# stivalaa/cuda_satabsearch

Hardware: AMD Instinct MI355X
Metric: db-structure scorings/sec (query×db pairs/sec) at r=128; 1/2/4/8 MI355X (higher is better)
Workload: dtype i32

## Files before the change

### cuda_satabsearch_amd/_native.py

```python
import ctypes as C
import os

PKG = os.path.dirname(os.path.abspath(__file__))
DEVICE_LIB = os.environ.get("SAT_DEVICE_LIB") or os.path.join(PKG, "libsatabsearch.so")
HOST_LIB = os.path.join(PKG, "libsathost.so")

MAXDIM = 111
LABELSIZE = 8

ABI_SYMBOLS = (
    "sat_last_error", "sat_abi_version", "sat_device_count", "sat_ctx_create", "sat_ctx_destroy",
    "sat_db_upload_packed", "sat_db_upload_search", "sat_db_upload_dense", "sat_db_size", "sat_query_set", "sat_search",
    "sat_search_async", "sat_device_scores", "sat_device_ssemaps", "sat_query_order", "sat_sync",
    "sat_search_timed", "sat_use_stream", "sat_use_own_stream", "sat_results", "sat_queries_set", "sat_query_count", "sat_topk",
    "sat_topk_hits", "sat_stat_d2h_bytes", "sat_debug_lds_layout", "sat_last_launch_info",
    "sat_multi_create", "sat_multi_destroy", "sat_multi_device_count", "sat_multi_gather_kind", "sat_multi_db_upload_packed",
    "sat_multi_shards", "sat_multi_queries_set", "sat_multi_search", "sat_multi_search_topk", "sat_multi_stat_d2h_bytes",
    "sat_search_matches", "sat_multi_search_matches",
    "sat_search_pairs", "sat_search_refine", "sat_multi_search_refine",
    "sat_hits_cutoff", "sat_multi_search_cutoff", "sat_multi_hits_cutoff",
    "sat_search_pairs_matches", "sat_multi_search_pairs_matches",
)


class SatError(RuntimeError):
    pass


class Hit(C.Structure):
    _fields_ = [("entry", C.c_int32), ("score", C.c_int32), ("norm2", C.c_double), ("zscore", C.c_double),
                ("pvalue", C.c_double)]


class StructSetC(C.Structure):
    _fields_ = [
        ("count", C.c_int), ("capacity", C.c_int),
        ("cells", C.c_int64), ("cells_cap", C.c_int64),
        ("order", C.POINTER(C.c_int)), ("name", C.POINTER(C.c_char)),
        ("cell_off", C.POINTER(C.c_int64)), ("tab", C.POINTER(C.c_uint8)),
        ("dist", C.POINTER(C.c_float)), ("skipped", C.c_int),
    ]


_device = None
_host = None


def device_lib():
    global _device
    if _device is None:
        if not os.path.exists(DEVICE_LIB):
            raise SatError(f"{DEVICE_LIB} is missing: run `python -m cuda_satabsearch_amd.build` "
                           "(the GPU search has no fallback implementation)")
        lib = C.CDLL(DEVICE_LIB)
        lib.sat_last_error.restype = C.c_char_p
        lib.sat_abi_version.restype = C.c_int
        lib.sat_device_count.restype = C.c_int
        lib.sat_ctx_create.restype = C.c_void_p
        lib.sat_ctx_create.argtypes = [C.c_int, C.c_uint64]
        lib.sat_ctx_destroy.argtypes = [C.c_void_p]
        lib.sat_ctx_destroy.restype = None
        lib.sat_db_upload_packed.argtypes = [C.c_void_p, C.c_int, C.c_void_p, C.c_void_p, C.c_void_p,
                                             C.c_void_p, C.c_void_p]
        lib.sat_db_upload_search.argtypes = [C.c_void_p, C.c_int, C.c_void_p, C.c_void_p, C.c_void_p,
                                             C.c_void_p, C.c_void_p, C.c_int, C.c_int, C.c_int]
        lib.sat_db_upload_dense.argtypes = [C.c_void_p, C.c_int, C.c_void_p, C.c_void_p, C.c_void_p,
                                            C.c_int, C.c_void_p]
        lib.sat_db_size.argtypes = [C.c_void_p]
        lib.sat_query_set.argtypes = [C.c_void_p, C.c_int, C.c_void_p, C.c_void_p, C.c_int, C.c_void_p,
                                      C.c_uint32]
        lib.sat_search.argtypes = [C.c_void_p, C.c_int, C.c_int, C.c_int, C.c_void_p, C.c_void_p,
                                   C.POINTER(C.c_double)]
        lib.sat_search_async.argtypes = [C.c_void_p, C.c_int, C.c_int, C.c_int]
        lib.sat_use_stream.argtypes = [C.c_void_p, C.c_void_p]
        lib.sat_use_own_stream.argtypes = [C.c_void_p]
        lib.sat_results.argtypes = [C.c_void_p, C.c_int, C.c_void_p, C.c_void_p]
        lib.sat_queries_set.argtypes = [C.c_void_p, C.c_int, C.c_void_p, C.c_void_p, C.c_void_p, C.c_int,
                                        C.c_void_p, C.c_uint32]
        lib.sat_query_count.argtypes = [C.c_void_p]
        lib.sat_topk.argtypes = [C.c_void_p, C.c_int, C.c_int, C.c_void_p, C.c_void_p]
        lib.sat_topk_hits.argtypes = [C.c_void_p, C.c_int, C.c_void_p, C.c_void_p]
        lib.sat_stat_d2h_bytes.argtypes = [C.c_void_p]
        lib.sat_stat_d2h_bytes.restype = C.c_uint64
        lib.sat_last_launch_info.argtypes = [C.c_void_p]
        lib.sat_last_launch_info.restype = C.c_char_p
        lib.sat_debug_lds_layout.argtypes = [C.c_int] * 8 + [C.c_void_p]
        lib.sat_debug_lds_layout.restype = None
        lib.sat_multi_create.restype = C.c_void_p
        lib.sat_multi_create.argtypes = [C.c_int, C.c_void_p, C.c_uint64]
        lib.sat_multi_destroy.argtypes = [C.c_void_p]
        lib.sat_multi_destroy.restype = None
        lib.sat_multi_device_count.argtypes = [C.c_void_p]
        lib.sat_multi_gather_kind.argtypes = [C.c_void_p]
        lib.sat_multi_gather_kind.restype = C.c_char_p
        lib.sat_multi_db_upload_packed.argtypes = [C.c_void_p, C.c_int, C.c_void_p, C.c_void_p, C.c_void_p, C.c_void_p]
        lib.sat_multi_shards.argtypes = [C.c_void_p, C.c_void_p]
        lib.sat_multi_queries_set.argtypes = [C.c_void_p, C.c_int, C.c_void_p, C.c_void_p, C.c_void_p, C.c_int, C.c_void_p, C.c_uint32]
        lib.sat_multi_search.argtypes = [C.c_void_p, C.c_int, C.c_int, C.c_int, C.c_void_p, C.c_void_p, C.POINTER(C.c_double)]
        lib.sat_multi_search_topk.argtypes = [C.c_void_p, C.c_int, C.c_int, C.c_int, C.c_int, C.c_void_p, C.c_void_p,
                                              C.POINTER(C.c_double)]
        lib.sat_search_matches.argtypes = [C.c_void_p, C.c_int, C.c_int, C.c_int, C.c_void_p, C.c_void_p, C.c_void_p,
                                           C.c_void_p, C.POINTER(C.c_double)]
        lib.sat_multi_search_matches.argtypes = [C.c_void_p, C.c_int, C.c_int, C.c_int, C.c_void_p, C.c_void_p,
                                                 C.c_void_p, C.c_void_p, C.POINTER(C.c_double)]
        lib.sat_search_pairs.argtypes = [C.c_void_p, C.c_int, C.c_int, C.c_int, C.c_int, C.c_void_p, C.c_void_p,
                                         C.c_void_p, C.c_void_p, C.POINTER(C.c_double)]
        lib.sat_search_pairs_matches.argtypes = [C.c_void_p, C.c_int, C.c_int, C.c_int, C.c_int, C.c_void_p, C.c_void_p,
                                                 C.c_void_p, C.c_void_p, C.c_void_p, C.c_void_p, C.POINTER(C.c_double)]
        lib.sat_multi_search_pairs_matches.argtypes = lib.sat_search_pairs_matches.argtypes
        lib.sat_search_refine.argtypes = [C.c_void_p, C.c_int, C.c_int, C.c_int, C.c_int, C.c_int, C.c_int,
                                          C.c_void_p, C.c_void_p, C.c_void_p]
        lib.sat_multi_search_refine.argtypes = [C.c_void_p, C.c_int, C.c_int, C.c_int, C.c_int, C.c_int, C.c_int,
                                                C.c_void_p, C.c_void_p, C.c_void_p, C.POINTER(C.c_double),
                                                C.POINTER(C.c_double)]
        lib.sat_hits_cutoff.argtypes = [C.c_void_p, C.c_double, C.c_int, C.c_void_p, C.c_int, C.c_void_p, C.c_void_p]
        lib.sat_multi_search_cutoff.argtypes = [C.c_void_p, C.c_int, C.c_int, C.c_int, C.c_double, C.c_int, C.c_void_p,
                                                C.c_int, C.c_void_p, C.c_void_p, C.POINTER(C.c_double)]
        lib.sat_multi_hits_cutoff.argtypes = [C.c_void_p, C.c_double, C.c_int, C.c_void_p, C.c_int, C.c_void_p, C.c_void_p]
        lib.sat_multi_stat_d2h_bytes.argtypes = [C.c_void_p]
        lib.sat_multi_stat_d2h_bytes.restype = C.c_uint64
        lib.sat_device_scores.argtypes = [C.c_void_p]
        lib.sat_device_scores.restype = C.c_void_p
        lib.sat_device_ssemaps.argtypes = [C.c_void_p]
        lib.sat_device_ssemaps.restype = C.c_void_p
        lib.sat_query_order.argtypes = [C.c_void_p]
        lib.sat_sync.argtypes = [C.c_void_p]
        lib.sat_search_timed.argtypes = [C.c_void_p, C.c_int, C.c_int, C.c_int, C.c_int,
                                         C.POINTER(C.c_double), C.POINTER(C.c_double)]
        _device = lib
    return _device


def host_lib():
    global _host
    if _host is None:
        if not os.path.exists(HOST_LIB):
            raise SatError(f"{HOST_LIB} is missing: run `python -m cuda_satabsearch_amd.build`")
        lib = C.CDLL(HOST_LIB)
        lib.sat_set_init.argtypes = [C.POINTER(StructSetC)]
        lib.sat_set_init.restype = None
        lib.sat_set_free.argtypes = [C.POINTER(StructSetC)]
        lib.sat_set_free.restype = None
        lib.sat_read_structures.argtypes = [C.c_void_p, C.POINTER(StructSetC), C.c_char_p]
        lib.sat_read_structures.restype = C.c_int
        lib.sat_read_structures_file.argtypes = [C.c_char_p, C.POINTER(StructSetC), C.c_char_p]
        lib.sat_read_structures_file.restype = C.c_int
        lib.sat_set_save_binary.argtypes = [C.POINTER(StructSetC), C.c_char_p]
        lib.sat_set_load_binary.argtypes = [C.c_char_p, C.POINTER(StructSetC)]
        lib.sat_set_write_ascii.argtypes = [C.POINTER(StructSetC), C.c_char_p]
        lib.sat_distance_cell.argtypes = [C.c_char_p]
        lib.sat_distance_cell.restype = C.c_float
        lib.sat_norm2.argtypes = [C.c_int, C.c_int, C.c_int]
        lib.sat_norm2.restype = C.c_double
        lib.sat_z_gumbel_trunc.argtypes = [C.c_double]
        lib.sat_z_gumbel_trunc.restype = C.c_double
        lib.sat_pv_gumbel.argtypes = [C.c_double]
        lib.sat_pv_gumbel.restype = C.c_double
        lib.sat_entry_cost.argtypes = [C.c_int]
        lib.sat_entry_cost.restype = C.c_double
        lib.sat_shard_cuts.argtypes = [C.c_int, C.c_void_p, C.c_int, C.c_void_p]
        _host = lib
    return _host


_libc = C.CDLL(None)
_libc.fopen.restype = C.c_void_p
_libc.fopen.argtypes = [C.c_char_p, C.c_char_p]
_libc.fclose.argtypes = [C.c_void_p]
_libc.fgets.restype = C.c_void_p
_libc.fgets.argtypes = [C.c_char_p, C.c_int, C.c_void_p]


def libc():
    return _libc
```

### cuda_satabsearch_amd/csrc/diag/sat_diag.hpp

```cpp
#pragma once

#define SAT_DIAG_ARGS unsigned long long *diag;

#ifdef SAT_DIAG_PHASE
#define SAT_PHASE_INIT unsigned long long ph_acc[11] = {0, 0, 0, 0, 0, 0, 0, 0, 0, 0, 0}, ph_t0 = __builtin_amdgcn_s_memtime()
#define SAT_PHASE(k) do { const unsigned long long ph_t1 = __builtin_amdgcn_s_memtime(); ph_acc[k] += ph_t1 - ph_t0; ph_t0 = ph_t1; } while (0)
#define SAT_PHASE_FLUSH do { if ((threadIdx.x & 63) == 0) for (int k = 0; k < 11; k++) if (k < 8 || k == 10) atomicAdd(a.diag + k, ph_acc[k]); } while (0)
#endif

#ifdef SAT_DIAG_FS_ROWS
#define SAT_DIAG_FS_ROWS_ONLY 1
#endif

#ifdef SAT_DIAG_DUP
#if SAT_DIAG_DUP == 1
#define SAT_DIAG_DUP_CELLS(row, l0, l1, l2, l3) do { if constexpr (CELLS == SAT_CELLS_FULL8) {                                            \
        typedef const volatile __attribute__((address_space(3))) unsigned long long *lds_vu64;                          \
        const unsigned long long dup0 = *(lds_vu64)&(row).cells[l0], dup1 = *(lds_vu64)&(row).cells[l1],                  \
                                 dup2 = *(lds_vu64)&(row).cells[l2], dup3 = *(lds_vu64)&(row).cells[l3];                  \
        asm volatile("" : : "v"(dup0), "v"(dup1), "v"(dup2), "v"(dup3)); } } while (0)
#elif SAT_DIAG_DUP == 2
#define SAT_DIAG_DUP_MAPWORD(p) (void)*(const volatile __attribute__((address_space(3))) uint32_t *)(p)
#elif SAT_DIAG_DUP == 3
#define SAT_DIAG_DUP_ATOMIC(p) __hip_atomic_fetch_add((p), 0, __ATOMIC_RELAXED, __HIP_MEMORY_SCOPE_WAVEFRONT)
#elif SAT_DIAG_DUP == 4
#define SAT_DIAG_DUP_MAPBYTE(p) (void)*(const volatile __attribute__((address_space(3))) uint8_t *)(p)
#endif
#endif

#ifdef SAT_DIAG_PERTURB
#define SAT_R10(x) x x x x x x x x x x
namespace satk {
__device__ __forceinline__ void perturb(uint32_t (&d)[4])
{
#if SAT_DIAG_PERTURB == 1
    asm volatile(SAT_R10("v_add_u32 %0, %0, 1\n v_add_u32 %1, %1, 1\n v_add_u32 %2, %2, 1\n v_add_u32 %3, %3, 1\n")
                 : "+v"(d[0]), "+v"(d[1]), "+v"(d[2]), "+v"(d[3]));
#elif SAT_DIAG_PERTURB == 2
    uint32_t s0 = __builtin_amdgcn_readfirstlane(d[1]), s1 = __builtin_amdgcn_readfirstlane(d[2]);
    asm volatile(SAT_R10("s_add_u32 %0, %0, 1\n s_add_u32 %1, %1, 1\n s_add_u32 %0, %0, 3\n s_add_u32 %1, %1, 3\n")
                 : "+s"(s0), "+s"(s1) : : "scc");
    d[1] = s0; d[2] = s1;
#elif SAT_DIAG_PERTURB == 3
    uint32_t addr = (threadIdx.x & 63u) << 2, t0, t1;
    asm volatile("ds_read_b32 %0, %2\n ds_read_b32 %1, %2 offset:256\n ds_read_b32 %0, %2 offset:512\n ds_read_b32 %1, %2 offset:768\n"
                 "ds_read_b32 %0, %2 offset:1024\n ds_read_b32 %1, %2 offset:1280\n ds_read_b32 %0, %2 offset:1536\n"
                 "ds_read_b32 %1, %2 offset:1792\n ds_read_b32 %0, %2 offset:2048\n ds_read_b32 %1, %2 offset:2304\n s_waitcnt lgkmcnt(0)\n"
                 : "=&v"(t0), "=&v"(t1) : "v"(addr) : "memory");
    d[0] ^= t0 & t1 & 0x80000000u;
#elif SAT_DIAG_PERTURB == 4
    asm volatile(SAT_R10("s_nop 0\n s_nop 0\n s_nop 0\n s_nop 0\n"));
#elif SAT_DIAG_PERTURB == 5
    asm volatile(SAT_R10("v_lshlrev_b32 %0, 1, %0\n v_lshlrev_b32 %1, 1, %1\n v_lshlrev_b32 %2, 1, %2\n v_lshlrev_b32 %3, 1, %3\n")
                 : "+v"(d[0]), "+v"(d[1]), "+v"(d[2]), "+v"(d[3]));
#endif
}
}
#define SAT_DIAG_PERTURB_INIT uint32_t pert[4] = { (uint32_t)lane_id, 1u, 2u, 3u }
#define SAT_DIAG_PERTURB_STEP satk::perturb(pert)
#define SAT_DIAG_PERTURB_END do { if ((pert[0] ^ pert[1] ^ pert[2] ^ pert[3]) == 0xDEADBEEFu) Q.scores[e] = -1; } while (0)
#endif

#ifdef SAT_DIAG_SELFCHECK
#define SAT_DIAG_SELFCHECK_STEP do {                                                                                     \
        const uint8_t keep_ = smap_b[map_byte_addr(ssei)];                                                               \
        smap_b[map_byte_addr(ssei)] = (uint8_t)newj;                                                                     \
        int chk_ = score_rows();                                                                                         \
        if (lpc >= 2) chk_ += __shfl_xor(chk_, 1, 64);                                                                   \
        if (lpc == 4) chk_ += __shfl_xor(chk_, 2, 64);                                                                   \
        smap_b[map_byte_addr(ssei)] = keep_;                                                                             \
        if (part == 0) { atomicAdd(a.diag + 9, 1ull); if (chk_ != newscore) atomicAdd(a.diag + 8, 1ull); }               \
    } while (0)
#endif

#if defined(SAT_DIAG_HOST)
#include <cstdio>
namespace satdiag {
inline unsigned long long *&buffer() { static unsigned long long *d = nullptr; return d; }
inline unsigned long long (&last())[16] { static unsigned long long h[16]; return h; }
inline hipError_t begin(hipStream_t stream, unsigned long long *&arg)
{
    if (!buffer()) { hipError_t e = hipMalloc(&buffer(), 16 * sizeof(unsigned long long)); if (e != hipSuccess) return e; }
    arg = buffer();
    return hipMemsetAsync(buffer(), 0, 16 * sizeof(unsigned long long), stream);
}
inline hipError_t end(hipStream_t stream)
{
    hipError_t e = hipStreamSynchronize(stream);
    if (e != hipSuccess) return e;
    e = hipMemcpy(last(), buffer(), sizeof(unsigned long long) * 16, hipMemcpyDeviceToHost);
#ifdef SAT_DIAG_PHASE
    unsigned long long tot = 0;
    for (int k = 0; k < 11; k++) if (k < 8 || k == 10) tot += last()[k];
    static const char *nm[11] = { "draw+proposal", "compaction set-up", "compacted rounds", "read-back/static loops",
                                 "best tracking", "metropolis+update", "initial full score", "staging+restart loop", "", "",
                                 "thinit" };
    for (int k = 0; k < 11; k++)
        if (k < 8 || k == 10) fprintf(stderr, "phase %-24s %14llu wave-cycles %5.1f%%\n", nm[k], last()[k], tot ? 100.0 * last()[k] / tot : 0.0);
#endif
    return e;
}
}
extern "C" void sat_diag_counters(unsigned long long out[16]) { for (int k = 0; k < 16; k++) out[k] = satdiag::last()[k]; }
#endif
```

### cuda_satabsearch_amd/csrc/sat_capi.hip

```cpp
#include <hip/hip_runtime.h>

#include <algorithm>
#include <atomic>
#include <chrono>
#include <cmath>
#include <cstdarg>
#include <cstdio>
#include <cstdlib>
#include <cstring>
#include <new>
#include <thread>
#include <type_traits>
#include <vector>

#include "satabsearch.h"
#ifdef SAT_DIAG
#define SAT_DIAG_HOST 1
#endif
#include "sat_sa_kernel.hpp"
#include "sat_ctx.hpp"
#include "host/sat_gumbel.h"

namespace {

thread_local char g_err[512] = "";

}

int sat_fail(int code, const char *fmt, ...)
{
    va_list ap;
    va_start(ap, fmt);
    vsnprintf(g_err, sizeof(g_err), fmt, ap);
    va_end(ap);
    return code;
}

namespace {

const int kBucketMax[kNumBuckets] = { 16, 32, 48, 64, 80, 96, 111 };
constexpr size_t kLdsLimit = 160 * 1024;

int build_metropolis_table(sat_ctx *ctx)
{
    const int max_nd = 4 * (SAT_MAXDIM - 1);
    const float umin = 2.3283064e-10f;
    std::vector<float> tab;
    std::vector<int32_t> rows(2 * SAT_MAXITER);
    volatile float temp = 10.0f;
    for (int it = 0; it < SAT_MAXITER; it++) {
        int last = 0;
        std::vector<float> row(max_nd + 1);
        for (int nd = 0; nd <= max_nd; nd++) {
            volatile float x = (float)(-nd) / temp;
            row[nd] = expf(x);
            if (row[nd] > umin) last = nd;
        }
        rows[2 * it] = (int32_t)tab.size();
        rows[2 * it + 1] = last;
        tab.push_back(8589934592.0f);
        for (int nd = 0; nd <= last; nd++) tab.push_back(ldexpf(row[nd], 32));
        tab.push_back(0.0f);
        temp = temp * 0.95f;
    }
    int rc;
    if ((rc = ctx->d_ptab.grow(tab.size())) != SAT_OK || (rc = ctx->d_prow.grow(rows.size())) != SAT_OK) return rc;
    HIP_TRY(hipMemcpy(ctx->d_ptab.get(), tab.data(), tab.size() * sizeof(float), hipMemcpyHostToDevice));
    HIP_TRY(hipMemcpy(ctx->d_prow.get(), rows.data(), rows.size() * sizeof(int32_t), hipMemcpyHostToDevice));
    return SAT_OK;
}

int build_gumbel_tables(sat_ctx *ctx)
{
    double z[256], p[256];
    for (int x = -128; x < 128; x++) {
        z[x + 128] = sat_z_gumbel_trunc((double)x);
        p[x + 128] = sat_pv_gumbel(z[x + 128]);
    }
    int rc;
    if ((rc = ctx->d_gumbel_z.grow(256)) != SAT_OK || (rc = ctx->d_gumbel_p.grow(256)) != SAT_OK) return rc;
    HIP_TRY(hipMemcpy(ctx->d_gumbel_z.get(), z, sizeof z, hipMemcpyHostToDevice));
    HIP_TRY(hipMemcpy(ctx->d_gumbel_p.get(), p, sizeof p, hipMemcpyHostToDevice));
    return SAT_OK;
}

void free_db(sat_ctx *ctx)
{
    ctx->d_orders.reset();
    ctx->d_cell_off.reset();
    ctx->d_tab.reset();
    ctx->d_dist.reset();
    ctx->d_ordinal.reset();
    ctx->d_lists.reset();
    ctx->d_scores.reset();
    ctx->d_ssemaps.reset();
    ctx->desc_dirty = true;
    ctx->n_entries = 0;
    ctx->min_rows = 0;
    ctx->searched_nq = 0;
    ctx->h_orders.clear();
}

template <int V> using Int = std::integral_constant<int, V>;

template <typename F> auto by_class(int n1p, F f)
{
    switch (n1p) {
    case 16: return f(Int<16>{});
    case 32: return f(Int<32>{});
    case 64: return f(Int<64>{});
    default: return f(Int<112>{});
    }
}

template <typename F> auto by_flag(bool b, F f) { return b ? f(std::true_type{}) : f(std::false_type{}); }

template <int First, int Last, typename F> auto by_value(int v, F f)
{
    if constexpr (First == Last) return f(Int<Last>{});
    else return v == First ? f(Int<First>{}) : by_value<First + 1, Last>(v, f);
}

template <typename F> auto by_layout(int m2w, int cells, F f)
{
    if (m2w == 1) return f(Int<1>{}, Int<SAT_CELLS_FULL8>{});
    if (m2w == 2) return cells == SAT_CELLS_FULL5 ? f(Int<2>{}, Int<SAT_CELLS_FULL5>{}) : f(Int<2>{}, Int<SAT_CELLS_TRI5>{});
    return f(Int<4>{}, Int<SAT_CELLS_TRI5>{});
}

enum SaMode { kPlain = 0, kMatch = 1, kPair = 2, kPairMatch = 3 };

struct SaKernel { const void *fn; int mode, n1p, m2w, cells; bool qlds; int opt, wpl; };

template <int MODE, int N1P, int M2W, bool QLDS, int OPT, int WPL, int CELLS> const void *sa_instance()
{
    static_assert(MODE == kPlain || WPL == 0, "words per lane are an argument of the plain kernel only");
    static_assert(MODE == kPlain || MODE == kPair || OPT == -1, "the match families read their options from the arguments");
    if constexpr (MODE == kPlain) return reinterpret_cast<const void *>(sat_sa_kernel<N1P, M2W, QLDS, OPT, WPL, CELLS>);
    else if constexpr (MODE == kPair) return reinterpret_cast<const void *>(sat_sa_pair_kernel<N1P, M2W, QLDS, OPT, CELLS>);
    else if constexpr (MODE == kMatch) return reinterpret_cast<const void *>(sat_sa_match_kernel<N1P, M2W, QLDS, CELLS>);
    else return reinterpret_cast<const void *>(sat_sa_pair_match_kernel<N1P, M2W, QLDS, CELLS>);
}

SaKernel pick_sa_kernel(int mode, int n1p, int m2w, int cells, bool qlds, int opt, int wpl)
{
    SaKernel k = { nullptr, mode, n1p, m2w, cells, qlds, -1, 0 };
    by_value<kPlain, kPairMatch>(mode, [&](auto md) {
        by_class(n1p, [&](auto c) {
            constexpr int MODE = decltype(md)::value, N1P = decltype(c)::value;
            constexpr bool kQ = N1P < 32;
            auto take = [&](auto q, auto o, auto w) {
                k.opt = decltype(o)::value;
                k.wpl = decltype(w)::value;
                k.fn = by_layout(m2w, cells, [](auto m, auto l) {
                    return sa_instance<MODE, N1P, decltype(m)::value, decltype(q)::value, decltype(o)::value, decltype(w)::value,
                                       decltype(l)::value>();
                });
            };
            const std::bool_constant<kQ> q{};
            if constexpr (MODE == kPlain) {
                if (opt >= 4 && qlds == kQ && m2w == 4)
                    return by_value<4, 11>(opt, [&](auto o) {
                        k.opt = decltype(o)::value;
                        k.fn = sa_instance<kPlain, N1P, 4, kQ, decltype(o)::value, 0, SAT_CELLS_TRI5>();
                    });
                if (opt >= 0 && opt < 4 && qlds == kQ)
                    return by_value<0, 3>(opt, [&](auto o) {
                        if constexpr ((decltype(o)::value & 1) == 0) take(q, o, Int<0>{});
                        else {
                            if (wpl == 4) return take(q, o, Int<4>{});
                            if constexpr (N1P <= 64)
                                if (wpl == 3) return take(q, o, Int<3>{});
                            if constexpr (N1P == 16) {
                                if (wpl == 2) return take(q, o, Int<2>{});
                                if (wpl == 1) return take(q, o, Int<1>{});
                            }
                            take(q, o, Int<0>{});
                        }
                    });
            }
            if constexpr (MODE == kPair)
                if ((opt == 0 || opt == 1) && qlds == kQ) return by_value<0, 1>(opt, [&](auto o) { take(q, o, Int<0>{}); });
            by_flag(qlds, [&](auto qg) { take(qg, Int<-1>{}, Int<0>{}); });
        });
    });
    return k;
}

hipError_t launch_sa(const SaKernel &k, dim3 grid, dim3 block, size_t lds, hipStream_t stream, const SatKernelArgs &a,
                     const SatPairArgs *px, const SatMatchArgs *mx)
{
    void *args[3] = { const_cast<SatKernelArgs *>(&a), nullptr, nullptr };
    int n = 1;
    if (k.mode & kPair) args[n++] = const_cast<SatPairArgs *>(px);
    if (k.mode & kMatch) args[n++] = const_cast<SatMatchArgs *>(mx);
    (void)hipLaunchKernel(k.fn, grid, block, args, lds, stream);
    return hipGetLastError();
}

std::string launch_info(const SaKernel &k, int items, int grid_x, int grid_y, int epw, int threads, size_t lds)
{
    static const char *const kName[4] = { "sat_sa_kernel", "sat_sa_match_kernel", "sat_sa_pair_kernel", "sat_sa_pair_match_kernel" };
    char targs[48] = "", count[32] = "", buf[200];
    if (k.mode == kPlain) snprintf(targs, sizeof targs, "%d, %d, ", k.opt, k.wpl);
    if (k.mode == kPair) snprintf(targs, sizeof targs, "%d, ", k.opt);
    if (k.mode & kPair) snprintf(count, sizeof count, " items %d", items);
    snprintf(buf, sizeof buf, "%s<%d, %d, %s, %s%d>%s grid %d x %d block %d x %d lds %zu", kName[k.mode], k.n1p, k.m2w,
             k.qlds ? "true" : "false", targs, k.cells, count, grid_x, grid_y, epw, threads, lds);
    return buf;
}

const int kClassN1P[4] = { 16, 32, 64, 112 };

int refresh_descriptors(sat_ctx *ctx, bool lsoln, hipStream_t stream)
{
    const size_t nq = ctx->queries.size();
    const size_t rows = (size_t)(ctx->n_entries > ctx->min_rows ? ctx->n_entries : ctx->min_rows);
    bool moved = false;
    int rc = ctx->d_scores.grow(nq * rows, &moved);
    if (rc != SAT_OK) return rc;
    if (moved) ctx->desc_dirty = true;
    if (lsoln) {
        size_t need = 0, n1sum = 0;
        for (auto &q : ctx->queries) {
            q.ssemap_off = need;
            need += (size_t)ctx->n_entries * q.n1;
            n1sum += (size_t)q.n1;
        }
        if (rows * n1sum > need) need = rows * n1sum;
        if ((rc = ctx->d_ssemaps.grow(need, &moved)) != SAT_OK) return rc;
        if (moved || !ctx->desc_lsoln) ctx->desc_dirty = true;
    }
    if (!ctx->desc_dirty) return SAT_OK;

    std::vector<SatQuery> desc;
    desc.reserve(nq);
    for (int c = 0; c < 4; c++) {
        ctx->class_begin[c] = (int)desc.size();
        ctx->class_n1max[c] = 0;
        ctx->class_wpl[c] = -1;
        for (size_t qi = 0; qi < nq; qi++) {
            auto &q = ctx->queries[qi];
            if (q.n1p != kClassN1P[c]) continue;
            q.cls = c;
            q.desc = (int)desc.size();
            const uint8_t *blob = ctx->d_qblob.get() + q.blob_off;
            const size_t groups = (size_t)q.n1p / 4 * q.n1p;
            SatQuery d;
            d.qdist = reinterpret_cast<const float4 *>(blob);
            d.qcode = reinterpret_cast<const uint32_t *>(blob + groups * 16);
            d.qtypes = blob + groups * 20;
            d.qpair = reinterpret_cast<const uint2 *>(blob + ((groups * 20 + (size_t)q.n1p + 15) & ~(size_t)15));
            d.n1 = q.n1;
            d.pad_ = 0;
            d.seed_q = ctx->seed + ((uint64_t)q.ordinal << 32);
            d.scores = ctx->d_scores.get() + qi * (size_t)ctx->n_entries;
            d.ssemaps = lsoln ? ctx->d_ssemaps.get() + q.ssemap_off : nullptr;
            desc.push_back(d);
            if (q.n1 > ctx->class_n1max[c]) ctx->class_n1max[c] = q.n1;
            int lpi, wpl;
            satk::compaction_shape((q.n1 + 3) >> 2, lpi, wpl);
            ctx->class_wpl[c] = ctx->class_wpl[c] < 0 ? wpl : (ctx->class_wpl[c] == wpl ? wpl : 0);
        }
        if (ctx->class_wpl[c] < 0) ctx->class_wpl[c] = 0;
    }
    ctx->class_begin[4] = (int)desc.size();
    HIP_TRY(hipMemcpyAsync(ctx->d_qdesc.get(), desc.data(), desc.size() * sizeof(SatQuery), hipMemcpyHostToDevice, stream));
    HIP_TRY(hipStreamSynchronize(stream));
    ctx->desc_dirty = false;
    ctx->desc_lsoln = lsoln;
    return SAT_OK;
}

int resident_by_lds(size_t bytes) { return (int)(128 / ((bytes + 1279) / 1280)); }

int pick_epw(const void *fn, int threads, size_t lds_stride)
{
    int best = 1, best_entries = 0;
    for (int k = 1; k * threads <= 512 && (size_t)k * lds_stride <= kLdsLimit; k++) {
        if (k > 1 && (k * threads / 64) % 4 != 0) continue;
        int by_regs = 0;
        if (hipOccupancyMaxActiveBlocksPerMultiprocessor(&by_regs, fn, k * threads, 0) != hipSuccess) {
            (void)hipGetLastError();
            return 1;
        }
        const int by_lds = resident_by_lds((size_t)k * lds_stride);
        const int entries = (by_regs < by_lds ? by_regs : by_lds) * k;
        if (entries > best_entries) { best_entries = entries; best = k; }
    }
    return best;
}

int launch_setup(sat_ctx *ctx, const void *fn, int threads, size_t lds_stride, long long work, int *epw)
{
    if (ctx->lds_attr_done.insert(fn).second)
        HIP_TRY(hipFuncSetAttribute(fn, hipFuncAttributeMaxDynamicSharedMemorySize, (int)kLdsLimit));
    if (!epw) return SAT_OK;
    *epw = 1;
    if (work >= 8192) {
        const auto key = std::make_tuple(fn, threads, lds_stride);
        auto it = ctx->epw_choice.find(key);
        if (it == ctx->epw_choice.end()) it = ctx->epw_choice.emplace(key, pick_epw(fn, threads, lds_stride)).first;
        *epw = it->second;
    }
    if (ctx->tune.epw >= 1 && (size_t)ctx->tune.epw * lds_stride <= kLdsLimit && ctx->tune.epw * threads <= 1024)
        *epw = ctx->tune.epw;
    return SAT_OK;
}

SatKernelArgs base_args(const sat_ctx *ctx, int lorder, int lsoln, int maxstart)
{
    SatKernelArgs a;
    a.orders = ctx->d_orders.get();
    a.cell_off = ctx->d_cell_off.get();
    a.tab_tri = ctx->d_tab.get();
    a.dist_tri = ctx->d_dist.get();
    a.ordinal = ctx->d_ordinal.get();
    a.lorder = lorder ? 1 : 0;
    a.lsoln = lsoln ? 1 : 0;
    a.maxstart = maxstart;
    a.ptab = ctx->d_ptab.get();
    a.prow = ctx->d_prow.get();
    a.bmap_slabs = nullptr;
    a.bmap_slab_words = 0;
    return a;
}

int check_ready(const sat_ctx *ctx, bool need_db, int maxstart)
{
    if (!ctx) return sat_fail(SAT_EINVAL, "null context");
    if (need_db && ctx->n_entries <= 0) return sat_fail(SAT_ESTATE, "no database uploaded");
    if (ctx->queries.empty()) return sat_fail(SAT_ESTATE, "no query set");
    if (maxstart < 1) return sat_fail(SAT_EINVAL, "maxstart must be >= 1 (got %d)", maxstart);
    return SAT_OK;
}

struct WgShape { int chains, lpc_shift, threads; bool qlds, compact; size_t lds; };
int size_workgroup(const sat_ctx *ctx, int plan_starts, int n1max, int n1p, int n2max, bool lsoln, bool lorder, WgShape &out)
{
    int chains = (plan_starts + 63) / 64 * 64;
    if (chains > 256) chains = 256;
    if (ctx->tune.chains >= 64 && ctx->tune.chains < chains) chains = ctx->tune.chains / 64 * 64;
    bool compact = lorder != 0;
    if (ctx->tune.compact >= 0) compact = ctx->tune.compact != 0;
    bool qlds = n1p < 32;
    if (ctx->tune.qlds >= 0) qlds = ctx->tune.qlds != 0 || n1p < 32;
    size_t lds = 0;
    for (;;) {
        lds = satk::lds_bytes(n1max, n1p, n2max, chains, chains, lsoln, qlds, compact);
        if (lds <= kLdsLimit) break;
        if (chains > 64) { chains -= 64; continue; }
        if (qlds) {
            qlds = false;
            chains = (plan_starts + 63) / 64 * 64;
            if (chains > 256) chains = 256;
            continue;
        }
        return sat_fail(SAT_EINVAL, "workgroup does not fit in LDS (n1=%d n2=%d)", n1max, n2max);
    }
    int lpc_shift = 0;
    for (int l = 0; l <= 2; l++) {
        if ((chains << l) > 1024 || (l > 0 && n1max <= (8 << (l - 1)))) break;
        const size_t lds_l = satk::lds_bytes(n1max, n1p, n2max, chains, chains << l, lsoln, qlds, compact);
        if (lds_l > kLdsLimit) break;
        lpc_shift = l;
        const int want_waves = ctx->tune.lpc_waves > 0 ? ctx->tune.lpc_waves : (n1p == 112 ? 12 : 8);
        if (resident_by_lds(lds_l) * ((chains << l) / 64) >= want_waves) break;
    }
    if (ctx->tune.lpc >= 0 && ctx->tune.lpc <= 2 && (chains << ctx->tune.lpc) <= 1024) lpc_shift = ctx->tune.lpc;
    for (;; lpc_shift--) {
        lds = satk::lds_bytes(n1max, n1p, n2max, chains, chains << lpc_shift, lsoln, qlds, compact);
        if (lds <= kLdsLimit || lpc_shift == 0) break;
    }
    const int threads = chains << lpc_shift;
    if (ctx->tune.lds_pad && lds + ctx->tune.lds_pad <= kLdsLimit) lds += ctx->tune.lds_pad;
    out.chains = chains;
    out.lpc_shift = lpc_shift;
    out.threads = threads;
    out.qlds = qlds;
    out.compact = compact;
    out.lds = lds;
    return SAT_OK;
}

struct SaLaunch { WgShape w; SaKernel k; int epw; size_t lds_stride, lds_launch; SatKernelArgs args; };

int prepare_sa(sat_ctx *ctx, int mode, int lorder, int lsoln, int maxstart, int plan_starts, int c, int n2max, long long work,
               bool pack, SaLaunch &out)
{
    const int n1p = kClassN1P[c], m2w = satk::set_words(n2max);
    WgShape &w = out.w;
    int rc = size_workgroup(ctx, plan_starts, ctx->class_n1max[c], n1p, n2max, lsoln != 0, lorder != 0, w);
    if (rc != SAT_OK) return rc;
    const bool special = (w.lpc_shift == 0 || m2w == 4) && w.compact == (lorder != 0) && !ctx->tune.general && !(mode & kMatch);
    const int opt = special ? (lorder ? 1 : 0) | (lsoln ? 2 : 0) | (w.lpc_shift << 2) : -1;
    out.k = pick_sa_kernel(mode, n1p, m2w, satk::cell_layout(n2max), w.qlds, opt, ctx->class_wpl[c]);
    if (!out.k.fn) return sat_fail(SAT_EDEVICE, "no kernel variant for n1p=%d m2w=%d", n1p, m2w);
    out.lds_stride = (w.lds + 15) & ~(size_t)15;
    out.epw = 1;
    if ((rc = launch_setup(ctx, out.k.fn, w.threads, out.lds_stride, work, pack ? &out.epw : nullptr)) != SAT_OK) return rc;
    out.lds_launch = out.epw > 1 ? (size_t)out.epw * out.lds_stride : w.lds;
    out.args = base_args(ctx, lorder, lsoln, maxstart);
    out.args.epw = out.epw;
    out.args.tpe = w.threads;
    out.args.lds_stride = (uint32_t)out.lds_stride;
    out.args.lpc_shift = w.lpc_shift;
    out.args.compact = w.compact ? 1 : 0;
    return SAT_OK;
}

struct ListView {
    const int32_t *d_list;
    const int *begin;
    const int *n2max;
    int n;
};

int launch_search(sat_ctx *ctx, int lorder, int lsoln, int maxstart, hipStream_t stream, const ListView *piece = nullptr,
                  const SatMatchArgs *mx = nullptr)
{
    int rc = check_ready(ctx, true, maxstart);
    if (rc != SAT_OK) return rc;
    const ListView whole = { ctx->d_lists.get(), ctx->bucket_begin, ctx->bucket_n2max, ctx->n_entries };
    const ListView &view = piece ? *piece : whole;
    HIP_TRY(hipSetDevice(ctx->device));
    if ((rc = refresh_descriptors(ctx, lsoln != 0, stream)) != SAT_OK) return rc;
#ifdef SAT_DIAG
    unsigned long long *diag = nullptr;
    HIP_TRY(satdiag::begin(stream, diag));
#endif

    const bool replay = mx && mx->replay;
    struct Planned { SaLaunch l; int count, nqc, n2max, max_entries; size_t slab_words; };
    std::vector<Planned> plan;
    for (int c = 0; c < 4; c++) {
        const int nqc = ctx->class_begin[c + 1] - ctx->class_begin[c];
        if (nqc == 0) continue;
        const bool one_launch = (long long)view.n * nqc <= 4096;
        int overall_n2max = 0;
        for (int b = 0; b < kNumBuckets; b++)
            if (view.n2max[b] > overall_n2max) overall_n2max = view.n2max[b];
        for (int b = 0; b < kNumBuckets; b++) {
            Planned pl;
            pl.count = view.begin[b + 1] - view.begin[b];
            pl.n2max = view.n2max[b];
            if (one_launch) {
                if (b > 0) break;
                pl.count = view.n;
                pl.n2max = overall_n2max;
            }
            if (pl.count == 0) continue;
            pl.nqc = nqc;
            rc = prepare_sa(ctx, mx ? kMatch : kPlain, lorder, lsoln, maxstart, replay ? mx->max_matches : maxstart, c, pl.n2max,
                            (long long)pl.count * nqc, true, pl.l);
            if (rc != SAT_OK) return rc;
            pl.l.args.queries = ctx->d_qdesc.get() + ctx->class_begin[c];
            pl.l.args.entry_list = view.d_list + (one_launch ? view.begin[0] : view.begin[b]);
#ifdef SAT_DIAG
            pl.l.args.diag = diag;
#endif
            pl.slab_words = (lsoln || replay) ? (size_t)((ctx->class_n1max[c] + 3) / 4) * pl.l.w.chains
                          : (mx ? (size_t)(1 + pl.l.k.m2w) * (size_t)maxstart : 0);
            plan.push_back(pl);
        }
    }

    std::stable_sort(plan.begin(), plan.end(), [](const Planned &x, const Planned &y) { return x.n2max > y.n2max; });
    const bool fork = plan.size() > 1 && ctx->tune.streams != 0 && ctx->side_stream[0] != nullptr;
    const int nlanes = fork ? (int)(plan.size() < (size_t)kNumBuckets ? plan.size() : (size_t)kNumBuckets) : 1;
    if (fork) HIP_TRY(hipEventRecord(ctx->ev_fork, stream));
    const size_t lane_budget_words = ((size_t)1 << 30) / 4 / (size_t)nlanes;
    const bool slabs = lsoln || mx;
    if (slabs) {
        size_t need_total = 0;
        for (size_t i = 0; i < plan.size(); i++) {
            Planned &pl = plan[i];
            size_t fit = lane_budget_words / pl.slab_words;
            if (fit < 1) fit = 1;
            const int qn_cap = pl.nqc < 65535 ? pl.nqc : 65535;
            pl.max_entries = (int)(fit / (size_t)qn_cap);
            if (pl.max_entries < 1) pl.max_entries = 1;
            if (pl.max_entries > pl.count) pl.max_entries = pl.count;
            const size_t need = pl.slab_words * (size_t)(pl.max_entries + pl.l.epw - 1) * (size_t)qn_cap;
            if (need > need_total) need_total = need;
        }
        need_total *= (size_t)nlanes;
        if ((rc = ctx->d_bmap_slabs.grow_after(stream, need_total)) != SAT_OK) return rc;
    }
    const size_t lane_region_words = slabs ? ctx->d_bmap_slabs.capacity() / (size_t)nlanes : 0;
    for (size_t i = 0; i < plan.size(); i++) {
        const Planned &pl = plan[i];
        const int lane = fork ? (int)(i % (size_t)nlanes) : 0;
        hipStream_t s = fork ? ctx->side_stream[lane] : stream;
        if (fork && i < (size_t)nlanes) HIP_TRY(hipStreamWaitEvent(s, ctx->ev_fork, 0));
        const int max_entries = slabs ? pl.max_entries : pl.count, epw = pl.l.epw;
        for (int q0 = 0; q0 < pl.nqc; q0 += 65535) {
            const int qn = pl.nqc - q0 < 65535 ? pl.nqc - q0 : 65535;
            for (int e0 = 0; e0 < pl.count; e0 += max_entries) {
                const int en = pl.count - e0 < max_entries ? pl.count - e0 : max_entries;
                SatKernelArgs part = pl.l.args;
                part.queries += q0;
                part.entry_list += e0;
                part.n_list = en;
                SatMatchArgs mpart = mx ? *mx : SatMatchArgs{};
                if (lsoln || replay) {
                    part.bmap_slabs = ctx->d_bmap_slabs.get() + (size_t)lane * lane_region_words;
                    part.bmap_slab_words = (uint32_t)pl.slab_words;
                } else if (mx) {
                    mpart.rec_slabs = ctx->d_bmap_slabs.get() + (size_t)lane * lane_region_words;
                    mpart.rec_slab_words = (uint32_t)pl.slab_words;
                }
                HIP_TRY(launch_sa(pl.l.k, dim3((en + epw - 1) / epw, qn), dim3(pl.l.w.threads * epw), pl.l.lds_launch, s, part, nullptr,
                                  &mpart));
            }
        }
    }
    if (fork)
        for (int lane = 0; lane < nlanes; lane++) {
            HIP_TRY(hipEventRecord(ctx->ev_join[lane], ctx->side_stream[lane]));
            HIP_TRY(hipStreamWaitEvent(stream, ctx->ev_join[lane], 0));
        }
    ctx->searched_nq = ctx->queries.size();
    ctx->searched_lsoln = lsoln != 0;
    ctx->last_launch_info.clear();
    for (size_t i = 0; i < plan.size(); i++) {
        const Planned &pl = plan[i];
        if (i) ctx->last_launch_info += "; ";
        ctx->last_launch_info += launch_info(pl.l.k, 0, (pl.count + pl.l.epw - 1) / pl.l.epw, pl.nqc, pl.l.epw, pl.l.w.threads, pl.l.w.lds);
    }
#ifdef SAT_DIAG
    HIP_TRY(satdiag::end(stream));
#endif
    return SAT_OK;
}


int order_bucket(int n2)
{
    int b = 0;
    while (b < kNumBuckets - 1 && n2 > kBucketMax[b]) b++;
    return b;
}

__global__ void __launch_bounds__(256) pair_winners(SatPairItem *items, int n, const unsigned long long *keys)
{
    const int i = blockIdx.x * blockDim.x + threadIdx.x;
    if (i >= n) return;
    const int r = (int)(0xFFFFFFFFu - (uint32_t)(keys[items[i].pair] & 0xFFFFFFFFu));
    items[i].r0 = r;
    items[i].r1 = r + 1;
}

__global__ void __launch_bounds__(256) pair_scores(const unsigned long long *keys, int n, int32_t *scores)
{
    const int i = blockIdx.x * blockDim.x + threadIdx.x;
    if (i < n) scores[i] = (int32_t)(uint32_t)(keys[i] >> 32) - 0x40000000;
}

__global__ void __launch_bounds__(256) pair_match_select(int pair0, int R, int M, const uint32_t *slabs, uint32_t slab_words,
                                                         const uint8_t *setw, const unsigned long long *keys, int32_t *counts,
                                                         int32_t *scores, int32_t *restarts)
{
    __shared__ unsigned long long red[4];
    __shared__ uint32_t uni[4];
    const int p = pair0 + (int)blockIdx.x;
    const uint32_t *rec = slabs + (size_t)blockIdx.x * slab_words;
    const int W = setw[p];
    const int t = (int)threadIdx.x, wave = t >> 6;
    if (t < 4) uni[t] = 0u;
    int m = 0;
    unsigned long long first = 0ull;
    for (int round = 0; round < M; round++) {
        __syncthreads();
        unsigned long long k = 0ull;
        for (int r = t; r < R; r += 256) {
            const int s = (int)rec[r];
            uint32_t hit = 0u;
            for (int w = 0; w < W; w++) hit |= rec[(size_t)(w + 1) * (size_t)R + (size_t)r] & uni[w];
            const unsigned long long rk = (((unsigned long long)(uint32_t)(s + 0x40000000)) << 32) | (0xFFFFFFFFu - (uint32_t)r);
            k = ((round == 0 || (s > 0 && hit == 0u)) && rk > k) ? rk : k;
        }
#pragma unroll
        for (int off = 32; off > 0; off >>= 1) {
            const unsigned long long other = __shfl_xor(k, off, 64);
            k = other > k ? other : k;
        }
        if ((t & 63) == 0) red[wave] = k;
        __syncthreads();
        unsigned long long cur = red[0];
        for (int w = 1; w < 4; w++) cur = red[w] > cur ? red[w] : cur;
        if (cur == 0ull) break;
        if (round == 0) first = cur;
        const uint32_t r = 0xFFFFFFFFu - (uint32_t)(cur & 0xFFFFFFFFu);
        if (t == 0) {
            scores[(size_t)p * M + m] = (int32_t)(uint32_t)(cur >> 32) - 0x40000000;
            restarts[(size_t)p * M + m] = (int32_t)r;
        }
        if (t < W) uni[t] |= rec[(size_t)(t + 1) * (size_t)R + (size_t)r];
        m++;
    }
    if (t == 0) {
        counts[p] = first == keys[p] ? m : -1;
        for (int x = m; x < M; x++) {
            scores[(size_t)p * M + x] = 0;
            restarts[(size_t)p * M + x] = -1;
        }
    }
}

struct PairMatchPass { SatMatchArgs mx; int maxstart; };

struct PairGroups { std::vector<size_t> goff, moff; std::vector<int> gcls, gn2; };

int launch_pair_pass(sat_ctx *ctx, int lorder, bool map_pass, int starts, const SatPairItem *d_items, const PairGroups &grp,
                     std::string &info, const PairMatchPass *pm = nullptr)
{
    hipStream_t stream = ctx->stream;
    const std::vector<size_t> &off = map_pass ? grp.moff : grp.goff;
    SatPairArgs px;
    px.items = nullptr;
    px.keys = ctx->d_pkeys.get();
    px.maps = ctx->d_pmaps.get();
    SatMatchArgs mpart = pm ? pm->mx : SatMatchArgs{};
    mpart.replay = map_pass ? 1 : 0;
    for (size_t g = 0; g < grp.gcls.size(); g++) {
        const int count = (int)(off[g + 1] - off[g]);
        if (count == 0) continue;
        SaLaunch l;
        int rc = prepare_sa(ctx, pm ? kPairMatch : kPair, lorder, map_pass && !pm, pm ? pm->maxstart : starts,
                            map_pass ? (pm ? pm->mx.max_matches : 1) : starts, grp.gcls[g], grp.gn2[g], count, !map_pass, l);
        if (rc != SAT_OK) return rc;
        SatKernelArgs &a = l.args;
        a.entry_list = nullptr;
        a.queries = ctx->d_qdesc.get();
#ifdef SAT_DIAG
        HIP_TRY(satdiag::begin(stream, a.diag));
#endif
        int per_launch = count;
        if (map_pass) {
            const size_t slab_words = (size_t)((ctx->class_n1max[grp.gcls[g]] + 3) / 4) * (size_t)l.w.chains;
            const size_t budget = ((size_t)1 << 28) / 4;
            per_launch = (int)std::min<size_t>((size_t)count, std::max<size_t>(1, budget / slab_words));
            const size_t slabs = (size_t)per_launch + (size_t)l.epw - 1;
            if ((rc = ctx->d_bmap_slabs.grow_after(stream, slab_words * slabs)) != SAT_OK) return rc;
            a.bmap_slabs = ctx->d_bmap_slabs.get();
            a.bmap_slab_words = (uint32_t)slab_words;
        }
        for (int i0 = 0; i0 < count; i0 += per_launch) {
            const int n = count - i0 < per_launch ? count - i0 : per_launch;
            a.n_list = n;
            px.items = d_items + off[g] + (size_t)i0;
            HIP_TRY(launch_sa(l.k, dim3((n + l.epw - 1) / l.epw, 1), dim3(l.w.threads * l.epw), l.lds_launch, stream, a, &px, &mpart));
        }
        if (!info.empty()) info += "; ";
        info += launch_info(l.k, count, (count + l.epw - 1) / l.epw, 1, l.epw, l.w.threads, l.w.lds);
#ifdef SAT_DIAG
        HIP_TRY(satdiag::end(stream));
#endif
    }
    return SAT_OK;
}

int check_pairs(const sat_ctx *ctx, const int32_t *query, const int32_t *entry, int npairs)
{
    if (npairs < 0 || (npairs > 0 && (!query || !entry))) return sat_fail(SAT_EINVAL, "bad pair list");
    const int nq = (int)ctx->queries.size();
    for (int p = 0; p < npairs; p++) {
        if (query[p] < 0 || query[p] >= nq) return sat_fail(SAT_EINVAL, "pair %d: query %d out of range", p, query[p]);
        if (entry[p] < 0 || entry[p] >= ctx->n_entries) return sat_fail(SAT_EINVAL, "pair %d: entry %d out of range", p, entry[p]);
    }
    return SAT_OK;
}

int pair_split(const sat_ctx *ctx, int maxstart, int npairs)
{
    if (ctx->tune.refine_split > 0) return ctx->tune.refine_split < maxstart ? ctx->tune.refine_split : maxstart;
    constexpr long long kTargetItems = 2048;
    const int t0 = std::min(256, (maxstart + 63) / 64 * 64);
    const long long rounds = (maxstart + t0 - 1) / t0;
    long long items = (kTargetItems + npairs - 1) / npairs;
    if (items > rounds) items = rounds;
    if (items < 1) items = 1;
    const long long per = (rounds + items - 1) / items;
    return (int)std::min<long long>(maxstart, per * t0);
}

size_t pair_item_count(int npairs, int maxstart, int split, bool maps)
{
    return (size_t)npairs * (size_t)((maxstart + split - 1) / split) + (maps ? (size_t)npairs : 0);
}

PairGroups build_pair_items(const sat_ctx *ctx, const int32_t *query, const int32_t *entry, int p0, int n, int maxstart, int split,
                            bool maps, std::vector<SatPairItem> &items, uint8_t *setw)
{
    std::vector<std::vector<int>> members(4 * kNumBuckets);
    std::vector<int> n2max(4 * kNumBuckets, 0);
    for (int p = p0; p < p0 + n; p++) {
        const int n2 = ctx->h_orders[(size_t)entry[p]];
        const int g = ctx->queries[(size_t)query[p]].cls * kNumBuckets + order_bucket(n2);
        members[(size_t)g].push_back(p);
        n2max[(size_t)g] = std::max(n2max[(size_t)g], n2);
    }
    auto item_of = [&](int p, int r0, int r1) {
        SatPairItem it{};
        it.pair = p;
        it.desc = ctx->queries[(size_t)query[p]].desc;
        it.entry = entry[p];
        it.r0 = r0;
        it.r1 = r1;
        it.slab = p - p0;
        return it;
    };
    PairGroups grp;
    grp.goff.push_back(items.size());
    for (int g = 0; g < 4 * kNumBuckets; g++) {
        if (members[(size_t)g].empty()) continue;
        for (int p : members[(size_t)g]) {
            if (setw) setw[p] = (uint8_t)satk::set_words(n2max[(size_t)g]);
            for (int r0 = 0; r0 < maxstart; r0 += split) items.push_back(item_of(p, r0, maxstart - r0 < split ? maxstart : r0 + split));
        }
        grp.goff.push_back(items.size());
        grp.gcls.push_back(g / kNumBuckets);
        grp.gn2.push_back(n2max[(size_t)g]);
    }
    if (maps) {
        grp.moff.push_back(items.size());
        for (int g = 0; g < 4 * kNumBuckets; g++) {
            if (members[(size_t)g].empty()) continue;
            for (int p : members[(size_t)g]) items.push_back(item_of(p, 0, 0));
            grp.moff.push_back(items.size());
        }
    }
    return grp;
}

void expand_map(const int8_t *in, int n1, bool used, int32_t *out)
{
    for (int i = 0; i < SAT_MAXDIM; i++) out[i] = (used && i < n1) ? in[i] : -1;
}

int match_args(const sat_ctx *ctx, int max_matches, SatMatchArgs &mx)
{
    if (!ctx) return sat_fail(SAT_EINVAL, "null context");
    if (max_matches < 1 || max_matches > SAT_MAX_MATCHES)
        return sat_fail(SAT_EINVAL, "max_matches must be 1..%d (got %d)", SAT_MAX_MATCHES, max_matches);
    mx = SatMatchArgs{};
    mx.desc_base = ctx->d_qdesc.get();
    mx.max_matches = max_matches;
    mx.map_pitch = SAT_MAXDIM;
    return SAT_OK;
}

}

int sat_pairs_launch(sat_ctx *ctx, int lorder, int maxstart, bool maps, const int32_t *query, const int32_t *entry, int npairs)
{
    int rc = check_ready(ctx, true, maxstart);
    if (rc != SAT_OK) return rc;
    if ((rc = check_pairs(ctx, query, entry, npairs)) != SAT_OK) return rc;
    HIP_TRY(hipSetDevice(ctx->device));
    if ((rc = refresh_descriptors(ctx, false, ctx->stream)) != SAT_OK) return rc;
    ctx->last_launch_info.clear();
    if (npairs == 0) return SAT_OK;

    const int split = pair_split(ctx, maxstart, npairs);
    std::vector<SatPairItem> &items = ctx->h_pitems;
    HIP_TRY(hipStreamSynchronize(ctx->stream));
    items.clear();
    items.reserve(pair_item_count(npairs, maxstart, split, maps));
    const PairGroups grp = build_pair_items(ctx, query, entry, 0, npairs, maxstart, split, maps, items, nullptr);
    if ((rc = ctx->d_pitems.grow_after(ctx->stream, items.size())) != SAT_OK) return rc;
    if ((rc = ctx->d_pkeys.grow_after(ctx->stream, (size_t)npairs)) != SAT_OK) return rc;
    if (maps && (rc = ctx->d_pmaps.grow_after(ctx->stream, (size_t)npairs * SAT_MAXDIM)) != SAT_OK) return rc;
    HIP_TRY(hipMemcpyAsync(ctx->d_pitems.get(), items.data(), items.size() * sizeof(SatPairItem), hipMemcpyHostToDevice, ctx->stream));
    HIP_TRY(hipMemsetAsync(ctx->d_pkeys.get(), 0, (size_t)npairs * sizeof(unsigned long long), ctx->stream));
    std::string info;
    rc = launch_pair_pass(ctx, lorder, false, split, ctx->d_pitems.get(), grp, info);
    if (rc != SAT_OK) return rc;
    char head[96];
    snprintf(head, sizeof head, "score pass (%d restarts, %d per item): ", maxstart, split);
    ctx->last_launch_info = head + info;
    if (maps) {
        const size_t n_score = grp.moff[0];
        const int n_map = (int)(items.size() - n_score);
        HIP_TRY(hipMemsetAsync(ctx->d_pmaps.get(), 0xFF, (size_t)npairs * SAT_MAXDIM, ctx->stream));
        hipLaunchKernelGGL(pair_winners, dim3((unsigned)((n_map + 255) / 256)), dim3(256), 0, ctx->stream,
                           ctx->d_pitems.get() + n_score, n_map, ctx->d_pkeys.get());
        HIP_TRY(hipGetLastError());
        info.clear();
        rc = launch_pair_pass(ctx, lorder, true, 1, ctx->d_pitems.get(), grp, info);
        if (rc != SAT_OK) return rc;
        ctx->last_launch_info += " | map pass: " + info;
    }
    return SAT_OK;
}

int sat_launch_plain(sat_ctx *ctx, int lorder, int maxstart)
{
    return launch_search(ctx, lorder, 0, maxstart, ctx->stream);
}

int sat_pairs_collect(sat_ctx *ctx, int npairs, int32_t *scores, int32_t *ssemaps, const int32_t *query)
{
    HIP_TRY(hipSetDevice(ctx->device));
    if (npairs == 0) return SAT_OK;
    const int rc = ctx->d_pscores.grow_after(ctx->stream, (size_t)npairs);
    if (rc != SAT_OK) return rc;
    hipLaunchKernelGGL(pair_scores, dim3((unsigned)((npairs + 255) / 256)), dim3(256), 0, ctx->stream, ctx->d_pkeys.get(), npairs,
                       ctx->d_pscores.get());
    HIP_TRY(hipGetLastError());
    HIP_TRY(hipStreamSynchronize(ctx->stream));
    HIP_TRY(hipMemcpy(scores, ctx->d_pscores.get(), (size_t)npairs * sizeof(int32_t), hipMemcpyDeviceToHost));
    ctx->d2h_bytes += (size_t)npairs * sizeof(int32_t);
    if (ssemaps) {
        std::vector<int8_t> mp((size_t)npairs * SAT_MAXDIM);
        HIP_TRY(hipMemcpy(mp.data(), ctx->d_pmaps.get(), mp.size(), hipMemcpyDeviceToHost));
        ctx->d2h_bytes += mp.size();
        for (size_t p = 0; p < (size_t)npairs; p++)
            expand_map(mp.data() + p * SAT_MAXDIM, ctx->queries[(size_t)query[p]].n1, true, ssemaps + p * SAT_MAXDIM);
    }
    return SAT_OK;
}

int sat_pair_matches_launch(sat_ctx *ctx, int lorder, int maxstart, int max_matches, bool maps, const int32_t *query,
                            const int32_t *entry, int npairs)
{
    PairMatchPass pm{};
    int rc = match_args(ctx, max_matches, pm.mx);
    if (rc != SAT_OK) return rc;
    if ((rc = check_ready(ctx, true, maxstart)) != SAT_OK) return rc;
    if ((rc = check_pairs(ctx, query, entry, npairs)) != SAT_OK) return rc;
    HIP_TRY(hipSetDevice(ctx->device));
    if ((rc = refresh_descriptors(ctx, false, ctx->stream)) != SAT_OK) return rc;
    ctx->last_launch_info.clear();
    if (npairs == 0) return SAT_OK;
    const size_t M = (size_t)max_matches;
    const int split = pair_split(ctx, maxstart, npairs);

    int n2_all = 0;
    for (int p = 0; p < npairs; p++) n2_all = std::max(n2_all, ctx->h_orders[(size_t)entry[p]]);
    const size_t slab_words = (size_t)(1 + satk::set_words(n2_all)) * (size_t)maxstart;
    const size_t budget_words = ((size_t)1 << 30) / 4;
    const int chunk = (int)std::min<size_t>((size_t)npairs, std::max<size_t>(1, budget_words / slab_words));

    struct Chunk { int p0, n; PairGroups grp; };
    std::vector<Chunk> chunks;
    std::vector<SatPairItem> &items = ctx->h_pitems;
    std::vector<uint8_t> &setw = ctx->h_psetw;
    HIP_TRY(hipStreamSynchronize(ctx->stream));
    items.clear();
    items.reserve(pair_item_count(npairs, maxstart, split, maps));
    setw.assign((size_t)npairs, 0);
    for (int p0 = 0; p0 < npairs; p0 += chunk) {
        const int n = std::min(chunk, npairs - p0);
        chunks.push_back({ p0, n, build_pair_items(ctx, query, entry, p0, n, maxstart, split, maps, items, setw.data()) });
    }
    if ((rc = ctx->d_pitems.grow_after(ctx->stream, items.size())) != SAT_OK ||
        (rc = ctx->d_pkeys.grow_after(ctx->stream, (size_t)npairs)) != SAT_OK ||
        (rc = ctx->d_psetw.grow_after(ctx->stream, (size_t)npairs)) != SAT_OK ||
        (rc = ctx->d_pmout.grow_after(ctx->stream, (size_t)npairs * (1 + 2 * M))) != SAT_OK ||
        (rc = ctx->d_bmap_slabs.grow_after(ctx->stream, slab_words * (size_t)chunk)) != SAT_OK ||
        (maps && (rc = ctx->d_pmaps.grow_after(ctx->stream, (size_t)npairs * M * SAT_MAXDIM)) != SAT_OK))
        return rc;
    HIP_TRY(hipMemcpyAsync(ctx->d_pitems.get(), items.data(), items.size() * sizeof(SatPairItem), hipMemcpyHostToDevice, ctx->stream));
    HIP_TRY(hipMemcpyAsync(ctx->d_psetw.get(), setw.data(), setw.size(), hipMemcpyHostToDevice, ctx->stream));
    HIP_TRY(hipMemsetAsync(ctx->d_pkeys.get(), 0, (size_t)npairs * sizeof(unsigned long long), ctx->stream));
    if (maps) HIP_TRY(hipMemsetAsync(ctx->d_pmaps.get(), 0xFF, (size_t)npairs * M * SAT_MAXDIM, ctx->stream));

    pm.maxstart = maxstart;
    pm.mx.n_entries = 0;
    pm.mx.rec_slab_words = (uint32_t)slab_words;
    pm.mx.counts = ctx->d_pmout.get();
    pm.mx.scores = pm.mx.counts + npairs;
    pm.mx.restarts = pm.mx.scores + (size_t)npairs * M;
    pm.mx.maps = ctx->d_pmaps.get();
    std::string rec_info, map_info;
    for (const Chunk &ch : chunks) {
        pm.mx.rec_slabs = ctx->d_bmap_slabs.get();
        if ((rc = launch_pair_pass(ctx, lorder, false, split, ctx->d_pitems.get(), ch.grp, rec_info, &pm)) != SAT_OK)
            return rc;
        hipLaunchKernelGGL(pair_match_select, dim3((unsigned)ch.n), dim3(256), 0, ctx->stream, ch.p0, maxstart, max_matches,
                           (const uint32_t *)ctx->d_bmap_slabs.get(), (uint32_t)slab_words, (const uint8_t *)ctx->d_psetw.get(),
                           (const unsigned long long *)ctx->d_pkeys.get(), pm.mx.counts, pm.mx.scores, pm.mx.restarts);
        HIP_TRY(hipGetLastError());
        if (maps && (rc = launch_pair_pass(ctx, lorder, true, 1, ctx->d_pitems.get(), ch.grp, map_info, &pm)) != SAT_OK)
            return rc;
    }
    char head[128];
    snprintf(head, sizeof head, "record pass (%d restarts, %d per item, %zu launches of up to %d pairs): ", maxstart, split,
             chunks.size(), chunk);
    ctx->last_launch_info = head + rec_info + " | select";
    if (maps) ctx->last_launch_info += " | map pass: " + map_info;
    return SAT_OK;
}

int sat_pair_matches_collect(sat_ctx *ctx, int max_matches, int npairs, int32_t *counts, int32_t *scores, int32_t *restarts,
                             int32_t *ssemaps, const int32_t *query)
{
    HIP_TRY(hipSetDevice(ctx->device));
    if (npairs == 0) return SAT_OK;
    HIP_TRY(hipStreamSynchronize(ctx->stream));
    const size_t P = (size_t)npairs, M = (size_t)max_matches;
    std::vector<int32_t> out(P * (1 + 2 * M));
    HIP_TRY(hipMemcpy(out.data(), ctx->d_pmout.get(), out.size() * sizeof(int32_t), hipMemcpyDeviceToHost));
    ctx->d2h_bytes += out.size() * sizeof(int32_t);
    for (size_t p = 0; p < P; p++)
        if (out[p] < 1 || out[p] > (int32_t)M)
            return sat_fail(SAT_EDEVICE, "pair %zu: the records and the arg-max key of the record pass disagree", p);
    memcpy(counts, out.data(), P * sizeof(int32_t));
    memcpy(scores, out.data() + P, P * M * sizeof(int32_t));
    memcpy(restarts, out.data() + P + P * M, P * M * sizeof(int32_t));
    if (ssemaps) {
        std::vector<int8_t> mp(P * M * SAT_MAXDIM);
        HIP_TRY(hipMemcpy(mp.data(), ctx->d_pmaps.get(), mp.size(), hipMemcpyDeviceToHost));
        ctx->d2h_bytes += mp.size();
        for (size_t p = 0; p < P; p++)
            for (size_t m = 0; m < M; m++)
                expand_map(mp.data() + (p * M + m) * SAT_MAXDIM, ctx->queries[(size_t)query[p]].n1, (int32_t)m < counts[p],
                           ssemaps + (p * M + m) * SAT_MAXDIM);
    }
    return SAT_OK;
}

namespace {

__global__ void __launch_bounds__(256) validate_cells(int e_begin, int e_end, const int32_t *orders, const int64_t *cell_off,
                                                      const uint8_t *tab, const float *dist, int32_t *first_bad)
{
    const int e = e_begin + blockIdx.x * 4 + (threadIdx.x >> 6), lane = threadIdx.x & 63;
    if (e >= e_end) return;
    const int n = orders[e];
    const int64_t base = cell_off[e];
    const int cells = n * (n + 1) / 2;
    bool bad = false;
    for (int c = lane; c < cells; c += 64) {
        int i = (int)((sqrtf(8.0f * (float)c + 1.0f) - 1.0f) * 0.5f);
        while ((i + 1) * (i + 2) / 2 <= c) i++;
        while (i * (i + 1) / 2 > c) i--;
        const bool diagonal = c == i * (i + 1) / 2 + i;
        const uint8_t t = tab[base + c];
        if (diagonal) {
            bad |= t > 3;
        } else {
            const float ad = fabsf(dist[base + c]);
            bad |= (t & 0x88u) != 0 || (ad >= 1.0e29f && ad <= 3.4028234e38f);
        }
    }
    if (__builtin_amdgcn_ballot_w64(bad) != 0ull && lane == 0) atomicMin(first_bad, e);
}

template <typename F> int timed(sat_ctx *ctx, double *kernel_ms, F launch)
{
    HIP_TRY(hipSetDevice(ctx->device));
    HIP_TRY(hipEventRecord(ctx->ev0, ctx->stream));
    const int rc = launch();
    if (rc != SAT_OK) return rc;
    HIP_TRY(hipEventRecord(ctx->ev1, ctx->stream));
    HIP_TRY(hipStreamSynchronize(ctx->stream));
    if (kernel_ms) {
        float ms = 0.f;
        HIP_TRY(hipEventElapsedTime(&ms, ctx->ev0, ctx->ev1));
        *kernel_ms = ms;
    }
    return SAT_OK;
}

}

extern "C" {

const char *sat_last_error(void) { return g_err; }

int sat_abi_version(void) { return SAT_ABI_VERSION; }

int sat_device_count(void)
{
    int n = 0;
    if (hipGetDeviceCount(&n) != hipSuccess) return 0;
    return n;
}

sat_ctx *sat_ctx_create(int device, uint64_t seed)
{
    int n = sat_device_count();
    if (n <= 0) {
        sat_fail(SAT_ENODEVICE, "no HIP device available (this library has no CPU path)");
        return nullptr;
    }
    if (device < 0 || device >= n) {
        sat_fail(SAT_ENODEVICE, "device %d out of range (0..%d)", device, n - 1);
        return nullptr;
    }
    sat_ctx *ctx = new (std::nothrow) sat_ctx();
    if (!ctx) {
        sat_fail(SAT_ENOMEM, "out of host memory");
        return nullptr;
    }
    ctx->device = device;
    ctx->seed = seed;
    auto init = [&]() -> int {
        HIP_TRY(hipSetDevice(device));
        HIP_TRY(hipStreamCreateWithFlags(&ctx->own_stream, hipStreamNonBlocking));
        ctx->stream = ctx->own_stream;
        HIP_TRY(hipEventCreate(&ctx->ev0));
        HIP_TRY(hipEventCreate(&ctx->ev1));
        auto env_int = [](const char *name, int dflt) { const char *v = getenv(name); return v && *v ? atoi(v) : dflt; };
        ctx->tune.compact = env_int("SAT_EXP_COMPACT", -1);
        ctx->tune.qlds = env_int("SAT_EXP_QLDS", -1);
        ctx->tune.lpc = env_int("SAT_EXP_LPC", -1);
        ctx->tune.general = env_int("SAT_EXP_GENERAL", 0);
        ctx->tune.streams = env_int("SAT_EXP_STREAMS", -1);
        ctx->tune.upload_threads = env_int("SAT_EXP_UPLOAD_THREADS", 0);
        ctx->tune.upload_timing = env_int("SAT_EXP_UPLOAD_TIMING", 0);
        ctx->tune.upload_pieces = env_int("SAT_EXP_UPLOAD_PIECES", 0);
        ctx->tune.epw = env_int("SAT_EXP_EPW", 0);
        ctx->tune.lpc_waves = env_int("SAT_EXP_LPC_WAVES", 0);
        ctx->tune.chains = env_int("SAT_EXP_CHAINS", 0);
        ctx->tune.refine_split = env_int("SAT_EXP_REFINE_SPLIT", 0);
        const int pad = env_int("SAT_EXP_LDS_PAD", 0);
        ctx->tune.lds_pad = pad > 0 ? (size_t)pad : 0;
        if (ctx->tune.streams != 0) {
            for (int b = 0; b < kNumBuckets; b++) {
                HIP_TRY(hipStreamCreateWithFlags(&ctx->side_stream[b], hipStreamNonBlocking));
                HIP_TRY(hipEventCreateWithFlags(&ctx->ev_join[b], hipEventDisableTiming));
            }
            HIP_TRY(hipEventCreateWithFlags(&ctx->ev_fork, hipEventDisableTiming));
        }
        const int rc_tab = build_metropolis_table(ctx);
        if (rc_tab != SAT_OK) return rc_tab;
        hipLaunchKernelGGL(validate_cells, dim3(1), dim3(256), 0, ctx->stream, 0, 0, nullptr, nullptr, nullptr, nullptr, nullptr);
        HIP_TRY(hipGetLastError());
        HIP_TRY(hipStreamSynchronize(ctx->stream));
        return build_gumbel_tables(ctx);
    };
    if (init() != SAT_OK) {
        sat_ctx_destroy(ctx);
        return nullptr;
    }
    return ctx;
}

void sat_ctx_destroy(sat_ctx *ctx)
{
    if (!ctx) return;
    (void)hipSetDevice(ctx->device);
    (void)hipStreamSynchronize(ctx->stream);
    std::vector<hipEvent_t> events = { ctx->ev0, ctx->ev1, ctx->ev_fork };
    events.insert(events.end(), ctx->ev_join, ctx->ev_join + kNumBuckets);
    std::vector<hipStream_t> streams(ctx->side_stream, ctx->side_stream + kNumBuckets);
    streams.push_back(ctx->own_stream);
    delete ctx;
    for (hipEvent_t e : events)
        if (e) (void)hipEventDestroy(e);
    for (hipStream_t st : streams)
        if (st) (void)hipStreamDestroy(st);
}

struct FirstSearch { int lorder, lsoln, maxstart; };

static void bucket_lists(const int32_t *orders, int e_begin, int e_end, int32_t *out, int pos, int *begin, int *n2max)
{
    int count[SAT_MAXDIM + 1] = { 0 }, start[SAT_MAXDIM + 1] = { 0 };
    for (int e = e_begin; e < e_end; e++) count[orders[e]]++;
    for (int b = 0; b < kNumBuckets; b++) {
        begin[b] = pos;
        n2max[b] = 0;
        const int lo = b == 0 ? 0 : kBucketMax[b - 1];
        for (int n = kBucketMax[b] < SAT_MAXDIM ? kBucketMax[b] : SAT_MAXDIM; n > lo; n--) {
            start[n] = pos;
            pos += count[n];
            if (count[n] && n2max[b] == 0) n2max[b] = n;
        }
    }
    begin[kNumBuckets] = pos;
    for (int e = e_begin; e < e_end; e++) out[(size_t)start[orders[e]]++] = e;
}

static int upload_impl(sat_ctx *ctx, int n_entries, const int32_t *orders,
                       const int64_t *cell_off, const uint8_t *tab_tri,
                       const float *dist_tri, const int64_t *db_ordinal, const FirstSearch *first)
{
    if (!ctx) return sat_fail(SAT_EINVAL, "null context");
    if (n_entries <= 0 || !orders || !cell_off || !tab_tri || !dist_tri)
        return sat_fail(SAT_EINVAL, "empty database or null array");
    if (first) {
        const int rc = check_ready(ctx, false, first->maxstart);
        if (rc != SAT_OK) return rc;
    }
    int64_t cells_end = 0;
    bool ascending = true;
    for (int e = 0; e < n_entries; e++) {
        const int n = orders[e];
        if (n < 1 || n > SAT_MAXDIM)
            return sat_fail(SAT_EINVAL, "entry %d: order %d outside 1..%d", e, n, SAT_MAXDIM);
        if (cell_off[e] < 0) return sat_fail(SAT_EINVAL, "entry %d: negative cell offset", e);
        if (cell_off[e] < cells_end) ascending = false;
        int64_t end = cell_off[e] + (int64_t)n * (n + 1) / 2;
        if (end > cells_end) cells_end = end;
        if (db_ordinal && (db_ordinal[e] < 0 || db_ordinal[e] > 0xFFFFFFFFll))
            return sat_fail(SAT_EINVAL, "entry %d: db ordinal out of range", e);
    }
    HIP_TRY(hipSetDevice(ctx->device));
    HIP_TRY(hipStreamSynchronize(ctx->stream));
    free_db(ctx);
    const bool timing = ctx->tune.upload_timing != 0;
    auto now_ms = [] { return std::chrono::duration<double, std::milli>(std::chrono::steady_clock::now().time_since_epoch()).count(); };
    double t_mark = now_ms();
    auto lap = [&](const char *what) {
        if (timing) { const double t = now_ms(); fprintf(stderr, "upload: %-18s %7.3f ms\n", what, t - t_mark); t_mark = t; }
    };

    const size_t dist_bytes = (size_t)cells_end * sizeof(float), tab_bytes = (size_t)cells_end;
    int npieces = 1;
    if (first && ascending) {
        const size_t by_size = dist_bytes / ((size_t)24 << 20);
        npieces = ctx->tune.upload_pieces > 0 ? ctx->tune.upload_pieces : (int)(by_size < 8 ? by_size : 8);
        if (npieces > n_entries) npieces = n_entries;
        if (npieces < 1) npieces = 1;
    }
    std::vector<int> piece_e((size_t)npieces + 1, n_entries);
    piece_e[0] = 0;
    for (int c = 1, e = 0; c < npieces; c++) {
        const int64_t target = cells_end * c / npieces;
        while (e < n_entries && cell_off[e] < target) e++;
        piece_e[(size_t)c] = e > piece_e[(size_t)c - 1] ? e : piece_e[(size_t)c - 1];
    }
    auto piece_cell = [&](int c) -> int64_t { return c >= npieces || piece_e[(size_t)c] >= n_entries ? cells_end : (c == 0 ? 0 : cell_off[piece_e[(size_t)c]]); };

    std::vector<int32_t> lists((size_t)n_entries * (npieces > 1 ? 2 : 1));
    bucket_lists(orders, 0, n_entries, lists.data(), 0, ctx->bucket_begin, ctx->bucket_n2max);
    std::vector<int> piece_begin((size_t)npieces * (kNumBuckets + 1)), piece_n2max((size_t)npieces * kNumBuckets);
    if (npieces > 1) {
        int pos = n_entries;
        for (int c = 0; c < npieces; c++) {
            bucket_lists(orders, piece_e[(size_t)c], piece_e[(size_t)c + 1], lists.data(), pos,
                         &piece_begin[(size_t)c * (kNumBuckets + 1)], &piece_n2max[(size_t)c * kNumBuckets]);
            pos += piece_e[(size_t)c + 1] - piece_e[(size_t)c];
        }
    }

    std::vector<uint32_t> ord(n_entries);
    for (int e = 0; e < n_entries; e++) ord[e] = db_ordinal ? (uint32_t)db_ordinal[e] : (uint32_t)e;

    lap("host lists");
    DevBuf<int32_t> d_bad;
    const int32_t none = 0x7FFFFFFF;
    auto body = [&]() -> int {
        const size_t n = (size_t)n_entries;
        int rc;
        if ((rc = ctx->d_orders.grow(n)) != SAT_OK || (rc = ctx->d_cell_off.grow(n)) != SAT_OK ||
            (rc = ctx->d_ordinal.grow(n)) != SAT_OK || (rc = ctx->d_lists.grow(lists.size())) != SAT_OK ||
            (rc = ctx->d_tab.grow((size_t)cells_end)) != SAT_OK || (rc = ctx->d_dist.grow((size_t)cells_end)) != SAT_OK ||
            (rc = ctx->d_scores.grow(n)) != SAT_OK || (rc = d_bad.grow(1)) != SAT_OK)
            return rc;
        lap("hipMalloc");
        HIP_TRY(hipMemcpy(ctx->d_orders.get(), orders, n * sizeof(int32_t), hipMemcpyHostToDevice));
        HIP_TRY(hipMemcpy(ctx->d_cell_off.get(), cell_off, n * sizeof(int64_t), hipMemcpyHostToDevice));
        HIP_TRY(hipMemcpy(ctx->d_ordinal.get(), ord.data(), n * sizeof(uint32_t), hipMemcpyHostToDevice));
        HIP_TRY(hipMemcpy(ctx->d_lists.get(), lists.data(), lists.size() * sizeof(int32_t), hipMemcpyHostToDevice));
        HIP_TRY(hipMemset(ctx->d_scores.get(), 0, n * sizeof(int32_t)));
        HIP_TRY(hipMemcpy(d_bad.get(), &none, sizeof none, hipMemcpyHostToDevice));
        lap("header copies");
        ctx->n_entries = n_entries;

        unsigned hw = std::thread::hardware_concurrency();
        int nthreads = (int)(hw ? (hw < 4 ? hw : 4) : 1);
        if (ctx->tune.upload_threads > 0) nthreads = ctx->tune.upload_threads;
        if (dist_bytes < ((size_t)32 << 20)) nthreads = 1;
        std::vector<hipError_t> err((size_t)nthreads, hipSuccess);
        std::vector<std::atomic<int>> landed((size_t)npieces);
        for (auto &x : landed) x.store(0);
        auto copy_piece = [&](int t, int c) {
            const size_t c0 = (size_t)piece_cell(c), c1 = (size_t)piece_cell(c + 1);
            auto part = [&](const void *src, void *dst, size_t unit) {
                const size_t bytes = (c1 - c0) * unit, base = c0 * unit;
                const size_t lo = (bytes * (size_t)t / (size_t)nthreads) & ~(size_t)255;
                const size_t hi = t + 1 == nthreads ? bytes : (bytes * (size_t)(t + 1) / (size_t)nthreads) & ~(size_t)255;
                if (hi > lo && err[(size_t)t] == hipSuccess)
                    err[(size_t)t] = hipMemcpy((char *)dst + base + lo, (const char *)src + base + lo, hi - lo, hipMemcpyHostToDevice);
            };
            part(dist_tri, ctx->d_dist.get(), sizeof(float));
            part(tab_tri, ctx->d_tab.get(), 1);
            landed[(size_t)c].fetch_add(1, std::memory_order_release);
        };
        auto piece_complete = [&](int c) {
            while (landed[(size_t)c].load(std::memory_order_acquire) < nthreads) std::this_thread::yield();
        };
        auto helper = [&](int t) {
            (void)hipSetDevice(ctx->device);
            for (int c = 0; c < npieces; c++) {
                copy_piece(t, c);
                if (c + 1 < npieces) piece_complete(c);
            }
        };
        std::vector<std::thread> pool;
        for (int t = 1; t < nthreads; t++) pool.emplace_back(helper, t);
        rc = SAT_OK;
        for (int c = 0; c < npieces; c++) {
            copy_piece(0, c);
            piece_complete(c);
            if (rc != SAT_OK) continue;
            const int e0 = piece_e[(size_t)c], e1 = piece_e[(size_t)c + 1];
            if (e1 <= e0) continue;
            hipLaunchKernelGGL(validate_cells, dim3((unsigned)((e1 - e0 + 3) / 4)), dim3(256), 0, ctx->stream,
                               e0, e1, ctx->d_orders.get(), ctx->d_cell_off.get(), ctx->d_tab.get(), ctx->d_dist.get(), d_bad.get());
            if (hipGetLastError() != hipSuccess) { rc = sat_fail(SAT_EDEVICE, "launch of the cell check failed"); continue; }
            if (first) {
                if (npieces > 1) {
                    const ListView piece = { ctx->d_lists.get(), &piece_begin[(size_t)c * (kNumBuckets + 1)],
                                             &piece_n2max[(size_t)c * kNumBuckets], e1 - e0 };
                    rc = launch_search(ctx, first->lorder, first->lsoln, first->maxstart, ctx->stream, &piece);
                } else {
                    rc = launch_search(ctx, first->lorder, first->lsoln, first->maxstart, ctx->stream);
                }
            }
        }
        for (auto &th : pool) th.join();
        if (rc != SAT_OK) return rc;
        for (int t = 0; t < nthreads; t++) HIP_TRY(err[(size_t)t]);
        lap(first ? "cell copies, checks and the search queued" : "cell copies");
        int32_t bad = none;
        HIP_TRY(hipStreamSynchronize(ctx->stream));
        HIP_TRY(hipMemcpy(&bad, d_bad.get(), sizeof bad, hipMemcpyDeviceToHost));
        lap(first ? "search + validate on GPU" : "validate on GPU");
        if (bad != none) {
            const int e = bad, n = orders[e];
            for (int i = 0; i < n; i++) {
                const int64_t rowbase = cell_off[e] + (int64_t)i * (i + 1) / 2;
                uint8_t ty = tab_tri[rowbase + i];
                if (ty > 3) return sat_fail(SAT_EINVAL, "entry %d: SSE %d has type code %u (0..3 expected)", e, i, ty);
                for (int j = 0; j < i; j++) {
                    if (tab_tri[rowbase + j] & 0x88)
                        return sat_fail(SAT_EINVAL, "entry %d: tableau code 0x%02x at (%d,%d) has a nibble above 7", e, tab_tri[rowbase + j], i, j);
                    float d = dist_tri[rowbase + j];
                    if (std::isfinite(d) && std::fabs(d) >= 1.0e29f)
                        return sat_fail(SAT_EINVAL, "entry %d: distance %g at (%d,%d) out of range", e, d, i, j);
                }
            }
            return sat_fail(SAT_EINVAL, "entry %d: invalid cell", e);
        }
        return SAT_OK;
    };
    const int rc = body();
    d_bad.reset();
    if (rc != SAT_OK) {
        (void)hipStreamSynchronize(ctx->stream);
        free_db(ctx);
        return rc;
    }
    ctx->h_orders.assign(orders, orders + n_entries);
    return SAT_OK;
}

int sat_db_upload_packed(sat_ctx *ctx, int n_entries, const int32_t *orders,
                         const int64_t *cell_off, const uint8_t *tab_tri,
                         const float *dist_tri, const int64_t *db_ordinal)
{
    return upload_impl(ctx, n_entries, orders, cell_off, tab_tri, dist_tri, db_ordinal, nullptr);
}

int sat_db_upload_search(sat_ctx *ctx, int n_entries, const int32_t *orders,
                         const int64_t *cell_off, const uint8_t *tab_tri,
                         const float *dist_tri, const int64_t *db_ordinal,
                         int lorder, int lsoln, int maxstart)
{
    const FirstSearch first = { lorder, lsoln, maxstart };
    return upload_impl(ctx, n_entries, orders, cell_off, tab_tri, dist_tri, db_ordinal, &first);
}

int sat_db_upload_dense(sat_ctx *ctx, int n_entries, const int32_t *orders,
                        const uint8_t *tabs, const float *dmats, int pitch,
                        const int64_t *db_ordinal)
{
    if (!ctx) return sat_fail(SAT_EINVAL, "null context");
    if (n_entries <= 0 || !orders || !tabs || !dmats || pitch < 1)
        return sat_fail(SAT_EINVAL, "empty database or null array");
    std::vector<int64_t> off(n_entries);
    int64_t cells = 0;
    for (int e = 0; e < n_entries; e++) {
        if (orders[e] < 1 || orders[e] > SAT_MAXDIM || orders[e] > pitch)
            return sat_fail(SAT_EINVAL, "entry %d: order %d outside 1..min(%d, pitch %d)", e, orders[e], SAT_MAXDIM, pitch);
        off[e] = cells;
        cells += (int64_t)orders[e] * (orders[e] + 1) / 2;
    }
    std::vector<uint8_t> tt((size_t)cells);
    std::vector<float> dd((size_t)cells);
    for (int e = 0; e < n_entries; e++) {
        const uint8_t *t = tabs + (size_t)e * pitch * pitch;
        const float *d = dmats + (size_t)e * pitch * pitch;
        int64_t c = off[e];
        for (int i = 0; i < orders[e]; i++)
            for (int j = 0; j <= i; j++, c++) {
                tt[(size_t)c] = t[(size_t)i * pitch + j];
                dd[(size_t)c] = d[(size_t)i * pitch + j];
            }
    }
    return sat_db_upload_packed(ctx, n_entries, orders, off.data(), tt.data(), dd.data(), db_ordinal);
}

int sat_db_size(const sat_ctx *ctx) { return ctx ? ctx->n_entries : 0; }

int sat_queries_set(sat_ctx *ctx, int n_queries, const int32_t *n1s, const uint8_t *qtabs,
                    const float *qdmats, int pitch, const uint8_t *qssetypes, uint32_t first_query_ordinal)
{
    if (!ctx) return sat_fail(SAT_EINVAL, "null context");
    if (n_queries < 1 || !n1s || !qtabs || !qdmats || !qssetypes || pitch < 1)
        return sat_fail(SAT_EINVAL, "bad query batch (n_queries=%d pitch=%d)", n_queries, pitch);
    std::vector<sat_ctx::QueryInfo> infos((size_t)n_queries);
    size_t blob_bytes = 0;
    for (int qi = 0; qi < n_queries; qi++) {
        const int n1 = n1s[qi];
        if (n1 < 1 || n1 > SAT_MAXDIM || n1 > pitch)
            return sat_fail(SAT_EINVAL, "query %d: order %d outside 1..min(%d, pitch %d)", qi, n1, SAT_MAXDIM, pitch);
        auto &q = infos[(size_t)qi];
        q.n1 = n1;
        q.n1p = n1 <= 16 ? 16 : (n1 <= 32 ? 32 : (n1 <= 64 ? 64 : 112));
        q.ordinal = first_query_ordinal + (uint32_t)qi;
        q.blob_off = blob_bytes;
        q.ssemap_off = 0;
        const size_t groups = (size_t)q.n1p / 4 * q.n1p;
        blob_bytes += ((groups * 20 + (size_t)q.n1p + 15) & ~(size_t)15) + (size_t)q.n1p * q.n1p * 8;
    }
    std::vector<uint8_t> blob(blob_bytes, 0);
    for (int qi = 0; qi < n_queries; qi++) {
        const auto &q = infos[(size_t)qi];
        const int n1 = q.n1, n1p = q.n1p, groups = n1p / 4;
        const uint8_t *qtab = qtabs + (size_t)qi * pitch * pitch;
        const float *qdmat = qdmats + (size_t)qi * pitch * pitch;
        const uint8_t *types = qssetypes + (size_t)qi * pitch;
        float4 *qdist = reinterpret_cast<float4 *>(blob.data() + q.blob_off);
        uint32_t *qcode = reinterpret_cast<uint32_t *>(blob.data() + q.blob_off + (size_t)groups * n1p * 16);
        uint8_t *qtypes = blob.data() + q.blob_off + (size_t)groups * n1p * 20;
        uint32_t *qpair = reinterpret_cast<uint32_t *>(blob.data() + q.blob_off + (((size_t)groups * n1p * 20 + (size_t)n1p + 15) & ~(size_t)15));
        for (int i = 0; i < n1p; i++)
            for (int k = 0; k < n1p; k++) {
                float d = SAT_K_QSENT;
                uint32_t code = 0;
                if (k < n1 && i < n1 && k != i) {
                    const float v = qdmat[(size_t)i * pitch + k];
                    if (std::isfinite(v)) d = v;
                    code = qtab[(size_t)i * pitch + k];
                }
                memcpy(&qpair[((size_t)i * n1p + k) * 2], &d, sizeof d);
                qpair[((size_t)i * n1p + k) * 2 + 1] = code;
            }
        for (int i = 0; i < n1; i++) {
            if (types[i] > 3)
                return sat_fail(SAT_EINVAL, "query %d: SSE %d has type code %u (0..3 expected)", qi, i, types[i]);
            qtypes[i] = types[i];
        }
        for (int kw = 0; kw < groups; kw++)
            for (int i = 0; i < n1p; i++) {
                float d[4];
                uint32_t codes = 0;
                for (int sidx = 0; sidx < 4; sidx++) {
                    const int k = 4 * kw + sidx;
                    d[sidx] = SAT_K_QSENT;
                    if (k < n1 && i < n1 && k != i) {
                        const float v = qdmat[(size_t)i * pitch + k];
                        const uint32_t code = qtab[(size_t)i * pitch + k];
                        if (code & 0x88)
                            return sat_fail(SAT_EINVAL, "query %d: tableau code 0x%02x at (%d,%d) has a nibble above 7", qi, code, i, k);
                        if (std::isfinite(v)) {
                            if (std::fabs(v) >= 1.0e29f)
                                return sat_fail(SAT_EINVAL, "query %d: distance %g at (%d,%d) out of range", qi, v, i, k);
                            d[sidx] = v;
                        }
                        codes |= code << (8 * sidx);
                    }
                }
                qdist[(size_t)kw * n1p + i] = float4{ d[0], d[1], d[2], d[3] };
                qcode[(size_t)kw * n1p + i] = codes;
            }
    }
    HIP_TRY(hipSetDevice(ctx->device));
    HIP_TRY(hipStreamSynchronize(ctx->stream));
    ctx->d_qblob.reset();
    ctx->d_qdesc.reset();
    int rc;
    if ((rc = ctx->d_qblob.grow(blob_bytes)) != SAT_OK || (rc = ctx->d_qdesc.grow((size_t)n_queries)) != SAT_OK) return rc;
    HIP_TRY(hipMemcpy(ctx->d_qblob.get(), blob.data(), blob_bytes, hipMemcpyHostToDevice));
    ctx->queries.swap(infos);
    ctx->desc_dirty = true;
    ctx->searched_nq = 0;
    return SAT_OK;
}

int sat_query_set(sat_ctx *ctx, int n1, const uint8_t *qtab, const float *qdmat,
                  int pitch, const uint8_t *qssetypes, uint32_t query_ordinal)
{
    if (!ctx) return sat_fail(SAT_EINVAL, "null context");
    if (n1 < 1 || n1 > SAT_MAXDIM || !qtab || !qdmat || !qssetypes || pitch < n1)
        return sat_fail(SAT_EINVAL, "bad query (n1=%d pitch=%d)", n1, pitch);
    const int32_t n1s[1] = { n1 };
    return sat_queries_set(ctx, 1, n1s, qtab, qdmat, pitch, qssetypes, query_ordinal);
}

int sat_query_count(const sat_ctx *ctx) { return ctx ? (int)ctx->queries.size() : 0; }

int sat_use_stream(sat_ctx *ctx, void *hip_stream)
{
    if (!ctx) return sat_fail(SAT_EINVAL, "null context");
    HIP_TRY(hipSetDevice(ctx->device));
    HIP_TRY(hipStreamSynchronize(ctx->stream));
    ctx->stream = static_cast<hipStream_t>(hip_stream);
    return SAT_OK;
}

int sat_use_own_stream(sat_ctx *ctx)
{
    if (!ctx) return sat_fail(SAT_EINVAL, "null context");
    HIP_TRY(hipSetDevice(ctx->device));
    HIP_TRY(hipStreamSynchronize(ctx->stream));
    ctx->stream = ctx->own_stream;
    return SAT_OK;
}

int sat_search_async(sat_ctx *ctx, int lorder, int lsoln, int maxstart)
{
    if (!ctx) return sat_fail(SAT_EINVAL, "null context");
    return launch_search(ctx, lorder, lsoln, maxstart, ctx->stream);
}

void *sat_device_scores(sat_ctx *ctx) { return ctx ? ctx->d_scores.get() : nullptr; }
void *sat_device_ssemaps(sat_ctx *ctx) { return ctx ? ctx->d_ssemaps.get() : nullptr; }
int sat_query_order(const sat_ctx *ctx) { return (ctx && !ctx->queries.empty()) ? ctx->queries[0].n1 : 0; }

unsigned long long sat_stat_d2h_bytes(const sat_ctx *ctx) { return ctx ? ctx->d2h_bytes : 0ull; }

const char *sat_last_launch_info(const sat_ctx *ctx) { return ctx ? ctx->last_launch_info.c_str() : ""; }

void sat_debug_lds_layout(int m2w, int n1, int n1p, int n2, int chains, int threads, int q_in_lds, int compact,
                          uint32_t out[11])
{
    const int cells = (m2w >> 8) ? ((m2w >> 8) & 3) - 1 : satk::cell_layout(n2);
    m2w &= 0xFF;
    const satk::LdsLayout L = satk::lds_layout(m2w, cells, n2, satk::map_words((n1 + 3) >> 2), n1p, chains, threads,
                                               q_in_lds != 0, compact != 0);
    const uint32_t v[11] = { L.code, L.qdist, L.qcode, L.smap, L.tmask, L.qtypes, L.leader, L.red, L.red_stride, L.items, L.total };
    for (int i = 0; i < 11; i++) out[i] = v[i];
}

int sat_sync(sat_ctx *ctx)
{
    if (!ctx) return sat_fail(SAT_EINVAL, "null context");
    HIP_TRY(hipSetDevice(ctx->device));
    HIP_TRY(hipStreamSynchronize(ctx->stream));
    return SAT_OK;
}

int sat_results(sat_ctx *ctx, int lsoln, int32_t *scores, int32_t *ssemaps)
{
    if (!ctx) return sat_fail(SAT_EINVAL, "null context");
    if (!scores) return sat_fail(SAT_EINVAL, "scores buffer is null");
    if (lsoln && !ssemaps) return sat_fail(SAT_EINVAL, "lsoln set but ssemaps buffer is null");
    if (ctx->n_entries <= 0) return sat_fail(SAT_ESTATE, "no database uploaded");
    if (ctx->queries.empty() || !ctx->d_scores.get() || ctx->searched_nq != ctx->queries.size())
        return sat_fail(SAT_ESTATE, "no search has run since the last database upload / query change");
    HIP_TRY(hipSetDevice(ctx->device));
    HIP_TRY(hipStreamSynchronize(ctx->stream));
    const size_t nq = ctx->queries.size(), N = (size_t)ctx->n_entries;
    HIP_TRY(hipMemcpy(scores, ctx->d_scores.get(), nq * N * sizeof(int32_t), hipMemcpyDeviceToHost));
    ctx->d2h_bytes += nq * N * sizeof(int32_t);
    if (lsoln) {
        if (!ctx->d_ssemaps.get() || !ctx->searched_lsoln) return sat_fail(SAT_ESTATE, "the last search ran without lsoln");
        std::vector<int8_t> packed;
        for (size_t qi = 0; qi < nq; qi++) {
            const auto &q = ctx->queries[qi];
            packed.resize(N * q.n1);
            HIP_TRY(hipMemcpy(packed.data(), ctx->d_ssemaps.get() + q.ssemap_off, packed.size(), hipMemcpyDeviceToHost));
            ctx->d2h_bytes += packed.size();
            int32_t *out = ssemaps + qi * N * SAT_MAXDIM;
            for (size_t e = 0; e < N; e++)
                for (int i = 0; i < q.n1; i++)
                    out[e * SAT_MAXDIM + i] = packed[e * q.n1 + i];
        }
    }
    return SAT_OK;
}

int sat_search(sat_ctx *ctx, int lorder, int lsoln, int maxstart,
               int32_t *scores, int32_t *ssemaps, double *kernel_ms)
{
    if (!ctx) return sat_fail(SAT_EINVAL, "null context");
    if (!scores) return sat_fail(SAT_EINVAL, "scores buffer is null");
    if (lsoln && !ssemaps) return sat_fail(SAT_EINVAL, "lsoln set but ssemaps buffer is null");
    const int rc = timed(ctx, kernel_ms, [&] { return launch_search(ctx, lorder, lsoln, maxstart, ctx->stream); });
    if (rc != SAT_OK) return rc;
    return sat_results(ctx, lsoln, scores, ssemaps);
}

}

int sat_matches_launch(sat_ctx *ctx, int lorder, int maxstart, int max_matches, bool maps)
{
    SatMatchArgs mx;
    int rc = match_args(ctx, max_matches, mx);
    if (rc != SAT_OK) return rc;
    if ((rc = check_ready(ctx, true, maxstart)) != SAT_OK) return rc;
    HIP_TRY(hipSetDevice(ctx->device));
    const size_t rows = ctx->queries.size() * (size_t)ctx->n_entries, slots = rows * (size_t)max_matches;
    if ((rc = ctx->d_mcounts.grow_after(ctx->stream, rows)) != SAT_OK || (rc = ctx->d_mscores.grow_after(ctx->stream, slots)) != SAT_OK ||
        (rc = ctx->d_mrestarts.grow_after(ctx->stream, slots)) != SAT_OK ||
        (rc = ctx->d_mmaps.grow_after(ctx->stream, maps ? slots * SAT_MAXDIM : 0)) != SAT_OK)
        return rc;
    mx.n_entries = ctx->n_entries;
    mx.counts = ctx->d_mcounts.get();
    mx.scores = ctx->d_mscores.get();
    mx.restarts = ctx->d_mrestarts.get();
    mx.maps = ctx->d_mmaps.get();
    rc = launch_search(ctx, lorder, 0, maxstart, ctx->stream, nullptr, &mx);
    if (rc != SAT_OK) return rc;
    const std::string record_info = ctx->last_launch_info;
    ctx->last_launch_info = "record pass: " + record_info;
    if (!maps) return SAT_OK;
    mx.replay = 1;
    rc = launch_search(ctx, lorder, 0, maxstart, ctx->stream, nullptr, &mx);
    if (rc == SAT_OK) ctx->last_launch_info = "record pass: " + record_info + " | replay pass: " + ctx->last_launch_info;
    return rc;
}

int sat_matches_collect(sat_ctx *ctx, int max_matches, int32_t *counts, int32_t *scores, int32_t *restarts,
                        int32_t *ssemaps, size_t total, size_t offset)
{
    HIP_TRY(hipSetDevice(ctx->device));
    HIP_TRY(hipStreamSynchronize(ctx->stream));
    const size_t nq = ctx->queries.size(), N = (size_t)ctx->n_entries, M = (size_t)max_matches;
    std::vector<int32_t> c(nq * N), sc(nq * N * M), rs(nq * N * M);
    std::vector<int8_t> mp(ssemaps ? nq * N * M * SAT_MAXDIM : 0);
    HIP_TRY(hipMemcpy(c.data(), ctx->d_mcounts.get(), c.size() * sizeof(int32_t), hipMemcpyDeviceToHost));
    HIP_TRY(hipMemcpy(sc.data(), ctx->d_mscores.get(), sc.size() * sizeof(int32_t), hipMemcpyDeviceToHost));
    HIP_TRY(hipMemcpy(rs.data(), ctx->d_mrestarts.get(), rs.size() * sizeof(int32_t), hipMemcpyDeviceToHost));
    if (ssemaps) HIP_TRY(hipMemcpy(mp.data(), ctx->d_mmaps.get(), mp.size(), hipMemcpyDeviceToHost));
    ctx->d2h_bytes += (c.size() + sc.size() + rs.size()) * sizeof(int32_t) + mp.size();
    for (size_t qi = 0; qi < nq; qi++) {
        const size_t d = (size_t)ctx->queries[qi].desc;
        const int n1 = ctx->queries[qi].n1;
        for (size_t e = 0; e < N; e++) {
            const size_t src = d * N + e, dst = qi * total + offset + e;
            counts[dst] = c[src];
            for (size_t m = 0; m < M; m++) {
                scores[dst * M + m] = sc[src * M + m];
                restarts[dst * M + m] = rs[src * M + m];
                if (ssemaps) expand_map(mp.data() + (src * M + m) * SAT_MAXDIM, n1, (int)m < c[src], ssemaps + (dst * M + m) * SAT_MAXDIM);
            }
        }
    }
    return SAT_OK;
}

extern "C" {

int sat_search_matches(sat_ctx *ctx, int lorder, int maxstart, int max_matches, int32_t *counts, int32_t *scores,
                       int32_t *restarts, int32_t *ssemaps, double *kernel_ms)
{
    if (!ctx) return sat_fail(SAT_EINVAL, "null context");
    if (!counts || !scores || !restarts) return sat_fail(SAT_EINVAL, "counts / scores / restarts buffer is null");
    const int rc = timed(ctx, kernel_ms, [&] { return sat_matches_launch(ctx, lorder, maxstart, max_matches, ssemaps != nullptr); });
    if (rc != SAT_OK) return rc;
    return sat_matches_collect(ctx, max_matches, counts, scores, restarts, ssemaps, (size_t)ctx->n_entries, 0);
}

int sat_search_pairs(sat_ctx *ctx, int lorder, int lsoln, int maxstart, int npairs, const int32_t *query,
                     const int32_t *entry, int32_t *scores, int32_t *ssemaps, double *kernel_ms)
{
    if (!ctx) return sat_fail(SAT_EINVAL, "null context");
    if (npairs > 0 && !scores) return sat_fail(SAT_EINVAL, "scores buffer is null");
    if (lsoln && npairs > 0 && !ssemaps) return sat_fail(SAT_EINVAL, "lsoln set but ssemaps buffer is null");
    const int rc = timed(ctx, kernel_ms, [&] { return sat_pairs_launch(ctx, lorder, maxstart, lsoln != 0, query, entry, npairs); });
    if (rc != SAT_OK) return rc;
    return sat_pairs_collect(ctx, npairs, scores, lsoln ? ssemaps : nullptr, query);
}

int sat_search_pairs_matches(sat_ctx *ctx, int lorder, int maxstart, int max_matches, int npairs, const int32_t *query,
                             const int32_t *entry, int32_t *counts, int32_t *scores, int32_t *restarts, int32_t *ssemaps,
                             double *kernel_ms)
{
    if (!ctx) return sat_fail(SAT_EINVAL, "null context");
    if (npairs > 0 && (!counts || !scores || !restarts)) return sat_fail(SAT_EINVAL, "counts / scores / restarts buffer is null");
    const int rc = timed(ctx, kernel_ms, [&] {
        return sat_pair_matches_launch(ctx, lorder, maxstart, max_matches, ssemaps != nullptr, query, entry, npairs);
    });
    if (rc != SAT_OK) return rc;
    return sat_pair_matches_collect(ctx, max_matches, npairs, counts, scores, restarts, ssemaps, query);
}

int sat_search_timed(sat_ctx *ctx, int lorder, int lsoln, int maxstart, int repeats,
                     double *total_ms, double *kernel_ms)
{
    if (!ctx) return sat_fail(SAT_EINVAL, "null context");
    if (repeats < 1) return sat_fail(SAT_EINVAL, "repeats must be >= 1");
    HIP_TRY(hipSetDevice(ctx->device));
    HIP_TRY(hipStreamSynchronize(ctx->stream));
    HIP_TRY(hipEventRecord(ctx->ev0, ctx->stream));
    for (int r = 0; r < repeats; r++) {
        int rc = launch_search(ctx, lorder, lsoln, maxstart, ctx->stream);
        if (rc != SAT_OK) return rc;
    }
    HIP_TRY(hipEventRecord(ctx->ev1, ctx->stream));
    HIP_TRY(hipStreamSynchronize(ctx->stream));
    float ms = 0.f;
    HIP_TRY(hipEventElapsedTime(&ms, ctx->ev0, ctx->ev1));
    if (total_ms) *total_ms = ms;
    if (kernel_ms) *kernel_ms = ms;
    return SAT_OK;
}

}
```

### cuda_satabsearch_amd/csrc/sat_sa_body.inc

```
    using namespace satk;
    constexpr int M1W = (N1P + 31) / 32;
    extern __shared__ __align__(16) unsigned char lds_raw[];

    const int nthreads = a.tpe;
    const int wave_wg = __builtin_amdgcn_readfirstlane((int)(threadIdx.x >> 6));
    const int slot = a.epw > 1 ? wave_wg / (nthreads >> 6) : 0;
    const int wlane = (int)(threadIdx.x & 63u);
    const int lane_id = ((wave_wg - slot * (nthreads >> 6)) << 6) | wlane;
    __builtin_assume(lane_id >= 0 && lane_id < 1024);
    const uint32_t lds_base = (uint32_t)slot * a.lds_stride;
    unsigned char *const lds_slot = lds_raw + lds_base;
    constexpr bool FAST = OPT >= 0;
    const int lpc_shift = FAST ? (OPT >> 2) : a.lpc_shift;
    const bool opt_lorder = FAST ? (OPT & 1) != 0 : a.lorder != 0;
    const bool opt_compact = FAST ? (OPT & 1) != 0 : a.compact != 0;
    const int lpc = 1 << lpc_shift;
    const int tid = lane_id >> lpc_shift;
    const int part = lane_id & (lpc - 1);
    const int T = nthreads >> lpc_shift;
    const int list_pos = (int)blockIdx.x * a.epw + slot;
    SatPairItem pit{};
    if constexpr (PAIRS) pit = px.items[min(list_pos, a.n_list - 1)];
    const int e = PAIRS ? pit.entry : a.entry_list[min(list_pos, a.n_list - 1)];
    const SatQuery Q = PAIRS ? a.queries[pit.desc] : a.queries[blockIdx.y];
    const int n1 = Q.n1;
    const int n2 = a.orders[e];
    const int n2p = n2 + 1;
    const int n1w = (n1 + 3) >> 2;
    const int NULLJ = n2;
    const bool lsoln = MATCH ? false : (FAST ? (OPT & 2) != 0 : a.lsoln != 0);
    const bool replay = MATCH && mx.replay != 0;

    int cmp_lpi_q, cmp_wpl_q;
    compaction_shape(n1w, cmp_lpi_q, cmp_wpl_q);
    constexpr int LPI_CT = N1P == 16 ? 1 : (N1P == 32 ? 2 : 0);
    const int cmp_lpi = LPI_CT ? LPI_CT : cmp_lpi_q;
    const int cmp_wpl = WPL > 0 ? WPL : cmp_wpl_q;
    const int cmp_words = cmp_lpi * cmp_wpl;
    constexpr bool SPLIT = CELLS != SAT_CELLS_FULL8;
    const LdsLayout lay = lds_layout(M2W, CELLS, n2, cmp_words, N1P, T, nthreads, QLDS, opt_compact);
    uint2 *Dc = reinterpret_cast<uint2 *>(lds_slot);
    float *distL = reinterpret_cast<float *>(lds_slot);
    uint8_t *codeL = lds_slot + lay.code;
    auto db_row = [&](int j) -> DbRow<CELLS> {
        if constexpr (CELLS == SAT_CELLS_TRI5) return DbRow<SAT_CELLS_TRI5>{ distL, codeL, j };
        else if constexpr (CELLS == SAT_CELLS_FULL5) return DbRow<SAT_CELLS_FULL5>{ distL + __mul24(j, n2p), codeL + __mul24(j, n2p) };
        else return DbRow<SAT_CELLS_FULL8>{ Dc + __mul24(j, n2p) };
    };
    float4 *qdistL = reinterpret_cast<float4 *>(lds_slot + lay.qdist);
    uint32_t *qcodeL = reinterpret_cast<uint32_t *>(lds_slot + lay.qcode);
    uint32_t *smap = reinterpret_cast<uint32_t *>(lds_slot + lay.smap);
    const int TP = T + 1;
    uint32_t *tmask = reinterpret_cast<uint32_t *>(lds_slot + lay.tmask);
    uint32_t *bmap = (lsoln || replay) ? a.bmap_slabs + ((size_t)blockIdx.y * gridDim.x * a.epw + list_pos) * a.bmap_slab_words : nullptr;
    uint8_t *qtypes = lds_slot + lay.qtypes;
    uint32_t *qmask = reinterpret_cast<uint32_t *>(lds_slot + lay.qmask);
    unsigned char *red_b = lds_slot + lay.red;
    auto red_key = [&](int w) -> unsigned long long * { return reinterpret_cast<unsigned long long *>(red_b + (uint32_t)w * lay.red_stride); };
    constexpr int TMS = M2W;
    typedef __attribute__((address_space(3))) uint32_t lds_u32_t;
    typedef __attribute__((address_space(3))) int32_t lds_i32_t;
    const uint32_t items_off = lds_base + lay.items;
    typedef __attribute__((address_space(3))) unsigned long long lds_u64_t;
    lds_u64_t *leader = (lds_u64_t *)(uintptr_t)(lds_base + lay.leader);
    auto beats_leader = [&](int sc, int restart_) -> bool {
        const unsigned long long key = (((unsigned long long)(uint32_t)(sc + 0x40000000)) << 32) | (0xFFFFFFFFu - (uint32_t)restart_);
        if (key <= *leader) return false;
        __hip_atomic_fetch_max(leader, key, __ATOMIC_RELAXED, __HIP_MEMORY_SCOPE_WORKGROUP);
        return true;
    };
    lds_u32_t *items = (lds_u32_t *)(uintptr_t)(uint32_t)(items_off + (uint32_t)(lane_id >> 6) * 256u);
    typedef float f32x4_t __attribute__((ext_vector_type(4)));
    typedef const __attribute__((address_space(1))) f32x4_t *gptr_f4;
    typedef const __attribute__((address_space(1))) uint32_t *gptr_u32;
    const gptr_f4 qdistG = (gptr_f4)(uintptr_t)Q.qdist;
    const gptr_u32 qcodeG = (gptr_u32)(uintptr_t)Q.qcode;
    typedef const __attribute__((address_space(1))) char *gptr_c;
    typedef const __attribute__((address_space(4))) int32_t *cptr_i32;
    const cptr_i32 prowC = (cptr_i32)(uintptr_t)a.prow;
    typedef const __attribute__((address_space(1))) float *gptr_f32;
    const gptr_f32 ptabG = (gptr_f32)(uintptr_t)a.ptab;
    auto load_qdist = [&](uint32_t off16) -> float4 {
        if constexpr (QLDS) return *reinterpret_cast<const float4 *>(reinterpret_cast<const unsigned char *>(qdistL) + off16);
        else {
            const f32x4_t v = *(gptr_f4)((gptr_c)qdistG + off16);
            return float4{ v.x, v.y, v.z, v.w };
        }
    };
    auto load_qcode = [&](uint32_t off4) -> uint32_t {
        if constexpr (QLDS) return *reinterpret_cast<const uint32_t *>(reinterpret_cast<const unsigned char *>(qcodeL) + off4);
        else return *(gptr_u32)((gptr_c)qcodeG + off4);
    };
    typedef const __attribute__((address_space(4))) f32x4_t *cptr_f4;
    typedef const __attribute__((address_space(4))) uint32_t *cptr_u32;
    const cptr_f4 qdistC = (cptr_f4)(uintptr_t)Q.qdist;
    const cptr_u32 qcodeC = (cptr_u32)(uintptr_t)Q.qcode;
    auto load_qdist_uniform = [&](uint32_t idx) -> float4 {
        if constexpr (QLDS) return qdistL[idx];
        else {
            const f32x4_t v = qdistC[idx];
            return float4{ v.x, v.y, v.z, v.w };
        }
    };
    auto load_qcode_uniform = [&](uint32_t idx) -> uint32_t {
        if constexpr (QLDS) return qcodeL[idx];
        else return qcodeC[idx];
    };

    SAT_PHASE_INIT;
    {
        const uint8_t *tt = a.tab_tri + a.cell_off[e];
        const float *dd = a.dist_tri + a.cell_off[e];
        auto clean = [](float v) -> uint32_t { return __float_as_uint(fabsf(v) <= 3.0e38f ? v : SAT_K_DSENT); };
        auto put = [&](int c, uint32_t dist_bits, uint32_t code) {
            if constexpr (SPLIT) {
                distL[c] = __uint_as_float(dist_bits);
                codeL[c] = (uint8_t)code;
            } else {
                Dc[c] = uint2{ dist_bits, code };
            }
        };
        if constexpr (CELLS == SAT_CELLS_TRI5) {
            const int ncell = (n2 * n2p) >> 1;
            typedef float f32x4u_t __attribute__((ext_vector_type(4), aligned(4)));
            typedef uint32_t u32u_t __attribute__((aligned(1)));
            for (int t = lane_id << 2; t + 3 < ncell; t += nthreads << 2) {
                const f32x4u_t v = *reinterpret_cast<const f32x4u_t *>(dd + t);
                const uint32_t c4 = *reinterpret_cast<const u32u_t *>(tt + t);
                *reinterpret_cast<uint4 *>(distL + t) = uint4{ clean(v.x), clean(v.y), clean(v.z), clean(v.w) };
                *reinterpret_cast<uint32_t *>(codeL + t) = c4;
            }
            for (int t = (ncell & ~3) + lane_id; t < ncell; t += nthreads) put(t, clean(dd[t]), tt[t]);
            for (int x = lane_id; x <= n2; x += nthreads) put(ncell + x, __float_as_uint(SAT_K_DSENT), 0u);
        } else {
            const int swave = lane_id >> 6, swaves = nthreads >> 6;
            const int pairs = (n2 + 1) >> 1;
            for (int r = swave; r < pairs; r += swaves) {
                const int rb = n2 - 1 - r;
                for (int x = wlane; x <= n2; x += 64) {
                    const bool first = x <= r;
                    if (!first && rb == r) continue;
                    const int hi = first ? r : rb, lo = first ? x : x - r - 1;
                    const int t = ((hi * (hi + 1)) >> 1) + lo;
                    const uint32_t dist_bits = clean(dd[t]), code = tt[t];
                    put(__mul24(hi, n2p) + lo, dist_bits, code);
                    if (lo != hi) put(__mul24(lo, n2p) + hi, dist_bits, code);
                }
            }
            for (int j = lane_id; j < n2; j += nthreads) put(__mul24(j, n2p) + n2, __float_as_uint(SAT_K_DSENT), 0u);
        }
        if (lane_id < 4 * TMS) tmask[lane_id] = 0u;
        if (lane_id == 0) *reinterpret_cast<unsigned long long *>(lds_slot + lay.leader) = 0ull;
        for (int i = lane_id; i < N1P; i += nthreads) qtypes[i] = Q.qtypes[i];
        if (QLDS) {
            const int groups = cmp_words * N1P;
            for (int c = lane_id; c < groups; c += nthreads) {
                qdistL[c] = Q.qdist[c];
                qcodeL[c] = Q.qcode[c];
            }
        }
    }
    __syncthreads();
    for (int j = lane_id; j < n2; j += nthreads) {
        int t = a.tab_tri[a.cell_off[e] + (int64_t)j * (j + 1) / 2 + j] & 3;
        atomicOr(&tmask[t * TMS + (j >> 5)], 1u << (j & 31));
    }
    __syncthreads();
    if constexpr (M2W == 1) {
        for (int i = lane_id; i < N1P; i += nthreads) qmask[i] = tmask[qtypes[i] & 3];
        __syncthreads();
    }

    uint8_t *smap_b = reinterpret_cast<uint8_t *>(smap);
    uint8_t *bmap_b = reinterpret_cast<uint8_t *>(bmap);
    auto bmap_byte_addr = [&](int k) -> int { return (__mul24(k >> 2, T) + tid) * 4 + (k & 3); };
    const int T4 = TP << 2, tid4 = tid << 2;
    auto map_byte_addr = [&](int k) -> int { return __mul24(k >> 2, T4) + tid4 + (k & 3); };

    auto score_rows = [&]() -> int {
        int total = 0;
        for (int i = 0; i < n1 - 1; i++) {
            const int j = smap_b[map_byte_addr(i)];
            const bool jreal = j != NULLJ;
            const DbRow<CELLS> drow = db_row(jreal ? j : 0);
            int rowsum = 0;
            auto row_group = [&](int kw) {
                const int below = i + 1 - 4 * kw;
                const uint32_t force = below <= 0 ? 0u : (0x04040404u >> (8 * (4 - below)));
                const uint32_t qi = (uint32_t)(kw * N1P + i);
                rowsum = quad_terms(load_qdist(qi << 4), load_qcode(qi << 2), drow, smap[kw * TP + tid], force, rowsum);
            };
            if (lpc == 1) {
                for (int kw = (i + 1) >> 2; kw < n1w; kw++) {
                    const int below = i + 1 - 4 * kw;
                    const uint32_t force = below <= 0 ? 0u : (0x04040404u >> (8 * (4 - below)));
                    const uint32_t qi = (uint32_t)(kw * N1P + i);
                    rowsum = quad_terms(load_qdist_uniform(qi), load_qcode_uniform(qi), drow, smap[kw * TP + tid], force, rowsum);
                }
            } else {
                for (int kw = ((i + 1) >> 2) + part; kw < n1w; kw += lpc) row_group(kw);
            }
            total += jreal ? rowsum : 0;
        }
        return total;
    };

    const uint64_t subseq_lo = (uint64_t)a.ordinal[e];
    int best = SAT_K_NO_SCORE;
    uint32_t best_restart = 0xFFFFFFFFu;
    bool any = false;

    const int cmp_recip = (65536 + cmp_lpi - 1) / cmp_lpi;
    const int per_round = (64 * cmp_recip) >> 16;
    const int sub = __mul24(wlane, cmp_recip) >> 16, kw = wlane - __mul24(sub, cmp_lpi);
    const bool lane_ok = sub < per_round;
    const int tail1_recip = (65536 + n1w - 1) / n1w, tail1_rows = (64 * tail1_recip) >> 16;
    const int tail2_lpi = (n1w + 1) >> 1;
    const int tail2_recip = (65536 + tail2_lpi - 1) / tail2_lpi;
    const int tail2_rows = 2 * tail2_lpi <= cmp_words ? (64 * tail2_recip) >> 16 : 0;
    const uint32_t nullword = (uint32_t)NULLJ * 0x01010101u;
    SAT_PHASE(7);
    SAT_DIAG_PERTURB_INIT;
    size_t mrow = 0;
    uint32_t *mrec = nullptr;
    int r_begin = tid, r_end = a.maxstart;
    if constexpr (PAIRS) {
        r_begin = pit.r0 + tid;
        r_end = pit.r1;
    }
    int rbest = SAT_K_NO_SCORE;
    Bits<M2W> rset = bits_zero<M2W>();
    if constexpr (MATCH) {
        if constexpr (PAIRS) {
            mrow = (size_t)pit.pair;
            mrec = mx.rec_slabs + (size_t)pit.slab * mx.rec_slab_words;
        } else {
            mrow = (size_t)(&a.queries[blockIdx.y] - mx.desc_base) * (size_t)mx.n_entries + (size_t)e;
            mrec = mx.rec_slabs + ((size_t)blockIdx.y * gridDim.x * a.epw + list_pos) * mx.rec_slab_words;
        }
        if (replay) {
            const int cnt = mx.counts[mrow];
            r_begin = tid < cnt ? mx.restarts[mrow * mx.max_matches + tid] : 0;
            r_end = tid < cnt ? r_begin + 1 : 0;
        }
    }
    for (int restart = r_begin; restart < r_end; restart += T) {
        any = true;
        SAT_PHASE(7);
        const uint64_t subseq = subseq_lo | ((uint64_t)(uint32_t)restart << 32);

        Bits<M1W> mapped = bits_zero<M1W>();
        Bits<M2W> occ = bits_zero<M2W>();
        {
            {
                int wa = tid;
                asm volatile("" : "+v"(wa));
                for (int w = 0; w < cmp_words; w++, wa += TP) smap[wa] = nullword;
            }
            int j = 0;
            bool stopped = false;
            for (int i0 = 0; i0 < n1; i0 += 4) {
                if constexpr (N1P > 32)
                    if (__builtin_amdgcn_ballot_w64(!stopped) == 0ull) break;
                uint4 r = philox_block(Q.seed_q, subseq, (uint32_t)(i0 >> 2));
                uint32_t rv[4] = { r.x, r.y, r.z, r.w };
#pragma unroll
                for (int s = 0; s < 4; s++) {
                    const int i = i0 + s;
                    if (i < n1) {
                        if (!stopped && rv[s] < 0x7FFFFFC0u) {
                            Bits<M2W> cand, below = bits_below<M2W>(j);
                            if constexpr (M2W == 1) {
                                cand.w[0] = qmask[i] & ~below.w[0];
                            } else {
                                const int t = qtypes[i];
#pragma unroll
                                for (int w = 0; w < M2W; w++) cand.w[w] = tmask[t * TMS + w] & ~below.w[w];
                            }
                            int jj = bits_lowest<M2W>(cand);
                            if (jj < 0) {
                                stopped = true;
                            } else {
                                smap_b[map_byte_addr(i)] = (uint8_t)jj;
                                bits_set<M1W>(mapped, i);
                                bits_set<M2W>(occ, jj);
                                j = jj + 1;
                            }
                        }
                    }
                }
            }
        }

        SAT_PHASE(10);
        int score = 0;
        constexpr bool FS_PAIRS = N1P > 16 && !SAT_DIAG_FS_ROWS_ONLY;
        bool walk_pairs = FS_PAIRS;
        if constexpr (FS_PAIRS) {
            constexpr int PAIR_COST = 27;
            const int m = bits_count<M1W>(mapped);
            walk_pairs = __builtin_amdgcn_ballot_w64(__mul24(__mul24(m, m - 1), PAIR_COST) > __mul24(__mul24(n1w, n1), 31)) == 0ull;
        }
        if (walk_pairs) {
            typedef uint32_t u32x2_t __attribute__((ext_vector_type(2)));
            typedef const __attribute__((address_space(1))) u32x2_t *gptr_u2;
            const gptr_c qpairG = (gptr_c)(uintptr_t)Q.qpair;
            constexpr bool POP_IMAGES = M2W == 1;
            Bits<M1W> ri = mapped;
            Bits<M2W> rj = occ;
            auto pop = [](auto &b, bool &valid) -> int {
                constexpr int W = sizeof(b.w) / sizeof(b.w[0]);
                valid = bits_any<W>(b);
                const int pos = max(bits_lowest<W>(b), 0);
                bits_drop_lowest<W>(b);
                return pos;
            };
            constexpr bool FS_TEAMS = SAT_FS_TEAMS && M1W == 1 && M2W == 1 && FAST && (OPT == 0 || OPT == 1);
            bool teamed = false;
            if constexpr (FS_TEAMS) teamed = __builtin_amdgcn_ballot_w64(true) == ~0ull;
            if (FS_TEAMS && teamed) {
                const int pl = wlane & 1;
                const uint32_t om = (uint32_t)__shfl_xor((int)mapped.w[0], 1, 64), oo = (uint32_t)__shfl_xor((int)occ.w[0], 1, 64);
                const uint32_t m0 = pl ? om : mapped.w[0], o0 = pl ? oo : occ.w[0];
                const uint32_t m1 = pl ? mapped.w[0] : om, o1 = pl ? occ.w[0] : oo;
                const int c0n = __popc(m0), c1n = __popc(m1);
                const bool big1 = c1n > c0n;
                const uint32_t mb = big1 ? m1 : m0, ob = big1 ? o1 : o0, msm = big1 ? m0 : m1, osm = big1 ? o0 : o1;
                const int rb = max((big1 ? c1n : c0n) - 1, 0), rs = max((big1 ? c0n : c1n) - 1, 0);
                const int dlead = rb - rs, etot = rb + rs;
                uint32_t rm = mb, ro = ob;
                int cur = 0, acc_b = 0, acc_s = 0;
                bool on_small = false;
                for (int e = pl; __builtin_amdgcn_ballot_w64(e < etot) != 0ull; e += 2) {
                    const bool act = e < etot;
                    const int e2 = e - dlead;
                    const bool small = e2 >= 0 && (e2 & 1) != 0;
                    const int len = e2 < 0 ? rb - e : rs - (e2 >> 1);
                    const int a = (small ? rs : rb) - len;
                    if (small && !on_small) { rm = msm; ro = osm; cur = 0; on_small = true; }
#pragma unroll
                    for (int q = 0; q < 2; q++) {
                        const uint32_t go = (act && cur < a) ? 1u : 0u;
                        rm &= rm - go;
                        ro &= ro - go;
                        cur += (int)go;
                    }
                    const int i = act ? __ffs(rm) - 1 : 0, ji = act ? __ffs(ro) - 1 : 0;
                    Bits<1> rk, rl;
                    rk.w[0] = act ? rm & (rm - 1u) : 0u;
                    rl.w[0] = act ? ro & (ro - 1u) : 0u;
                    const DbRow<CELLS> drow = db_row(ji);
                    const uint32_t qrow = (uint32_t)__mul24(i, N1P * 8);
                    int rowsum = 0;
                    while (__builtin_amdgcn_ballot_w64(rk.w[0] != 0u) != 0ull) {
                        int ll[SAT_FS_UNROLL];
                        bool vv[SAT_FS_UNROLL];
                        u32x2_t qcell[SAT_FS_UNROLL];
#pragma unroll
                        for (int u = 0; u < SAT_FS_UNROLL; u++) {
                            bool vl;
                            const int k = pop(rk, vv[u]);
                            ll[u] = pop(rl, vl);
                            qcell[u] = *(gptr_u2)(qpairG + (qrow + ((uint32_t)k << 3)));
                        }
#pragma unroll
                        for (int u = 0; u < SAT_FS_UNROLL; u++) {
                            const uint2 c = db_cell<CELLS>(drow, ll[u]);
                            const int term = pair_term(qcell[u].x, qcell[u].y, c.x, c.y);
                            rowsum += vv[u] ? term : 0;
                        }
                    }
                    acc_s += small ? rowsum : 0;
                    acc_b += small ? 0 : rowsum;
                }
                const int acc0 = big1 ? acc_s : acc_b, acc1 = big1 ? acc_b : acc_s;
                score = (pl ? acc1 : acc0) + __shfl_xor(pl ? acc0 : acc1, 1, 64);
            } else
            while (__builtin_amdgcn_ballot_w64(bits_any<M1W>(ri)) != 0ull) {
                bool ai, aj;
                int i = 0, ji = 0;
                ai = false;
                Bits<M1W> rk = bits_zero<M1W>();
                Bits<M2W> rl = bits_zero<M2W>();
                for (int p = 0; p < lpc; p++) {
                    bool v;
                    const int pos = pop(ri, v);
                    int img = 0;
                    if constexpr (POP_IMAGES) { bool vj; img = pop(rj, vj); }
                    if (p == part) {
                        i = pos;
                        ai = v;
                        ji = img;
                        rk = ri;
                        rl = rj;
                    }
                }
                (void)aj;
                if constexpr (!POP_IMAGES) { ji = smap_b[map_byte_addr(i)]; ji = ai ? ji : 0; }
                const DbRow<CELLS> drow = db_row(ji);
                const uint32_t qrow = (uint32_t)__mul24(i, N1P * 8);
                int rowsum = 0;
                while (__builtin_amdgcn_ballot_w64(bits_any<M1W>(rk)) != 0ull) {
                    int ll[SAT_FS_UNROLL];
                    bool vv[SAT_FS_UNROLL];
                    u32x2_t qcell[SAT_FS_UNROLL];
#pragma unroll
                    for (int u = 0; u < SAT_FS_UNROLL; u++) {
                        const int ku = pop(rk, vv[u]);
                        ll[u] = 0;
                        if constexpr (POP_IMAGES) { bool vl; ll[u] = pop(rl, vl); }
                        if constexpr (!POP_IMAGES) ll[u] = smap_b[map_byte_addr(ku)];
                        qcell[u] = *(gptr_u2)(qpairG + (qrow + ((uint32_t)ku << 3)));
                    }
#pragma unroll
                    for (int u = 0; u < SAT_FS_UNROLL; u++) {
                        const uint2 c = db_cell<CELLS>(drow, ll[u]);
                        const int term = pair_term(qcell[u].x, qcell[u].y, c.x, c.y);
                        rowsum += vv[u] ? term : 0;
                    }
                }
                score += rowsum;
            }
        } else {
            score = score_rows();
        }
        if (lpc >= 2) score += __shfl_xor(score, 1, 64);
        if (lpc == 4) score += __shfl_xor(score, 2, 64);
        const int best_before = best;
        if (score > best) {
            best = score;
            if (lsoln && beats_leader(score, restart))
                for (int w = 0; w < n1w; w++) bmap[w * T + tid] = smap[w * TP + tid];
        }
        if constexpr (MATCH) {
            rbest = score;
            rset = occ;
            if (replay && part == 0)
                for (int w = 0; w < n1w; w++) bmap[w * T + tid] = smap[w * TP + tid];
        }

        SAT_PHASE(6);
        uint4 blk = uint4{ 0u, 0u, 0u, 0u };
        for (int iter = 0; iter < SAT_K_MAXITER; iter++) {
            const int rowoff = prowC[2 * iter], rowmax = prowC[2 * iter + 1];
            constexpr bool ROW_IN_LANES = N1P >= 32 && M2W == 1 && (OPT < 0 || (OPT & 1) != 0);
            float rowv = 0.0f;
            if constexpr (ROW_IN_LANES)
                rowv = *(gptr_f32)((gptr_c)ptabG + (((uint32_t)rowoff + (uint32_t)min(wlane, rowmax + 2)) << 2));
            if ((iter & 1) == 0) {
                blk = philox_block(Q.seed_q, subseq, (uint32_t)(SAT_K_STEP_BLOCK0 + (iter >> 1)));
            } else {
                blk.x = blk.z;
                blk.y = blk.w;
            }
            const uint32_t word_a = blk.x, word_b = blk.y;
            SAT_DIAG_PERTURB_STEP;

            const int ssei = scaled_index16(word_a >> 16, n1, n1 - 1);

            int oldj;
            Bits<M2W> cand;
            if (M2W == 1 && opt_lorder) {
                int p;
                bool none;
                highest_mapped_upto(mapped, ssei, p, none);
                const int A = smap_b[map_byte_addr(p)];
                SAT_DIAG_DUP_MAPBYTE(&smap_b[map_byte_addr(p)]);
                oldj = p == ssei ? A : NULLJ;
                const uint32_t above = 0xFFFFFFFEu << (A & 31);
                const uint32_t y = occ.w[0] & above;
                const uint32_t gap = (y - 1u) & ~y & above;
                const bool empty = none || (y == 0u && ssei != n1 - 1);
                cand.w[0] = empty ? 0u : (qmask[ssei] & gap);
            } else if (M2W == 2 && FAST && opt_lorder) {
                int p;
                bool none;
                highest_mapped_upto(mapped, ssei, p, none);
                const int t = qtypes[ssei];
                const int A = smap_b[map_byte_addr(p)];
                oldj = p == ssei ? A : NULLJ;
                const unsigned long long occ64 = (unsigned long long)occ.w[0] | ((unsigned long long)occ.w[1] << 32);
                const unsigned long long above = (~1ull) << (A & 63);
                const unsigned long long y = occ64 & above;
                const unsigned long long gap = (y - 1ull) & ~y & above;
                const unsigned long long tm = *reinterpret_cast<const unsigned long long *>(&tmask[t * TMS]);
                const bool empty = none || (y == 0ull && ssei != n1 - 1);
                const unsigned long long c64 = empty ? 0ull : (tm & gap);
                cand.w[0] = (uint32_t)c64;
                cand.w[M2W - 1] = (uint32_t)(c64 >> 32);
            } else if (M2W == 4 && FAST && opt_lorder) {
                int p;
                bool none;
                highest_mapped_upto(mapped, ssei, p, none);
                const int t = qtypes[ssei];
                const int A = smap_b[map_byte_addr(p)];
                oldj = p == ssei ? A : NULLJ;
                const unsigned long long occ_lo = (unsigned long long)occ.w[0] | ((unsigned long long)occ.w[1] << 32),
                                         occ_hi = (unsigned long long)occ.w[2] | ((unsigned long long)occ.w[3] << 32);
                const unsigned long long base = (~1ull) << (A & 63);
                const bool a_hi = A >= 64;
                const unsigned long long above_lo = a_hi ? 0ull : base, above_hi = a_hi ? base : ~0ull;
                const unsigned long long y_lo = occ_lo & above_lo, y_hi = occ_hi & above_hi;
                const unsigned long long gap_lo = (y_lo - 1ull) & ~y_lo & above_lo;
                const unsigned long long gap_hi = (y_hi - (y_lo == 0ull ? 1ull : 0ull)) & ~y_hi & above_hi;
                const unsigned long long *tm = reinterpret_cast<const unsigned long long *>(&tmask[t * TMS]);
                const bool empty = none || ((y_lo | y_hi) == 0ull && ssei != n1 - 1);
                const unsigned long long c_lo = empty ? 0ull : (tm[0] & gap_lo), c_hi = empty ? 0ull : (tm[1] & gap_hi);
                cand.w[0] = (uint32_t)c_lo;
                cand.w[1 % M2W] = (uint32_t)(c_lo >> 32);
                cand.w[2 % M2W] = (uint32_t)c_hi;
                cand.w[3 % M2W] = (uint32_t)(c_hi >> 32);
            } else {
                oldj = smap_b[map_byte_addr(ssei)];
                int startj = 0, endj = n2;
                if (opt_lorder) {
                    Bits<M1W> upto = bits_below<M1W>(ssei + 1), lowpart, highpart;
#pragma unroll
                    for (int w = 0; w < M1W; w++) {
                        lowpart.w[w] = mapped.w[w] & upto.w[w];
                        highpart.w[w] = mapped.w[w] & ~upto.w[w];
                    }
                    const int p = bits_highest<M1W>(lowpart);
                    const int q = bits_lowest<M1W>(highpart);
                    const int pimg = smap_b[map_byte_addr(p < 0 ? 0 : p)];
                    const int qimg = smap_b[map_byte_addr(q < 0 ? 0 : q)];
                    startj = p < 0 ? n2 : pimg;
                    endj = (ssei == n1 - 1) ? n2 : (q < 0 ? -1 : qimg);
                }
                const int t = qtypes[ssei];
                Bits<M2W> lo = bits_below<M2W>(startj), hi = bits_below<M2W>(endj);
#pragma unroll
                for (int w = 0; w < M2W; w++)
                    cand.w[w] = tmask[t * TMS + w] & ~occ.w[w] & hi.w[w] & ~lo.w[w];
            }
            const int cnt = bits_count<M2W>(cand);
            const int pick = scaled_index16(word_a & 0xFFFFu, cnt, max(cnt - 1, 0));
            int sel;
            if (M2W == 1 && opt_lorder) {
                uint32_t c = cand.w[0];
                int left = pick;
                {
                    const uint32_t go = left > 0 ? 1u : 0u;
                    c &= c - go;
                    left -= (int)go;
                }
                while (__builtin_amdgcn_ballot_w64(left > 0) != 0ull) {
                    const uint32_t go = left > 0 ? 1u : 0u;
                    c &= c - go;
                    left -= (int)go;
                }
                sel = __ffs(c) - 1;
            } else if (M2W == 2 && FAST && opt_lorder && __builtin_amdgcn_ballot_w64(pick > 2) == 0ull) {
                unsigned long long c = (unsigned long long)cand.w[0] | ((unsigned long long)cand.w[M2W - 1] << 32);
                int left = pick;
#pragma unroll
                for (int q = 0; q < 2; q++) {
                    const unsigned long long go = left > 0 ? 1ull : 0ull;
                    c &= c - go;
                    left -= (int)go;
                }
                sel = __ffsll((long long)c) - 1;
            } else if (M2W == 4 && FAST && opt_lorder && __builtin_amdgcn_ballot_w64(pick > 2) == 0ull) {
                unsigned long long c_lo = (unsigned long long)cand.w[0] | ((unsigned long long)cand.w[1 % M2W] << 32),
                                   c_hi = (unsigned long long)cand.w[2 % M2W] | ((unsigned long long)cand.w[3 % M2W] << 32);
                int left = pick;
#pragma unroll
                for (int q = 0; q < 2; q++) {
                    const bool go = left > 0, in_lo = c_lo != 0ull;
                    c_lo &= c_lo - ((go && in_lo) ? 1ull : 0ull);
                    c_hi &= c_hi - ((go && !in_lo) ? 1ull : 0ull);
                    left -= go ? 1 : 0;
                }
                sel = c_lo != 0ull ? __ffsll((long long)c_lo) - 1 : 63 + __ffsll((long long)c_hi);
            } else {
                sel = bits_select<M2W>(cand, pick);
            }
            const bool nreal = cnt != 0;
            const int newj = nreal ? sel : NULLJ;

            SAT_PHASE(0);
            int delta;
            {
                const bool oreal = oldj != NULLJ;
                const bool lists = part == 0;
                const int nitems = lists ? (int)oreal + (int)nreal : 0;
                const unsigned long long bo = __builtin_amdgcn_ballot_w64(lists && oreal),
                                         bn = __builtin_amdgcn_ballot_w64(lists && nreal);
                const unsigned long long m1 = bo | bn, m2 = bo & bn;
                const int total_items = __popcll(m1) + __popcll(m2);
                if (opt_compact && __builtin_amdgcn_ballot_w64(true) == ~0ull && total_items <= 64) {
                    const int pre = __builtin_amdgcn_mbcnt_hi((uint32_t)(m1 >> 32), __builtin_amdgcn_mbcnt_lo((uint32_t)m1, 0)) +
                                    __builtin_amdgcn_mbcnt_hi((uint32_t)(m2 >> 32), __builtin_amdgcn_mbcnt_lo((uint32_t)m2, 0));
                    const uint32_t item1 = (uint32_t)(oreal ? oldj : newj) | ((uint32_t)ssei << 8) | ((uint32_t)tid << 16) |
                                           (oreal ? 1u << 24 : 0u);
                    const uint32_t item2 = (uint32_t)newj | ((uint32_t)ssei << 8) | ((uint32_t)tid << 16);
                    if (nitems >= 1) items[pre] = item1;
                    if (nitems == 2) items[pre + 1] = item2;
                    __builtin_amdgcn_fence(__ATOMIC_RELEASE, "wavefront");
                    __builtin_amdgcn_wave_barrier();
                    __builtin_amdgcn_fence(__ATOMIC_ACQUIRE, "wavefront");
                    SAT_PHASE(1);
                    auto one_round = [&](auto wtag, int first, int lpi, int rsub, int rkw, bool rlane_ok) {
                        constexpr int W = decltype(wtag)::value;
                        const int idx = first + rsub;
                        bool ok = rlane_ok && idx < total_items;
                        int v = 0;
                        if (ok) {
                            const uint32_t it = items[idx];
                            const int row = it & 0xFF, si = (it >> 8) & 0xFF, owner = (it >> 16) & 0xFF;
                            const DbRow<CELLS> drow = db_row(row);
                            float4 qd[W];
                            uint32_t qc[W], wd[W];
                            const uint32_t qoff4 = (uint32_t)(rkw * N1P + si) << 2, qoff16 = qoff4 << 2;
#pragma unroll
                            for (int u = 0; u < W; u++) {
                                const int kwu = rkw + u * lpi;
                                wd[u] = smap[kwu * TP + owner];
                                SAT_DIAG_DUP_MAPWORD(&smap[kwu * TP + owner]);
                                qd[u] = load_qdist(qoff16 + (uint32_t)(u * lpi * N1P * 16));
                                qc[u] = load_qcode(qoff4 + (uint32_t)(u * lpi * N1P * 4));
                            }
#pragma unroll
                            for (int u = 0; u < W; u++) v = quad_terms(qd[u], qc[u], drow, wd[u], 0u, v);
                            v = (it >> 24) ? -v : v;
                        }
                        if ((lpi & 3) == 0) {
                            v += __builtin_amdgcn_update_dpp(0, v, 0xB1, 0xF, 0xF, true);
                            v += __builtin_amdgcn_update_dpp(0, v, 0x4E, 0xF, 0xF, true);
                            ok = ok && (rkw & 3) == 0;
                        }
                        if (ok)
                            __hip_atomic_fetch_add((lds_i32_t *)(items + idx), v, __ATOMIC_RELAXED, __HIP_MEMORY_SCOPE_WAVEFRONT);
                        if (ok) SAT_DIAG_DUP_ATOMIC((lds_i32_t *)(items + idx));
                    };
                    auto main_round = [&](int first) {
                        if constexpr (WPL > 0) one_round(std::integral_constant<int, WPL>{}, first, cmp_lpi, sub, kw, lane_ok);
                        else switch (cmp_wpl) {
                        case 1: one_round(std::integral_constant<int, 1>{}, first, cmp_lpi, sub, kw, lane_ok); break;
                        case 2: one_round(std::integral_constant<int, 2>{}, first, cmp_lpi, sub, kw, lane_ok); break;
                        case 3: one_round(std::integral_constant<int, 3>{}, first, cmp_lpi, sub, kw, lane_ok); break;
                        default: one_round(std::integral_constant<int, 4>{}, first, cmp_lpi, sub, kw, lane_ok); break;
                        }
                    };
                    int first = 0;
                    for (; total_items - first > per_round; first += per_round) main_round(first);
                    const int rest = total_items - first;
                    if (rest > 0) {
                        if (cmp_wpl > 1 && rest <= tail1_rows) {
                            int l = wlane;
                            asm volatile("" : "+v"(l));
                            const int rsub = __mul24(l, tail1_recip) >> 16;
                            one_round(std::integral_constant<int, 1>{}, first, n1w, rsub, l - __mul24(rsub, n1w), rsub < tail1_rows);
                        } else if (cmp_wpl > 2 && rest <= tail2_rows) {
                            int l = wlane;
                            asm volatile("" : "+v"(l));
                            const int rsub = __mul24(l, tail2_recip) >> 16;
                            one_round(std::integral_constant<int, 2>{}, first, tail2_lpi, rsub, l - __mul24(rsub, tail2_lpi), rsub < tail2_rows);
                        } else {
                            main_round(first);
                        }
                    }
                    __builtin_amdgcn_fence(__ATOMIC_RELEASE, "wavefront");
                    __builtin_amdgcn_wave_barrier();
                    __builtin_amdgcn_fence(__ATOMIC_ACQUIRE, "wavefront");
                    SAT_PHASE(2);
                    delta = 0;
                    if (nitems >= 1) delta = (int)(items[pre] - item1);
                    if (nitems == 2) delta += (int)(items[pre + 1] - item2);
                    if (lpc > 1) delta = __shfl(delta, wlane & ~(lpc - 1), 64);
                } else {
                    const DbRow<CELLS> orow = db_row(oreal ? oldj : 0), nrow = db_row(nreal ? newj : 0);
                    int sum_new = 0, sum_old = 0;
                    auto move_group = [&](int kw) {
                        const uint32_t word = smap[kw * TP + tid];
                        const uint32_t qi = (uint32_t)(kw * N1P + ssei);
                        const float4 qd = load_qdist(qi << 4);
                        const uint32_t qc = load_qcode(qi << 2);
                        sum_new = quad_terms(qd, qc, nrow, word, 0u, sum_new);
                        sum_old = quad_terms(qd, qc, orow, word, 0u, sum_old);
                    };
                    if (lpc == 1) for (int kw = 0; kw < n1w; kw++) move_group(kw);
                    else for (int kw = part; kw < n1w; kw += lpc) move_group(kw);
                    delta = (nreal ? sum_new : 0) - (oreal ? sum_old : 0);
                    if (lpc >= 2) delta += __shfl_xor(delta, 1, 64);
                    if (lpc == 4) delta += __shfl_xor(delta, 2, 64);
                }
            }
            const int newscore = score + delta;
            SAT_PHASE(3);
            SAT_DIAG_SELFCHECK_STEP;

            if (lsoln && newscore > best) {
                if (beats_leader(newscore, restart)) {
                    for (int w = 0; w < n1w; w++) bmap[w * T + tid] = smap[w * TP + tid];
                    bmap_b[bmap_byte_addr(ssei)] = (uint8_t)newj;
                }
            }
            best = max(best, newscore);
            if constexpr (MATCH) {
                if (newscore > rbest) {
                    rbest = newscore;
                    rset = occ;
                    if (oldj != NULLJ) bits_clear<M2W>(rset, oldj);
                    if (nreal) bits_set<M2W>(rset, newj);
                    if (replay && part == 0) {
                        for (int w = 0; w < n1w; w++) bmap[w * T + tid] = smap[w * TP + tid];
                        bmap_b[bmap_byte_addr(ssei)] = (uint8_t)newj;
                    }
                }
            }

            SAT_PHASE(4);
            const float u = draw32(word_b);
            const uint32_t nd = (uint32_t)min(max(1 - delta, 0), rowmax + 2);
            float p;
            if (ROW_IN_LANES && __builtin_amdgcn_ballot_w64(true) == ~0ull && __builtin_amdgcn_ballot_w64(nd >= 64u) == 0ull)
                p = __int_as_float(__builtin_amdgcn_ds_bpermute((int)(nd << 2), __float_as_int(rowv)));
            else
                p = *(gptr_f32)((gptr_c)ptabG + (((uint32_t)rowoff + nd) << 2));
            const bool accept = p > u;
            if (accept) smap_b[map_byte_addr(ssei)] = (uint8_t)newj;
            score = accept ? newscore : score;
            {
                const bool oreal_ = oldj != NULLJ;
                if constexpr (M2W == 1) {
                    const uint32_t oldbit = (accept && oreal_) ? (1u << (oldj & 31)) : 0u;
                    const uint32_t newbit = (accept && nreal) ? (1u << (newj & 31)) : 0u;
                    occ.w[0] = (occ.w[0] & ~oldbit) | newbit;
                } else {
                    const uint32_t oldbit = (accept && oreal_) ? (1u << (oldj & 31)) : 0u;
                    const uint32_t newbit = (accept && nreal) ? (1u << (newj & 31)) : 0u;
                    const int ow = oldj >> 5, nw = newj >> 5;
#pragma unroll
                    for (int w = 0; w < M2W; w++) occ.w[w] ^= (ow == w ? oldbit : 0u) ^ (nw == w ? newbit : 0u);
                }
                if constexpr (M1W == 1) {
                    const uint32_t ibit = 1u << ssei;
                    const uint32_t setbit = (accept && nreal) ? ibit : 0u, clrbit = (accept && !nreal) ? ibit : 0u;
                    mapped.w[0] = (mapped.w[0] & ~clrbit) | setbit;
                } else {
                    const uint32_t ibit = (accept && oreal_ != nreal) ? (1u << (ssei & 31)) : 0u;
                    const int iw = ssei >> 5;
#pragma unroll
                    for (int w = 0; w < M1W; w++) mapped.w[w] ^= iw == w ? ibit : 0u;
                }
            }
            SAT_PHASE(5);
        }
        if (best > best_before) best_restart = (uint32_t)restart;
        if constexpr (MATCH) {
            if (!replay && part == 0) {
                mrec[restart] = (uint32_t)rbest;
#pragma unroll
                for (int w = 0; w < M2W; w++) mrec[(size_t)(w + 1) * a.maxstart + restart] = rset.w[w];
            }
        }
    }
    SAT_PHASE_FLUSH;
    SAT_DIAG_PERTURB_END;

    if constexpr (MATCH) {
        if (replay) {
            if (any && part == 0) {
                int8_t *out = mx.maps + (mrow * mx.max_matches + tid) * (size_t)mx.map_pitch;
                for (int i = 0; i < n1; i++) {
                    const int j = bmap_b[bmap_byte_addr(i)];
                    out[i] = (int8_t)(j == NULLJ ? -1 : j);
                }
            }
            return;
        }
    }

    unsigned long long key = any
        ? (((unsigned long long)(uint32_t)(best + 0x40000000)) << 32) | (0xFFFFFFFFu - best_restart)
        : 0ull;
#pragma unroll
    for (int off = 32; off > 0; off >>= 1) {
        unsigned long long other = __shfl_xor(key, off, 64);
        key = other > key ? other : key;
    }
    const int wave = lane_id >> 6, nwaves = (nthreads + 63) >> 6;
    if (wlane == 0) *red_key(wave) = key;
    __syncthreads();
    unsigned long long win = *red_key(0);
    for (int w = 1; w < nwaves; w++) win = *red_key(w) > win ? *red_key(w) : win;

    const uint32_t win_restart = 0xFFFFFFFFu - (uint32_t)(win & 0xFFFFFFFFu);
    if constexpr (PAIRS) {
        if (lane_id == 0 && !lsoln) atomicMax(px.keys + pit.pair, win);
    } else {
        if (lane_id == 0) Q.scores[e] = (int)(uint32_t)(win >> 32) - 0x40000000;
    }
    if (lsoln && any && part == 0 && best_restart == win_restart &&
        ((((unsigned long long)(uint32_t)(best + 0x40000000)) << 32) | (0xFFFFFFFFu - best_restart)) == win) {
        int8_t *out = PAIRS ? px.maps + (size_t)pit.pair * SAT_K_MAXDIM : Q.ssemaps + (size_t)e * n1;
        for (int i = 0; i < n1; i++) {
            int j = bmap_b[bmap_byte_addr(i)];
            out[i] = (int8_t)(j == NULLJ ? -1 : j);
        }
    }

    if constexpr (MATCH && !PAIRS) {
        uint32_t *uni = tmask;
        const int M = mx.max_matches;
        int m = 0;
        auto take = [&](unsigned long long k) {
            const uint32_t r = 0xFFFFFFFFu - (uint32_t)(k & 0xFFFFFFFFu);
            if (lane_id == 0) {
                mx.scores[mrow * M + m] = (int)(uint32_t)(k >> 32) - 0x40000000;
                mx.restarts[mrow * M + m] = (int)r;
            }
            if (part == 0 && (int)(r % (uint32_t)T) == tid) {
#pragma unroll
                for (int w = 0; w < M2W; w++) {
                    const uint32_t s = mrec[(size_t)(w + 1) * a.maxstart + r];
                    uni[w] = m == 0 ? s : (uni[w] | s);
                }
            }
            m++;
        };
        take(win);
        bool done = false;
        for (int round = 1; round < M; round++) {
            __syncthreads();
            unsigned long long k = 0ull;
            if (!done && part == 0) {
                for (int r = tid; r < a.maxstart; r += T) {
                    const int s = (int)mrec[r];
                    uint32_t hit = 0u;
#pragma unroll
                    for (int w = 0; w < M2W; w++) hit |= mrec[(size_t)(w + 1) * a.maxstart + r] & uni[w];
                    const unsigned long long rk = (((unsigned long long)(uint32_t)(s + 0x40000000)) << 32) | (0xFFFFFFFFu - (uint32_t)r);
                    k = (s > 0 && hit == 0u && rk > k) ? rk : k;
                }
            }
#pragma unroll
            for (int off = 32; off > 0; off >>= 1) {
                unsigned long long other = __shfl_xor(k, off, 64);
                k = other > k ? other : k;
            }
            if (wlane == 0) *red_key(wave) = k;
            __syncthreads();
            unsigned long long cur = *red_key(0);
            for (int w = 1; w < nwaves; w++) cur = *red_key(w) > cur ? *red_key(w) : cur;
            if (done || cur == 0ull) done = true;
            else take(cur);
        }
        if (lane_id == 0) {
            mx.counts[mrow] = m;
            for (int x = m; x < M; x++) {
                mx.scores[mrow * M + x] = 0;
                mx.restarts[mrow * M + x] = -1;
            }
        }
    }
```

### cuda_satabsearch_amd/csrc/sat_sa_kernel.hpp

```cpp
#pragma once

#include <hip/hip_runtime.h>
#include <type_traits>
#include <stdint.h>

#ifdef SAT_DIAG
#include "diag/sat_diag.hpp"
#endif
#ifndef SAT_DIAG_ARGS
#define SAT_DIAG_ARGS
#endif
#ifndef SAT_PHASE_INIT
#define SAT_PHASE_INIT
#define SAT_PHASE(k)
#define SAT_PHASE_FLUSH
#endif
#ifndef SAT_DIAG_FS_ROWS_ONLY
#define SAT_DIAG_FS_ROWS_ONLY 0
#endif
#ifndef SAT_DIAG_DUP_CELLS
#define SAT_DIAG_DUP_CELLS(row, l0, l1, l2, l3)
#endif
#ifndef SAT_DIAG_DUP_MAPWORD
#define SAT_DIAG_DUP_MAPWORD(p)
#endif
#ifndef SAT_DIAG_DUP_ATOMIC
#define SAT_DIAG_DUP_ATOMIC(p)
#endif
#ifndef SAT_DIAG_DUP_MAPBYTE
#define SAT_DIAG_DUP_MAPBYTE(p)
#endif
#ifndef SAT_DIAG_PERTURB_INIT
#define SAT_DIAG_PERTURB_INIT
#define SAT_DIAG_PERTURB_STEP
#define SAT_DIAG_PERTURB_END
#endif
#ifndef SAT_DIAG_SELFCHECK_STEP
#define SAT_DIAG_SELFCHECK_STEP
#endif

#define SAT_CELLS_FULL8 0
#define SAT_CELLS_FULL5 1
#define SAT_CELLS_TRI5  2
#ifndef SAT_FAST_WAVES
#define SAT_FAST_WAVES 6
#endif
#ifndef SAT_FS_TEAMS
#define SAT_FS_TEAMS 1
#endif
#define SAT_K_MAXITER 100
#define SAT_K_MAXDIM 111
#define SAT_FS_UNROLL 2
#define SAT_K_STEP_BLOCK0 32
#define SAT_K_EPS 1.1e-7
#define SAT_K_NO_SCORE (-99999)
#define SAT_K_QSENT 1.0e30f
#define SAT_K_DSENT (-1.0e30f)

struct SatQuery {
    const float4   *qdist;
    const uint32_t *qcode;
    const uint8_t  *qtypes;
    const uint2    *qpair;
    int32_t         n1;
    uint32_t        pad_;
    uint64_t        seed_q;
    int32_t        *scores;
    int8_t         *ssemaps;
};

struct SatKernelArgs {
    const int32_t  *orders;
    const int64_t  *cell_off;
    const uint8_t  *tab_tri;
    const float    *dist_tri;
    const uint32_t *ordinal;
    const int32_t  *entry_list;
    int32_t         n_list;
    int32_t         epw, tpe;
    uint32_t        lds_stride;
    const SatQuery *queries;
    int32_t         lorder, lsoln, maxstart;
    int32_t         lpc_shift;
    int32_t         compact;
    uint32_t       *bmap_slabs;
    uint32_t        bmap_slab_words;
    const float    *ptab;
    const int32_t  *prow;
    SAT_DIAG_ARGS
};

struct SatMatchArgs {
    const SatQuery *desc_base;
    int32_t         n_entries;
    int32_t         max_matches;
    int32_t         replay;
    int32_t         map_pitch;
    uint32_t       *rec_slabs;
    uint32_t        rec_slab_words;
    uint32_t        pad_;
    int32_t        *counts;
    int32_t        *scores;
    int32_t        *restarts;
    int8_t         *maps;
};

struct SatPairItem {
    int32_t pair;
    int32_t desc;
    int32_t entry;
    int32_t r0, r1;
    int32_t slab;
    int32_t pad_[2];
};
struct SatPairArgs {
    const SatPairItem   *items;
    unsigned long long  *keys;
    int8_t              *maps;
};

namespace satk {

template <int W> struct Bits { uint32_t w[W]; };

template <int W> __device__ __forceinline__ Bits<W> bits_zero()
{
    Bits<W> b;
#pragma unroll
    for (int i = 0; i < W; i++) b.w[i] = 0u;
    return b;
}
template <int W> __device__ __forceinline__ Bits<W> bits_below(int pos)
{
    Bits<W> b;
    if constexpr (W == 1) {
        const int s = 32 - min(max(pos, 0), 32);
        const int h = s >> 1;
        b.w[0] = (0xFFFFFFFFu >> h) >> (s - h);
        return b;
    }
    const int wi = pos >> 5;
    const uint32_t part = (1u << (pos & 31)) - 1u;
#pragma unroll
    for (int i = 0; i < W; i++) b.w[i] = i < wi ? 0xFFFFFFFFu : (i == wi ? part : 0u);
    return b;
}
template <int W> __device__ __forceinline__ void bits_set(Bits<W> &b, int pos)
{
#pragma unroll
    for (int i = 0; i < W; i++) b.w[i] |= ((pos >> 5) == i) ? (1u << (pos & 31)) : 0u;
}
template <int W> __device__ __forceinline__ void bits_clear(Bits<W> &b, int pos)
{
#pragma unroll
    for (int i = 0; i < W; i++) b.w[i] &= ~(((pos >> 5) == i) ? (1u << (pos & 31)) : 0u);
}
template <int W> __device__ __forceinline__ int bits_count(const Bits<W> &b)
{
    int c = 0;
#pragma unroll
    for (int i = 0; i < W; i++) c += __popc(b.w[i]);
    return c;
}
template <int W> __device__ __forceinline__ bool bits_any(const Bits<W> &b)
{
    uint32_t o = 0u;
#pragma unroll
    for (int i = 0; i < W; i++) o |= b.w[i];
    return o != 0u;
}
template <int W> __device__ __forceinline__ void bits_drop_lowest(Bits<W> &b)
{
    bool done = false;
#pragma unroll
    for (int i = 0; i < W; i++) {
        const bool here = !done && b.w[i] != 0u;
        b.w[i] = here ? b.w[i] & (b.w[i] - 1u) : b.w[i];
        done = done || here;
    }
}
template <int W> __device__ __forceinline__ int bits_lowest(const Bits<W> &b)
{
    int r = -1;
#pragma unroll
    for (int i = W - 1; i >= 0; i--) r = b.w[i] ? 32 * i + (__ffs(b.w[i]) - 1) : r;
    return r;
}
template <int W> __device__ __forceinline__ int bits_highest(const Bits<W> &b)
{
    int r = -1;
#pragma unroll
    for (int i = 0; i < W; i++) r = b.w[i] ? 32 * i + (31 - __clz(b.w[i])) : r;
    return r;
}
__device__ __forceinline__ int word_select(uint32_t v, int r)
{
    uint32_t a = v - ((v >> 1) & 0x55555555u);
    uint32_t b = (a & 0x33333333u) + ((a >> 2) & 0x33333333u);
    uint32_t c = (b + (b >> 4)) & 0x0F0F0F0Fu;
    uint32_t d = (c + (c >> 8)) & 0x00FF00FFu;
    int pos = 0;
    int t = (int)(d & 0xFFu);
    if (r >= t) { pos = 16; r -= t; }
    t = (int)((c >> pos) & 0xFu);
    if (r >= t) { pos += 8; r -= t; }
    t = (int)((b >> pos) & 0x7u);
    if (r >= t) { pos += 4; r -= t; }
    t = (int)((a >> pos) & 0x3u);
    if (r >= t) { pos += 2; r -= t; }
    t = (int)((v >> pos) & 0x1u);
    if (r >= t) { pos += 1; }
    return pos;
}
template <int W> __device__ __forceinline__ int bits_select(const Bits<W> &b, int r)
{
    uint32_t word = b.w[0];
    int base = 0, rr = r;
    bool found = false;
#pragma unroll
    for (int i = 0; i < W; i++) {
        const int c = __popc(b.w[i]);
        const bool here = !found && r < c;
        word = here ? b.w[i] : word;
        base = here ? 32 * i : base;
        rr = here ? r : rr;
        found = found || here;
        r -= c;
    }
    return found ? base + word_select(word, rr) : 0;
}

template <int W> __device__ __forceinline__ void highest_mapped_upto(const Bits<W> &mapped, int upto, int &p, bool &none)
{
    if constexpr (W == 1) {
        const uint32_t low = mapped.w[0] & (0xFFFFFFFFu >> (31 - upto));
        p = 31 ^ __builtin_clz(low | 1u);
        none = low == 0u;
    } else if constexpr (W == 2) {
        const unsigned long long m = (unsigned long long)mapped.w[0] | ((unsigned long long)mapped.w[1] << 32);
        const unsigned long long low = m & (~0ull >> (63 - upto));
        p = 63 ^ __builtin_clzll(low | 1ull);
        none = low == 0ull;
    } else {
        Bits<W> lowpart, below = bits_below<W>(upto + 1);
#pragma unroll
        for (int w = 0; w < W; w++) lowpart.w[w] = mapped.w[w] & below.w[w];
        p = bits_highest<W>(lowpart);
        none = p < 0;
        p = none ? 0 : p;
    }
}

template <int CELLS> struct DbRow;
template <> struct DbRow<SAT_CELLS_FULL8> { const uint2 *cells; };
template <> struct DbRow<SAT_CELLS_FULL5> { const float *dist; const uint8_t *code; };
template <> struct DbRow<SAT_CELLS_TRI5> { const float *dist; const uint8_t *code; int j; };
__host__ __device__ inline int cell_layout(int n2max) { return n2max <= 32 ? SAT_CELLS_FULL8 : (n2max <= 48 ? SAT_CELLS_FULL5 : SAT_CELLS_TRI5); }
__host__ __device__ inline int set_words(int n2) { return n2 <= 32 ? 1 : (n2 <= 64 ? 2 : 4); }
__device__ __forceinline__ int tri_index(int j, int l)
{
    const int mx = max(j, l), mn = min(j, l);
    return (int)((__umul24((uint32_t)mx, (uint32_t)mx) + (uint32_t)mx) >> 1) + mn;
}
__host__ __device__ inline uint32_t tri_cells(int n2) { return (uint32_t)(n2 + 1) * (uint32_t)(n2 + 2) / 2u; }
template <int CELLS> __device__ __forceinline__ uint2 db_cell(const DbRow<CELLS> row, int l)
{
    if constexpr (CELLS == SAT_CELLS_FULL8) return row.cells[l];
    else if constexpr (CELLS == SAT_CELLS_FULL5) return uint2{ __float_as_uint(row.dist[l]), row.code[l] };
    else { const int c = tri_index(row.j, l); return uint2{ __float_as_uint(row.dist[c]), row.code[c] }; }
}

template <int CELLS>
__device__ __forceinline__ int quad_terms(const float4 qd, const uint32_t qc, const DbRow<CELLS> row,
                                          const uint32_t word, const uint32_t force, const int acc)
{
    const uint32_t l0 = word & 0xFFu, l1 = (word >> 8) & 0xFFu, l2 = (word >> 16) & 0xFFu, l3 = word >> 24;
    SAT_DIAG_DUP_CELLS(row, l0, l1, l2, l3);
    const uint2 d0 = db_cell<CELLS>(row, (int)l0), d1 = db_cell<CELLS>(row, (int)l1), d2 = db_cell<CELLS>(row, (int)l2),
                d3 = db_cell<CELLS>(row, (int)l3);
    const float t0 = 4.0f - fabsf(qd.x - __uint_as_float(d0.x));
    const float t1 = 4.0f - fabsf(qd.y - __uint_as_float(d1.x));
    const float t2 = 4.0f - fabsf(qd.z - __uint_as_float(d2.x));
    const float t3 = 4.0f - fabsf(qd.w - __uint_as_float(d3.x));
    const uint32_t far = __builtin_amdgcn_perm(__float_as_uint(t1), __float_as_uint(t0), 0x0C0C0703u) |
                         __builtin_amdgcn_perm(__float_as_uint(t3), __float_as_uint(t2), 0x07030C0Cu);
    const uint32_t x = __builtin_amdgcn_perm(d1.y, d0.y, 0x0C0C0400u) ^
                       __builtin_amdgcn_perm(d3.y, d2.y, 0x04000C0Cu) ^ qc;
    const uint32_t z = (x + 0x77777777u) & 0x88888888u;
    uint32_t sel = __builtin_amdgcn_bitop3_b32(z >> 3, z >> 6, 0x03030303u, 0xA8);
    sel = __builtin_amdgcn_bitop3_b32(far >> 5, 0x04040404u, sel, 0xEA);
    sel |= force;
    const uint32_t terms = __builtin_amdgcn_perm(0u, 0xFE010102u, sel);
    return __builtin_amdgcn_sdot4((int)terms, 0x01010101, acc, false);
}

__device__ __forceinline__ int pair_term(const uint32_t qd_bits, const uint32_t qc, const uint32_t dd_bits, const uint32_t dc)
{
    const float t = 4.0f - fabsf(__uint_as_float(qd_bits) - __uint_as_float(dd_bits));
    const uint32_t z = ((qc ^ dc) + 0x77u) & 0x88u;
    uint32_t sel = __builtin_amdgcn_bitop3_b32(z >> 3, z >> 6, 0x3u, 0xA8);
    sel = __builtin_amdgcn_bitop3_b32(__float_as_uint(t) >> 29, 0x4u, sel, 0xEA);
    const uint32_t terms = __builtin_amdgcn_perm(0u, 0xFE010102u, sel);
    return (int)(int8_t)(terms & 0xFFu);
}

__device__ __forceinline__ uint4 philox_block(uint64_t seed_q, uint64_t subsequence, uint32_t block)
{
    uint32_t c0 = block, c1 = 0u, c2 = (uint32_t)subsequence, c3 = (uint32_t)(subsequence >> 32);
    uint32_t k0 = (uint32_t)seed_q, k1 = (uint32_t)(seed_q >> 32);
#pragma unroll
    for (int r = 0; r < 10; r++) {
        const uint64_t p0 = (uint64_t)0xD2511F53u * c0, p1 = (uint64_t)0xCD9E8D57u * c2;
        uint32_t n0, n2;
        if (r < 3) {
            n0 = (uint32_t)(p1 >> 32) ^ c1 ^ k0;
            n2 = (uint32_t)(p0 >> 32) ^ c3 ^ k1;
        } else {
            n0 = __builtin_amdgcn_bitop3_b32((uint32_t)(p1 >> 32), c1, k0, 0x96);
            n2 = __builtin_amdgcn_bitop3_b32((uint32_t)(p0 >> 32), c3, k1, 0x96);
        }
        c1 = (uint32_t)p1;
        c3 = (uint32_t)p0;
        c0 = n0;
        c2 = n2;
        k0 += 0x9E3779B9u;
        k1 += 0xBB67AE85u;
    }
    return uint4{ c0, c1, c2, c3 };
}
__device__ __forceinline__ float draw32(uint32_t v)
{
    return (float)v + 1.0f;
}
__device__ __forceinline__ float to_uniform(uint32_t v)
{
    return draw32(v) * 2.3283064365386963e-10f;
}
__device__ __forceinline__ int scaled_index16(uint32_t v16, int n, int nm1)
{
    return (int)(__umul24(v16, (uint32_t)n) + (uint32_t)nm1) >> 16;
}

__host__ __device__ inline void compaction_shape(int n1w, int &lpi, int &wpl)
{
    lpi = (n1w + 3) >> 2;
    wpl = lpi > 0 ? (n1w + lpi - 1) / lpi : 1;
    if (lpi < 1) lpi = 1;
}
__host__ __device__ inline int map_words(int n1w)
{
    int lpi, wpl;
    compaction_shape(n1w, lpi, wpl);
    return lpi * wpl;
}

struct LdsLayout {
    uint32_t code;
    uint32_t qdist;
    uint32_t qcode;
    uint32_t smap;
    uint32_t tmask;
    uint32_t qtypes;
    uint32_t qmask;
    uint32_t leader;
    uint32_t red;
    uint32_t red_stride;
    uint32_t items;
    uint32_t total;
};
__host__ __device__ inline LdsLayout lds_layout(int m2w, int cells, int n2, int words, int n1p, int chains, int threads,
                                                 bool q_in_lds, bool compact)
{
    LdsLayout L;
    const bool split = cells != SAT_CELLS_FULL8;
    uint32_t dcells = (uint32_t)n2 * (uint32_t)(n2 + 1);
    uint32_t off;
    if (split) {
        if (cells == SAT_CELLS_TRI5) dcells = tri_cells(n2);
        dcells = (dcells + 3u) & ~3u;
        L.code = dcells * 4u;
        off = L.code + ((dcells + 15u) & ~15u);
    } else {
        dcells = (dcells + 1u) & ~1u;
        L.code = 0u;
        off = dcells * 8u;
    }
    L.qdist = off;
    if (q_in_lds) off += (uint32_t)words * (uint32_t)n1p * 16u;
    L.qcode = off;
    if (q_in_lds) off += (uint32_t)words * (uint32_t)n1p * 4u;
    L.smap = off;
    off += (((uint32_t)words * (uint32_t)(chains + 1) + 1u) & ~1u) * 4u;
    L.tmask = off;
    off += 4u * (uint32_t)m2w * 4u;
    L.qtypes = off;
    off += ((uint32_t)n1p + 15u) & ~15u;
    L.qmask = off;
    if (m2w == 1) off += (uint32_t)n1p * 4u;
    off = (off + 7u) & ~7u;
    L.leader = off;
    off += 8u;
    L.red = off;
    L.red_stride = compact ? 256u : 8u;
    if (!compact) off += 16u * 8u;
    L.items = off;
    if (compact) off += (uint32_t)((threads + 63) / 64) * 64u * 4u;
    L.total = off;
    return L;
}

__host__ __device__ inline size_t lds_bytes(int n1, int n1p, int n2, int chains, int threads, bool lsoln, bool q_in_lds,
                                             bool compact)
{
    (void)lsoln;
    return lds_layout(set_words(n2), cell_layout(n2), n2, map_words((n1 + 3) >> 2), n1p, chains, threads, q_in_lds, compact).total;
}

}


template <int N1P, int M2W, bool QLDS, int OPT, int WPL, int CELLS>
__global__ void __launch_bounds__(1024) __attribute__((amdgpu_waves_per_eu((OPT < 0 || OPT >= 4) ? 4 : SAT_FAST_WAVES)))
sat_sa_kernel(const SatKernelArgs a)
{
    constexpr bool MATCH = false, PAIRS = false;
    const SatMatchArgs mx{};
    const SatPairArgs px{};
#include "sat_sa_body.inc"
}

template <int N1P, int M2W, bool QLDS, int CELLS>
__global__ void __launch_bounds__(1024) __attribute__((amdgpu_waves_per_eu(4)))
sat_sa_match_kernel(const SatKernelArgs a, const SatMatchArgs mx)
{
    constexpr bool MATCH = true, PAIRS = false;
    constexpr int OPT = -1, WPL = 0;
    const SatPairArgs px{};
#include "sat_sa_body.inc"
}

template <int N1P, int M2W, bool QLDS, int OPT, int CELLS>
__global__ void __launch_bounds__(1024) __attribute__((amdgpu_waves_per_eu((OPT < 0 || OPT >= 4) ? 4 : SAT_FAST_WAVES)))
sat_sa_pair_kernel(const SatKernelArgs a, const SatPairArgs px)
{
    constexpr bool MATCH = false, PAIRS = true;
    constexpr int WPL = 0;
    const SatMatchArgs mx{};
#include "sat_sa_body.inc"
}

template <int N1P, int M2W, bool QLDS, int CELLS>
__global__ void __launch_bounds__(1024) __attribute__((amdgpu_waves_per_eu(4)))
sat_sa_pair_match_kernel(const SatKernelArgs a, const SatPairArgs px, const SatMatchArgs mx)
{
    constexpr bool MATCH = true, PAIRS = true;
    constexpr int OPT = -1, WPL = 0;
#include "sat_sa_body.inc"
}
```

### include/satabsearch.h

```cpp
#ifndef SATABSEARCH_H
#define SATABSEARCH_H

#include <stdint.h>

#ifdef __cplusplus
extern "C" {
#endif

#define SAT_ABI_VERSION   1
#define SAT_MAXDIM        111
#define SAT_MAXITER       100
#define SAT_DEFAULT_SEED  1234
#define SAT_MAX_MATCHES   8

#define SAT_OK          0
#define SAT_EINVAL     -1
#define SAT_ENODEVICE  -2
#define SAT_ENOMEM     -3
#define SAT_EDEVICE    -4
#define SAT_ESTATE     -5

typedef struct sat_ctx sat_ctx;

const char *sat_last_error(void);

int sat_abi_version(void);

int sat_device_count(void);

sat_ctx *sat_ctx_create(int device, uint64_t seed);

void sat_ctx_destroy(sat_ctx *ctx);

int sat_db_upload_packed(sat_ctx *ctx, int n_entries, const int32_t *orders,
                         const int64_t *cell_off, const uint8_t *tab_tri,
                         const float *dist_tri, const int64_t *db_ordinal);

int sat_db_upload_search(sat_ctx *ctx, int n_entries, const int32_t *orders,
                         const int64_t *cell_off, const uint8_t *tab_tri,
                         const float *dist_tri, const int64_t *db_ordinal,
                         int lorder, int lsoln, int maxstart);

int sat_db_upload_dense(sat_ctx *ctx, int n_entries, const int32_t *orders,
                        const uint8_t *tabs, const float *dmats, int pitch,
                        const int64_t *db_ordinal);

int sat_db_size(const sat_ctx *ctx);

int sat_query_set(sat_ctx *ctx, int n1, const uint8_t *qtab, const float *qdmat,
                  int pitch, const uint8_t *qssetypes, uint32_t query_ordinal);

int sat_queries_set(sat_ctx *ctx, int n_queries, const int32_t *n1s, const uint8_t *qtabs,
                    const float *qdmats, int pitch, const uint8_t *qssetypes,
                    uint32_t first_query_ordinal);

int sat_query_count(const sat_ctx *ctx);

int sat_search(sat_ctx *ctx, int lorder, int lsoln, int maxstart,
               int32_t *scores, int32_t *ssemaps, double *kernel_ms);

int sat_search_matches(sat_ctx *ctx, int lorder, int maxstart, int max_matches,
                       int32_t *counts, int32_t *scores, int32_t *restarts, int32_t *ssemaps,
                       double *kernel_ms);
int sat_search_pairs(sat_ctx *ctx, int lorder, int lsoln, int maxstart, int npairs, const int32_t *query,
                     const int32_t *entry, int32_t *scores, int32_t *ssemaps, double *kernel_ms);

int sat_search_pairs_matches(sat_ctx *ctx, int lorder, int maxstart, int max_matches, int npairs, const int32_t *query,
                             const int32_t *entry, int32_t *counts, int32_t *scores, int32_t *restarts, int32_t *ssemaps,
                             double *kernel_ms);

int sat_use_stream(sat_ctx *ctx, void *hip_stream);
int sat_use_own_stream(sat_ctx *ctx);

int sat_search_async(sat_ctx *ctx, int lorder, int lsoln, int maxstart);
void *sat_device_scores(sat_ctx *ctx);
void *sat_device_ssemaps(sat_ctx *ctx);
int sat_query_order(const sat_ctx *ctx);

int sat_sync(sat_ctx *ctx);

int sat_results(sat_ctx *ctx, int lsoln, int32_t *scores, int32_t *ssemaps);

int sat_topk(sat_ctx *ctx, int query, int k, int32_t *entry_index, int32_t *scores_out);

typedef struct sat_hit {
    int32_t entry;
    int32_t score;
    double  norm2;
    double  zscore;
    double  pvalue;
} sat_hit;

int sat_topk_hits(sat_ctx *ctx, int k, sat_hit *hits, int32_t *ssemaps);

int sat_hits_cutoff(sat_ctx *ctx, double max_pvalue, int max_rows, int32_t *counts, int capacity, sat_hit *hits,
                    int32_t *ssemaps);

int sat_search_refine(sat_ctx *ctx, int lorder, int lsoln, int maxstart, int candidates, int refine_maxstart,
                      int k, sat_hit *hits, int32_t *ssemaps, int32_t *first_scores);


unsigned long long sat_stat_d2h_bytes(const sat_ctx *ctx);

const char *sat_last_launch_info(const sat_ctx *ctx);

void sat_debug_lds_layout(int m2w, int n1, int n1p, int n2, int chains, int threads, int q_in_lds, int compact,
                          uint32_t out[11]);

typedef struct sat_multi sat_multi;
sat_multi *sat_multi_create(int ndev, const int *devices, uint64_t seed);
void sat_multi_destroy(sat_multi *m);
int sat_multi_device_count(const sat_multi *m);
const char *sat_multi_gather_kind(const sat_multi *m);
int sat_multi_db_upload_packed(sat_multi *m, int n_entries, const int32_t *orders, const int64_t *cell_off,
                               const uint8_t *tab_tri, const float *dist_tri);
int sat_multi_shards(const sat_multi *m, int32_t *begin);
int sat_multi_queries_set(sat_multi *m, int n_queries, const int32_t *n1s, const uint8_t *qtabs,
                          const float *qdmats, int pitch, const uint8_t *qssetypes, uint32_t first_query_ordinal);
int sat_multi_search(sat_multi *m, int lorder, int lsoln, int maxstart, int32_t *scores, int32_t *ssemaps,
                     double *wall_ms);
int sat_multi_search_topk(sat_multi *m, int lorder, int lsoln, int maxstart, int k, sat_hit *hits,
                          int32_t *ssemaps, double *wall_ms);
int sat_multi_search_matches(sat_multi *m, int lorder, int maxstart, int max_matches, int32_t *counts,
                             int32_t *scores, int32_t *restarts, int32_t *ssemaps, double *wall_ms);
int sat_multi_search_refine(sat_multi *m, int lorder, int lsoln, int maxstart, int candidates, int refine_maxstart,
                            int k, sat_hit *hits, int32_t *ssemaps, int32_t *first_scores, double *wall_ms,
                            double *stage2_ms);
int sat_multi_search_pairs_matches(sat_multi *m, int lorder, int maxstart, int max_matches, int npairs, const int32_t *query,
                                   const int32_t *entry, int32_t *counts, int32_t *scores, int32_t *restarts,
                                   int32_t *ssemaps, double *wall_ms);
int sat_multi_search_cutoff(sat_multi *m, int lorder, int lsoln, int maxstart, double max_pvalue, int max_rows,
                            int32_t *counts, int capacity, sat_hit *hits, int32_t *ssemaps, double *wall_ms);
int sat_multi_hits_cutoff(sat_multi *m, double max_pvalue, int max_rows, int32_t *counts, int capacity, sat_hit *hits,
                          int32_t *ssemaps);
unsigned long long sat_multi_stat_d2h_bytes(const sat_multi *m);

int sat_search_timed(sat_ctx *ctx, int lorder, int lsoln, int maxstart, int repeats,
                     double *total_ms, double *kernel_ms);

#ifdef __cplusplus
}
#endif
#endif
```

Baseline: 11.71 million.

## Store FULL8 map bytes prescaled by 8 for direct LDS cell addressing

For the FULL8 cell layout, solution-map bytes now hold the image index shifted left by 3, with a dedicated unmatched bit. DB rows are laid out at a power-of-two stride and the LDS slot is aligned to 256 bytes, so each cell address becomes a single bitop3 of the map byte with the row base instead of extract, multiply and add. The unmatched bit also feeds straight into the score term selector, replacing the old sentinel column. The cost is possibly more LDS per slot from the power-of-two row padding and extra alignment, which can lower occupancy, plus decode overhead wherever images are read back.

Result: slower. 7.622 million (-34.9%).

```diff
diff --git a/cuda_satabsearch_amd/_native.py b/cuda_satabsearch_amd/_native.py
--- a/cuda_satabsearch_amd/_native.py
+++ b/cuda_satabsearch_amd/_native.py
@@ -13,7 +13,7 @@
     "sat_db_upload_packed", "sat_db_upload_search", "sat_db_upload_dense", "sat_db_size", "sat_query_set", "sat_search",
     "sat_search_async", "sat_device_scores", "sat_device_ssemaps", "sat_query_order", "sat_sync",
     "sat_search_timed", "sat_use_stream", "sat_use_own_stream", "sat_results", "sat_queries_set", "sat_query_count", "sat_topk",
-    "sat_topk_hits", "sat_stat_d2h_bytes", "sat_debug_lds_layout", "sat_last_launch_info",
+    "sat_topk_hits", "sat_stat_d2h_bytes", "sat_debug_lds_layout", "sat_debug_slot_stride", "sat_last_launch_info",
     "sat_multi_create", "sat_multi_destroy", "sat_multi_device_count", "sat_multi_gather_kind", "sat_multi_db_upload_packed",
     "sat_multi_shards", "sat_multi_queries_set", "sat_multi_search", "sat_multi_search_topk", "sat_multi_stat_d2h_bytes",
     "sat_search_matches", "sat_multi_search_matches",
@@ -86,6 +86,9 @@
         lib.sat_last_launch_info.restype = C.c_char_p
         lib.sat_debug_lds_layout.argtypes = [C.c_int] * 8 + [C.c_void_p]
         lib.sat_debug_lds_layout.restype = None
+        if hasattr(lib, "sat_debug_slot_stride"):
+            lib.sat_debug_slot_stride.argtypes = [C.c_uint32, C.c_int]
+            lib.sat_debug_slot_stride.restype = C.c_uint32
         lib.sat_multi_create.restype = C.c_void_p
         lib.sat_multi_create.argtypes = [C.c_int, C.c_void_p, C.c_uint64]
         lib.sat_multi_destroy.argtypes = [C.c_void_p]
diff --git a/cuda_satabsearch_amd/csrc/diag/sat_diag.hpp b/cuda_satabsearch_amd/csrc/diag/sat_diag.hpp
--- a/cuda_satabsearch_amd/csrc/diag/sat_diag.hpp
+++ b/cuda_satabsearch_amd/csrc/diag/sat_diag.hpp
@@ -14,11 +14,11 @@
 
 #ifdef SAT_DIAG_DUP
 #if SAT_DIAG_DUP == 1
-#define SAT_DIAG_DUP_CELLS(row, l0, l1, l2, l3) do { if constexpr (CELLS == SAT_CELLS_FULL8) {                                            \
+#define SAT_DIAG_DUP_CELLS(a0, a1, a2, a3) do {                                                                          \
         typedef const volatile __attribute__((address_space(3))) unsigned long long *lds_vu64;                          \
-        const unsigned long long dup0 = *(lds_vu64)&(row).cells[l0], dup1 = *(lds_vu64)&(row).cells[l1],                  \
-                                 dup2 = *(lds_vu64)&(row).cells[l2], dup3 = *(lds_vu64)&(row).cells[l3];                  \
-        asm volatile("" : : "v"(dup0), "v"(dup1), "v"(dup2), "v"(dup3)); } } while (0)
+        const unsigned long long dup0 = *(lds_vu64)(uintptr_t)(a0), dup1 = *(lds_vu64)(uintptr_t)(a1),                    \
+                                 dup2 = *(lds_vu64)(uintptr_t)(a2), dup3 = *(lds_vu64)(uintptr_t)(a3);                    \
+        asm volatile("" : : "v"(dup0), "v"(dup1), "v"(dup2), "v"(dup3)); } while (0)
 #elif SAT_DIAG_DUP == 2
 #define SAT_DIAG_DUP_MAPWORD(p) (void)*(const volatile __attribute__((address_space(3))) uint32_t *)(p)
 #elif SAT_DIAG_DUP == 3
@@ -64,7 +64,7 @@
 #ifdef SAT_DIAG_SELFCHECK
 #define SAT_DIAG_SELFCHECK_STEP do {                                                                                     \
         const uint8_t keep_ = smap_b[map_byte_addr(ssei)];                                                               \
-        smap_b[map_byte_addr(ssei)] = (uint8_t)newj;                                                                     \
+        smap_b[map_byte_addr(ssei)] = (uint8_t)newb;                                                                     \
         int chk_ = score_rows();                                                                                         \
         if (lpc >= 2) chk_ += __shfl_xor(chk_, 1, 64);                                                                   \
         if (lpc == 4) chk_ += __shfl_xor(chk_, 2, 64);                                                                   \
diff --git a/cuda_satabsearch_amd/csrc/sat_capi.hip b/cuda_satabsearch_amd/csrc/sat_capi.hip
--- a/cuda_satabsearch_amd/csrc/sat_capi.hip
+++ b/cuda_satabsearch_amd/csrc/sat_capi.hip
@@ -383,6 +383,12 @@
     return SAT_OK;
 }
 
+size_t slot_stride(size_t lds, int n2max)
+{
+    const size_t align = satk::prescaled_maps(satk::cell_layout(n2max)) ? 256 : 16;
+    return (lds + align - 1) & ~(align - 1);
+}
+
 struct SaLaunch { WgShape w; SaKernel k; int epw; size_t lds_stride, lds_launch; SatKernelArgs args; };
 
 int prepare_sa(sat_ctx *ctx, int mode, int lorder, int lsoln, int maxstart, int plan_starts, int c, int n2max, long long work,
@@ -396,7 +402,7 @@
     const int opt = special ? (lorder ? 1 : 0) | (lsoln ? 2 : 0) | (w.lpc_shift << 2) : -1;
     out.k = pick_sa_kernel(mode, n1p, m2w, satk::cell_layout(n2max), w.qlds, opt, ctx->class_wpl[c]);
     if (!out.k.fn) return sat_fail(SAT_EDEVICE, "no kernel variant for n1p=%d m2w=%d", n1p, m2w);
-    out.lds_stride = (w.lds + 15) & ~(size_t)15;
+    out.lds_stride = slot_stride(w.lds, n2max);
     out.epw = 1;
     if ((rc = launch_setup(ctx, out.k.fn, w.threads, out.lds_stride, work, pack ? &out.epw : nullptr)) != SAT_OK) return rc;
     out.lds_launch = out.epw > 1 ? (size_t)out.epw * out.lds_stride : w.lds;
@@ -1441,6 +1447,8 @@
     for (int i = 0; i < 11; i++) out[i] = v[i];
 }
 
+uint32_t sat_debug_slot_stride(uint32_t lds_bytes, int n2max) { return (uint32_t)slot_stride(lds_bytes, n2max); }
+
 int sat_sync(sat_ctx *ctx)
 {
     if (!ctx) return sat_fail(SAT_EINVAL, "null context");
diff --git a/cuda_satabsearch_amd/csrc/sat_sa_body.inc b/cuda_satabsearch_amd/csrc/sat_sa_body.inc
--- a/cuda_satabsearch_amd/csrc/sat_sa_body.inc
+++ b/cuda_satabsearch_amd/csrc/sat_sa_body.inc
@@ -38,6 +38,11 @@
     const int cmp_wpl = WPL > 0 ? WPL : cmp_wpl_q;
     const int cmp_words = cmp_lpi * cmp_wpl;
     constexpr bool SPLIT = CELLS != SAT_CELLS_FULL8;
+    constexpr bool PS = prescaled_maps(CELLS);
+    const uint32_t NULLB = PS ? SAT_K_UNMATCHED8 : (uint32_t)NULLJ;
+    auto map_image = [&](uint32_t b) -> int { return PS ? (int)(b >> 3) : (int)b; };
+    auto map_unmatched = [&](uint32_t b) -> bool { return PS ? (b & SAT_K_UNMATCHED8) != 0u : (int)b == NULLJ; };
+    const int cshift = PS ? full8_row_shift(n2) : 0, row_shift = cshift + 3;
     const LdsLayout lay = lds_layout(M2W, CELLS, n2, cmp_words, N1P, T, nthreads, QLDS, opt_compact);
     uint2 *Dc = reinterpret_cast<uint2 *>(lds_slot);
     float *distL = reinterpret_cast<float *>(lds_slot);
@@ -45,7 +50,7 @@
     auto db_row = [&](int j) -> DbRow<CELLS> {
         if constexpr (CELLS == SAT_CELLS_TRI5) return DbRow<SAT_CELLS_TRI5>{ distL, codeL, j };
         else if constexpr (CELLS == SAT_CELLS_FULL5) return DbRow<SAT_CELLS_FULL5>{ distL + __mul24(j, n2p), codeL + __mul24(j, n2p) };
-        else return DbRow<SAT_CELLS_FULL8>{ Dc + __mul24(j, n2p) };
+        else return DbRow<SAT_CELLS_FULL8>{ lds_base + ((uint32_t)j << row_shift) };
     };
     float4 *qdistL = reinterpret_cast<float4 *>(lds_slot + lay.qdist);
     uint32_t *qcodeL = reinterpret_cast<uint32_t *>(lds_slot + lay.qcode);
@@ -135,6 +140,7 @@
         } else {
             const int swave = lane_id >> 6, swaves = nthreads >> 6;
             const int pairs = (n2 + 1) >> 1;
+            auto cell_at = [&](int row, int col) -> int { return PS ? (row << cshift) + col : __mul24(row, n2p) + col; };
             for (int r = swave; r < pairs; r += swaves) {
                 const int rb = n2 - 1 - r;
                 for (int x = wlane; x <= n2; x += 64) {
@@ -143,11 +149,12 @@
                     const int hi = first ? r : rb, lo = first ? x : x - r - 1;
                     const int t = ((hi * (hi + 1)) >> 1) + lo;
                     const uint32_t dist_bits = clean(dd[t]), code = tt[t];
-                    put(__mul24(hi, n2p) + lo, dist_bits, code);
-                    if (lo != hi) put(__mul24(lo, n2p) + hi, dist_bits, code);
-                }
-            }
-            for (int j = lane_id; j < n2; j += nthreads) put(__mul24(j, n2p) + n2, __float_as_uint(SAT_K_DSENT), 0u);
+                    put(cell_at(hi, lo), dist_bits, code);
+                    if (lo != hi) put(cell_at(lo, hi), dist_bits, code);
+                }
+            }
+            if constexpr (!PS)
+                for (int j = lane_id; j < n2; j += nthreads) put(__mul24(j, n2p) + n2, __float_as_uint(SAT_K_DSENT), 0u);
         }
         if (lane_id < 4 * TMS) tmask[lane_id] = 0u;
         if (lane_id == 0) *reinterpret_cast<unsigned long long *>(lds_slot + lay.leader) = 0ull;
@@ -180,9 +187,9 @@
     auto score_rows = [&]() -> int {
         int total = 0;
         for (int i = 0; i < n1 - 1; i++) {
-            const int j = smap_b[map_byte_addr(i)];
-            const bool jreal = j != NULLJ;
-            const DbRow<CELLS> drow = db_row(jreal ? j : 0);
+            const uint32_t jb = smap_b[map_byte_addr(i)];
+            const bool jreal = !map_unmatched(jb);
+            const DbRow<CELLS> drow = db_row(jreal ? map_image(jb) : 0);
             int rowsum = 0;
             auto row_group = [&](int kw) {
                 const int below = i + 1 - 4 * kw;
@@ -218,7 +225,7 @@
     const int tail2_lpi = (n1w + 1) >> 1;
     const int tail2_recip = (65536 + tail2_lpi - 1) / tail2_lpi;
     const int tail2_rows = 2 * tail2_lpi <= cmp_words ? (64 * tail2_recip) >> 16 : 0;
-    const uint32_t nullword = (uint32_t)NULLJ * 0x01010101u;
+    const uint32_t nullword = NULLB * 0x01010101u;
     SAT_PHASE(7);
     SAT_DIAG_PERTURB_INIT;
     size_t mrow = 0;
@@ -281,7 +288,7 @@
                             if (jj < 0) {
                                 stopped = true;
                             } else {
-                                smap_b[map_byte_addr(i)] = (uint8_t)jj;
+                                smap_b[map_byte_addr(i)] = (uint8_t)(PS ? jj << 3 : jj);
                                 bits_set<M1W>(mapped, i);
                                 bits_set<M2W>(occ, jj);
                                 j = jj + 1;
@@ -396,7 +403,7 @@
                     }
                 }
                 (void)aj;
-                if constexpr (!POP_IMAGES) { ji = smap_b[map_byte_addr(i)]; ji = ai ? ji : 0; }
+                if constexpr (!POP_IMAGES) { ji = map_image(smap_b[map_byte_addr(i)]); ji = ai ? ji : 0; }
                 const DbRow<CELLS> drow = db_row(ji);
                 const uint32_t qrow = (uint32_t)__mul24(i, N1P * 8);
                 int rowsum = 0;
@@ -409,7 +416,7 @@
                         const int ku = pop(rk, vv[u]);
                         ll[u] = 0;
                         if constexpr (POP_IMAGES) { bool vl; ll[u] = pop(rl, vl); }
-                        if constexpr (!POP_IMAGES) ll[u] = smap_b[map_byte_addr(ku)];
+                        if constexpr (!POP_IMAGES) ll[u] = map_image(smap_b[map_byte_addr(ku)]);
                         qcell[u] = *(gptr_u2)(qpairG + (qrow + ((uint32_t)ku << 3)));
                     }
 #pragma unroll
@@ -464,9 +471,9 @@
                 int p;
                 bool none;
                 highest_mapped_upto(mapped, ssei, p, none);
-                const int A = smap_b[map_byte_addr(p)];
+                const int A = map_image(smap_b[map_byte_addr(p)]);
                 SAT_DIAG_DUP_MAPBYTE(&smap_b[map_byte_addr(p)]);
-                oldj = p == ssei ? A : NULLJ;
+                oldj = (p == ssei && !(PS && none)) ? A : NULLJ;
                 const uint32_t above = 0xFFFFFFFEu << (A & 31);
                 const uint32_t y = occ.w[0] & above;
                 const uint32_t gap = (y - 1u) & ~y & above;
@@ -477,7 +484,7 @@
                 bool none;
                 highest_mapped_upto(mapped, ssei, p, none);
                 const int t = qtypes[ssei];
-                const int A = smap_b[map_byte_addr(p)];
+                const int A = map_image(smap_b[map_byte_addr(p)]);
                 oldj = p == ssei ? A : NULLJ;
                 const unsigned long long occ64 = (unsigned long long)occ.w[0] | ((unsigned long long)occ.w[1] << 32);
                 const unsigned long long above = (~1ull) << (A & 63);
@@ -493,7 +500,7 @@
                 bool none;
                 highest_mapped_upto(mapped, ssei, p, none);
                 const int t = qtypes[ssei];
-                const int A = smap_b[map_byte_addr(p)];
+                const int A = map_image(smap_b[map_byte_addr(p)]);
                 oldj = p == ssei ? A : NULLJ;
                 const unsigned long long occ_lo = (unsigned long long)occ.w[0] | ((unsigned long long)occ.w[1] << 32),
                                          occ_hi = (unsigned long long)occ.w[2] | ((unsigned long long)occ.w[3] << 32);
@@ -511,7 +518,8 @@
                 cand.w[2 % M2W] = (uint32_t)c_hi;
                 cand.w[3 % M2W] = (uint32_t)(c_hi >> 32);
             } else {
-                oldj = smap_b[map_byte_addr(ssei)];
+                const uint32_t oldb = smap_b[map_byte_addr(ssei)];
+                oldj = map_unmatched(oldb) ? NULLJ : map_image(oldb);
                 int startj = 0, endj = n2;
                 if (opt_lorder) {
                     Bits<M1W> upto = bits_below<M1W>(ssei + 1), lowpart, highpart;
@@ -522,8 +530,8 @@
                     }
                     const int p = bits_highest<M1W>(lowpart);
                     const int q = bits_lowest<M1W>(highpart);
-                    const int pimg = smap_b[map_byte_addr(p < 0 ? 0 : p)];
-                    const int qimg = smap_b[map_byte_addr(q < 0 ? 0 : q)];
+                    const int pimg = map_image(smap_b[map_byte_addr(p < 0 ? 0 : p)]);
+                    const int qimg = map_image(smap_b[map_byte_addr(q < 0 ? 0 : q)]);
                     startj = p < 0 ? n2 : pimg;
                     endj = (ssei == n1 - 1) ? n2 : (q < 0 ? -1 : qimg);
                 }
@@ -577,6 +585,7 @@
             }
             const bool nreal = cnt != 0;
             const int newj = nreal ? sel : NULLJ;
+            const uint32_t newb = PS ? (nreal ? (uint32_t)sel << 3 : SAT_K_UNMATCHED8) : (uint32_t)newj;
 
             SAT_PHASE(0);
             int delta;
@@ -693,7 +702,7 @@
             if (lsoln && newscore > best) {
                 if (beats_leader(newscore, restart)) {
                     for (int w = 0; w < n1w; w++) bmap[w * T + tid] = smap[w * TP + tid];
-                    bmap_b[bmap_byte_addr(ssei)] = (uint8_t)newj;
+                    bmap_b[bmap_byte_addr(ssei)] = (uint8_t)newb;
                 }
             }
             best = max(best, newscore);
@@ -705,7 +714,7 @@
                     if (nreal) bits_set<M2W>(rset, newj);
                     if (replay && part == 0) {
                         for (int w = 0; w < n1w; w++) bmap[w * T + tid] = smap[w * TP + tid];
-                        bmap_b[bmap_byte_addr(ssei)] = (uint8_t)newj;
+                        bmap_b[bmap_byte_addr(ssei)] = (uint8_t)newb;
                     }
                 }
             }
@@ -719,7 +728,7 @@
             else
                 p = *(gptr_f32)((gptr_c)ptabG + (((uint32_t)rowoff + nd) << 2));
             const bool accept = p > u;
-            if (accept) smap_b[map_byte_addr(ssei)] = (uint8_t)newj;
+            if (accept) smap_b[map_byte_addr(ssei)] = (uint8_t)newb;
             score = accept ? newscore : score;
             {
                 const bool oreal_ = oldj != NULLJ;
@@ -764,8 +773,8 @@
             if (any && part == 0) {
                 int8_t *out = mx.maps + (mrow * mx.max_matches + tid) * (size_t)mx.map_pitch;
                 for (int i = 0; i < n1; i++) {
-                    const int j = bmap_b[bmap_byte_addr(i)];
-                    out[i] = (int8_t)(j == NULLJ ? -1 : j);
+                    const uint32_t b = bmap_b[bmap_byte_addr(i)];
+                    out[i] = (int8_t)(map_unmatched(b) ? -1 : map_image(b));
                 }
             }
             return;
@@ -796,8 +805,8 @@
         ((((unsigned long long)(uint32_t)(best + 0x40000000)) << 32) | (0xFFFFFFFFu - best_restart)) == win) {
         int8_t *out = PAIRS ? px.maps + (size_t)pit.pair * SAT_K_MAXDIM : Q.ssemaps + (size_t)e * n1;
         for (int i = 0; i < n1; i++) {
-            int j = bmap_b[bmap_byte_addr(i)];
-            out[i] = (int8_t)(j == NULLJ ? -1 : j);
+            const uint32_t b = bmap_b[bmap_byte_addr(i)];
+            out[i] = (int8_t)(map_unmatched(b) ? -1 : map_image(b));
         }
     }
 
diff --git a/cuda_satabsearch_amd/csrc/sat_sa_kernel.hpp b/cuda_satabsearch_amd/csrc/sat_sa_kernel.hpp
--- a/cuda_satabsearch_amd/csrc/sat_sa_kernel.hpp
+++ b/cuda_satabsearch_amd/csrc/sat_sa_kernel.hpp
@@ -19,7 +19,7 @@
 #define SAT_DIAG_FS_ROWS_ONLY 0
 #endif
 #ifndef SAT_DIAG_DUP_CELLS
-#define SAT_DIAG_DUP_CELLS(row, l0, l1, l2, l3)
+#define SAT_DIAG_DUP_CELLS(a0, a1, a2, a3)
 #endif
 #ifndef SAT_DIAG_DUP_MAPWORD
 #define SAT_DIAG_DUP_MAPWORD(p)
@@ -252,20 +252,29 @@
 }
 
 template <int CELLS> struct DbRow;
-template <> struct DbRow<SAT_CELLS_FULL8> { const uint2 *cells; };
+template <> struct DbRow<SAT_CELLS_FULL8> { uint32_t base; };
 template <> struct DbRow<SAT_CELLS_FULL5> { const float *dist; const uint8_t *code; };
 template <> struct DbRow<SAT_CELLS_TRI5> { const float *dist; const uint8_t *code; int j; };
 __host__ __device__ inline int cell_layout(int n2max) { return n2max <= 32 ? SAT_CELLS_FULL8 : (n2max <= 48 ? SAT_CELLS_FULL5 : SAT_CELLS_TRI5); }
 __host__ __device__ inline int set_words(int n2) { return n2 <= 32 ? 1 : (n2 <= 64 ? 2 : 4); }
+__host__ __device__ constexpr bool prescaled_maps(int cells) { return cells == SAT_CELLS_FULL8; }
+#define SAT_K_UNMATCHED8 0x04u
+__host__ __device__ inline int full8_row_shift(int n2) { return n2 > 1 ? 32 - __builtin_clz((unsigned)(n2 - 1)) : 0; }
 __device__ __forceinline__ int tri_index(int j, int l)
 {
     const int mx = max(j, l), mn = min(j, l);
     return (int)((__umul24((uint32_t)mx, (uint32_t)mx) + (uint32_t)mx) >> 1) + mn;
 }
 __host__ __device__ inline uint32_t tri_cells(int n2) { return (uint32_t)(n2 + 1) * (uint32_t)(n2 + 2) / 2u; }
+__device__ __forceinline__ uint2 lds_cell8(uint32_t addr)
+{
+    typedef uint32_t u32x2_t __attribute__((ext_vector_type(2)));
+    const u32x2_t v = *(const __attribute__((address_space(3))) u32x2_t *)(uintptr_t)addr;
+    return uint2{ v.x, v.y };
+}
 template <int CELLS> __device__ __forceinline__ uint2 db_cell(const DbRow<CELLS> row, int l)
 {
-    if constexpr (CELLS == SAT_CELLS_FULL8) return row.cells[l];
+    if constexpr (CELLS == SAT_CELLS_FULL8) return lds_cell8(row.base + ((uint32_t)l << 3));
     else if constexpr (CELLS == SAT_CELLS_FULL5) return uint2{ __float_as_uint(row.dist[l]), row.code[l] };
     else { const int c = tri_index(row.j, l); return uint2{ __float_as_uint(row.dist[c]), row.code[c] }; }
 }
@@ -274,10 +283,19 @@
 __device__ __forceinline__ int quad_terms(const float4 qd, const uint32_t qc, const DbRow<CELLS> row,
                                           const uint32_t word, const uint32_t force, const int acc)
 {
-    const uint32_t l0 = word & 0xFFu, l1 = (word >> 8) & 0xFFu, l2 = (word >> 16) & 0xFFu, l3 = word >> 24;
-    SAT_DIAG_DUP_CELLS(row, l0, l1, l2, l3);
-    const uint2 d0 = db_cell<CELLS>(row, (int)l0), d1 = db_cell<CELLS>(row, (int)l1), d2 = db_cell<CELLS>(row, (int)l2),
-                d3 = db_cell<CELLS>(row, (int)l3);
+    uint2 d0, d1, d2, d3;
+    if constexpr (prescaled_maps(CELLS)) {
+        const uint32_t a0 = __builtin_amdgcn_bitop3_b32(word, 0xF8u, row.base, 0xEA),
+                       a1 = __builtin_amdgcn_bitop3_b32(word >> 8, 0xF8u, row.base, 0xEA),
+                       a2 = __builtin_amdgcn_bitop3_b32(word >> 16, 0xF8u, row.base, 0xEA),
+                       a3 = __builtin_amdgcn_bitop3_b32(word >> 24, 0xF8u, row.base, 0xEA);
+        SAT_DIAG_DUP_CELLS(a0, a1, a2, a3);
+        d0 = lds_cell8(a0); d1 = lds_cell8(a1); d2 = lds_cell8(a2); d3 = lds_cell8(a3);
+    } else {
+        const uint32_t l0 = word & 0xFFu, l1 = (word >> 8) & 0xFFu, l2 = (word >> 16) & 0xFFu, l3 = word >> 24;
+        d0 = db_cell<CELLS>(row, (int)l0); d1 = db_cell<CELLS>(row, (int)l1); d2 = db_cell<CELLS>(row, (int)l2);
+        d3 = db_cell<CELLS>(row, (int)l3);
+    }
     const float t0 = 4.0f - fabsf(qd.x - __uint_as_float(d0.x));
     const float t1 = 4.0f - fabsf(qd.y - __uint_as_float(d1.x));
     const float t2 = 4.0f - fabsf(qd.z - __uint_as_float(d2.x));
@@ -288,7 +306,8 @@
                        __builtin_amdgcn_perm(d3.y, d2.y, 0x04000C0Cu) ^ qc;
     const uint32_t z = (x + 0x77777777u) & 0x88888888u;
     uint32_t sel = __builtin_amdgcn_bitop3_b32(z >> 3, z >> 6, 0x03030303u, 0xA8);
-    sel = __builtin_amdgcn_bitop3_b32(far >> 5, 0x04040404u, sel, 0xEA);
+    if constexpr (prescaled_maps(CELLS)) sel |= __builtin_amdgcn_bitop3_b32(far >> 5, word, 0x04040404u, 0xA8);
+    else sel = __builtin_amdgcn_bitop3_b32(far >> 5, 0x04040404u, sel, 0xEA);
     sel |= force;
     const uint32_t terms = __builtin_amdgcn_perm(0u, 0xFE010102u, sel);
     return __builtin_amdgcn_sdot4((int)terms, 0x01010101, acc, false);
@@ -373,7 +392,7 @@
 {
     LdsLayout L;
     const bool split = cells != SAT_CELLS_FULL8;
-    uint32_t dcells = (uint32_t)n2 * (uint32_t)(n2 + 1);
+    uint32_t dcells = split ? (uint32_t)n2 * (uint32_t)(n2 + 1) : (uint32_t)n2 << full8_row_shift(n2);
     uint32_t off;
     if (split) {
         if (cells == SAT_CELLS_TRI5) dcells = tri_cells(n2);
diff --git a/include/satabsearch.h b/include/satabsearch.h
--- a/include/satabsearch.h
+++ b/include/satabsearch.h
@@ -106,6 +106,7 @@
 
 void sat_debug_lds_layout(int m2w, int n1, int n1p, int n2, int chains, int threads, int q_in_lds, int compact,
                           uint32_t out[11]);
+uint32_t sat_debug_slot_stride(uint32_t lds_bytes, int n2max);
 
 typedef struct sat_multi sat_multi;
 sat_multi *sat_multi_create(int ndev, const int *devices, uint64_t seed);
```
